# hyperplane-lab/ACL-GAN

Hardware: AMD Instinct MI355X
Metric: training images/sec at 256x256 (gen+dis step) (higher is better)
Workload: dtype fp32

## Files before the change

acl-gan_amd/_lib.py:

```python
import ctypes as C
import os

_HERE = os.path.dirname(os.path.abspath(__file__))
LIB_PATH = os.path.join(_HERE, "libaclgan_hip.so")


class AclganError(RuntimeError):
    pass


if not os.path.exists(LIB_PATH):
    raise ImportError(
        "libaclgan_hip.so not found at %s -- build it first (python -c 'import __graft_entry__ as g; g.build()' "
        "or make -C acl-gan_amd/csrc).  There is no fallback path." % LIB_PATH)

lib = C.CDLL(LIB_PATH)


class Arch(C.Structure):
    _fields_ = [(n, C.c_int) for n in (
        "input_dim_a", "input_dim_b", "gen_dim", "gen_mlp_dim", "gen_style_dim", "gen_output_dim",
        "gen_n_downsample", "gen_n_res", "dis_dim", "dis_n_layer", "dis_num_scales")]


class HParams(C.Structure):
    _fields_ = [(n, C.c_float) for n in (
        "gan_w", "gan_cw", "recon_x_w", "focus_loss", "focus_delta", "focus_upper", "focus_lower",
        "focus_epsilon", "alpha")]


class Adam(C.Structure):
    _fields_ = [(n, C.c_float) for n in ("lr", "beta1", "beta2", "eps", "weight_decay")]


class ConvDesc(C.Structure):
    _fields_ = [(n, C.c_int) for n in ("B", "Hi", "Wi", "Ci", "Co", "k", "stride", "pad", "upsample", "act")]


class ImageDesc(C.Structure):
    _fields_ = [("src_offset", C.c_int64)] + [(n, C.c_int) for n in (
        "src_h", "src_w", "res_h", "res_w", "crop_y", "crop_x", "flip", "tab_x", "tab_y", "ksize_x", "ksize_y")]


GRID_MAX_SRCS = 16


class GridSrc(C.Structure):
    _fields_ = [("data", C.c_void_p), ("bstride", C.c_int64), ("n", C.c_int), ("channels", C.c_int)]


ACT = {"none": 0, "relu": 1, "lrelu": 2, "tanh": 3}
NORM = {"none": 0, "in": 1, "adain": 2, "ln": 3, "sn": 4}
DTYPE = {"fp32": 0, "bf16": 1, "fp16": 2}
GROUP_GEN, GROUP_DIS, GROUP_SN_STATE = 0, 1, 2
EMA_COPY, EMA_BLEND = 0, 1
WEIGHTS_LIVE, WEIGHTS_EMA = 0, 1
NETS = {"gen_AB": 0, "gen_BA": 1, "dis_A": 2, "dis_B": 3, "dis_2": 4}
LOSS_NAMES = [
    "loss_gen_adv_A", "loss_gen_adv_B", "loss_gen_adv_2",
    "loss_gen_focus_B_size", "loss_gen_focus_B_digit", "loss_gen_focus_A_size", "loss_gen_focus_A_digit",
    "loss_gen_focus_A2_size", "loss_gen_focus_A2_digit", "loss_idt_A", "loss_idt_B", "loss_gen_total",
    "loss_dis_A", "loss_dis_B", "loss_dis_2", "loss_dis_total",
]

vp, ci, cf, i64, sz = C.c_void_p, C.c_int, C.c_float, C.c_int64, C.c_size_t
BUCKET_FN = C.CFUNCTYPE(None, vp, ci, ci, i64, i64)
SYNC_FN = C.CFUNCTYPE(None, vp, vp, ci)

SIGNATURES = {
    "aclgan_version": (ci, []),
    "aclgan_launch_count": (C.c_longlong, []),
    "aclgan_gemm_slices_f32": (ci, [vp, vp, vp, ci, ci, ci, ci, vp]),
    "aclgan_winograd_filter_frag": (ci, [vp, vp, ci, ci, ci, vp]),
    "aclgan_conv3x3_winograd_fused": (ci, [vp, vp, vp, vp, ci, ci, ci, ci, ci, ci, ci, ci, vp, vp]),
    "aclgan_gemm_slices_x3_scratch_bytes": (sz, [ci, ci, ci, ci]),
    "aclgan_gemm_slices_x3": (ci, [vp, vp, vp, ci, ci, ci, ci, vp, vp]),
    "aclgan_set_deterministic": (ci, [ci]),
    "aclgan_get_deterministic": (ci, []),
    "aclgan_last_error": (C.c_char_p, []),
    "aclgan_ctx_create": (ci, [C.POINTER(Arch), C.POINTER(vp)]),
    "aclgan_ctx_create_dis_norm": (ci, [C.POINTER(Arch), ci, C.POINTER(vp)]),
    "aclgan_ctx_destroy": (None, [vp]),
    "aclgan_ctx_enable_capture": (ci, [vp]),
    "aclgan_warm_streams": (ci, [ci]),
    "aclgan_debug_capture_masks": (ci, [vp, vp, sz]),
    "aclgan_debug_mask_count": (ci, [vp]),
    "aclgan_debug_mask_info": (ci, [vp, ci, C.POINTER(ci), C.POINTER(C.c_longlong), C.POINTER(ci)]),
    "aclgan_group_numel": (i64, [vp, ci]),
    "aclgan_tensor_count": (ci, [vp, ci]),
    "aclgan_tensor_info": (ci, [vp, ci, ci, C.c_char_p, ci, C.POINTER(i64), C.POINTER(ci), C.POINTER(ci)]),
    "aclgan_bind_params": (ci, [vp, ci, vp, vp, vp, vp]),
    "aclgan_bind_sn_state": (ci, [vp, vp]),
    "aclgan_sn_scratch_bytes": (sz, [ci, vp, vp]),
    "aclgan_sn_power_iteration": (ci, [ci, vp, vp, vp, vp, vp, vp, vp, vp, vp]),
    "aclgan_sn_fold": (ci, [ci, vp, vp, vp, vp, vp, vp, vp, vp, vp, vp]),
    "aclgan_workspace_bytes": (ci, [vp, ci, ci, ci, C.POINTER(sz)]),
    "aclgan_bind_workspace": (ci, [vp, vp, sz]),
    "aclgan_forward_workspace_bytes": (ci, [vp, ci, ci, ci, C.POINTER(sz)]),
    "aclgan_step_algorithmic_bytes": (ci, [vp, ci, ci, ci, ci, C.POINTER(C.c_double)]),
    "aclgan_step_executed_flops": (ci, [vp, ci, ci, ci, ci, C.POINTER(C.c_double)]),
    "aclgan_gen_update": (ci, [vp, vp, vp, vp, ci, ci, ci, C.POINTER(HParams), vp, vp]),
    "aclgan_dis_update": (ci, [vp, vp, vp, vp, ci, ci, ci, C.POINTER(HParams), vp, vp]),
    "aclgan_set_grad_buckets": (ci, [vp, i64, BUCKET_FN, vp]),
    "aclgan_set_forward_sync": (ci, [vp, SYNC_FN, vp, ci]),
    "aclgan_focus_loss_global": (ci, [vp, i64, vp, i64, cf, cf, cf, cf, cf, vp, vp, vp, vp]),
    "aclgan_bucket_schedule": (ci, [vp, ci, ci, ci, ci, ci, C.POINTER(ci), ci, C.POINTER(ci)]),
    "aclgan_zero_grad": (ci, [vp, ci, vp]),
    "aclgan_adam_step": (ci, [vp, ci, C.POINTER(Adam), ci, vp]),
    "aclgan_bind_ema": (ci, [vp, ci, vp]),
    "aclgan_adam_step_ema": (ci, [vp, ci, C.POINTER(Adam), ci, cf, ci, vp]),
    "aclgan_set_forward_weights": (ci, [vp, ci]),
    "aclgan_gen_encode": (ci, [vp, ci, vp, ci, ci, ci, vp, vp, vp]),
    "aclgan_gen_decode": (ci, [vp, ci, vp, vp, ci, ci, ci, vp, vp]),
    "aclgan_dis_forward": (ci, [vp, ci, vp, ci, ci, ci, C.POINTER(vp), vp]),
    "aclgan_conv2d_fwd": (ci, [C.POINTER(ConvDesc), vp, vp, vp, vp, vp]),
    "aclgan_conv2d_fwd_ws": (ci, [C.POINTER(ConvDesc), vp, vp, vp, vp, vp, vp]),
    "aclgan_conv2d_fwd_scratch_bytes": (sz, [C.POINTER(ConvDesc)]),
    "aclgan_conv2d_fwd_naive": (ci, [C.POINTER(ConvDesc), vp, vp, vp, vp, vp]),
    "aclgan_set_compute_dtype": (ci, [vp, ci]),
    "aclgan_bind_params16": (ci, [vp, ci, vp, vp]),
    "aclgan_bind_loss_scale": (ci, [vp, vp]),
    "aclgan_conv16_eligible": (ci, [C.POINTER(ConvDesc), ci]),
    "aclgan_pack_weights16": (ci, [vp, vp, vp, ci, ci, ci, ci, vp]),
    "aclgan_conv2d_fwd16": (ci, [C.POINTER(ConvDesc), ci, vp, vp, vp, vp, vp, vp, vp]),
    "aclgan_conv2d_fwd16_x16": (ci, [C.POINTER(ConvDesc), ci, vp, vp, vp, vp, vp, vp, vp]),
    "aclgan_conv2d_dgrad16": (ci, [C.POINTER(ConvDesc), ci, vp, vp, vp, vp, ci, vp, vp]),
    "aclgan_conv2d_wgrad16": (ci, [C.POINTER(ConvDesc), ci, vp, vp, vp, vp, vp, vp]),
    "aclgan_conv16s_ok": (ci, [C.POINTER(ConvDesc), ci]),
    "aclgan_conv2d_fwd16s": (ci, [C.POINTER(ConvDesc), ci, vp, vp, vp, vp, ci, vp]),
    "aclgan_set_tuning": (ci, [C.c_char_p, ci]),
    "aclgan_tuning": (ci, [C.c_char_p, ci, C.POINTER(ci)]),
    "aclgan_tuning_get": (ci, [C.c_char_p, C.POINTER(C.c_longlong)]),
    "aclgan_check_workspace": (ci, [vp, ci, ci, ci]),
    "aclgan_conv2d_fwd16s_stats_chunk": (ci, [C.POINTER(ConvDesc)]),
    "aclgan_conv2d_fwd16s_stats": (ci, [C.POINTER(ConvDesc), ci, vp, vp, vp, vp, ci, vp, vp]),
    "aclgan_conv2d_dgrad16s_scratch_bytes": (sz, [C.POINTER(ConvDesc)]),
    "aclgan_conv2d_dgrad16s": (ci, [C.POINTER(ConvDesc), ci, vp, vp, vp, ci, ci, vp, vp]),
    "aclgan_conv2d_wgrad16_st": (ci, [C.POINTER(ConvDesc), ci, vp, ci, vp, ci, vp, vp, vp, vp]),
    "aclgan_cast_storage": (ci, [vp, ci, vp, ci, i64, vp]),
    "aclgan_norm_fwd_st": (ci, [ci, ci, ci, ci, ci, vp, vp, vp, ci, vp, vp, vp, vp, vp, C.POINTER(ci), vp]),
    "aclgan_norm_bwd_st": (ci, [ci, ci, ci, ci, ci, vp, vp, vp, vp, ci, vp, vp, vp, vp, vp, vp, ci, vp, C.POINTER(ci), vp]),
    "aclgan_conv2d_fwd16_x16_st": (ci, [C.POINTER(ConvDesc), ci, vp, vp, vp, vp, vp, ci, vp, vp]),
    "aclgan_norm_fwd_x": (ci, [ci, ci, ci, ci, ci, vp, vp, vp, ci, vp, vp, vp, vp, vp, vp, ci, C.POINTER(ci), vp, vp]),
    "aclgan_norm_bwd_x": (ci, [ci, ci, ci, ci, ci, vp, vp, vp, vp, ci, vp, vp, vp, vp, vp, vp, ci, vp, C.POINTER(ci), vp, vp, vp]),
    "aclgan_norm_bwd_ln_params": (ci, [vp, ci, ci, vp, vp, vp]),
    "aclgan_conv2d_fwd16_scratch_bytes": (sz, [C.POINTER(ConvDesc)]),
    "aclgan_conv2d_dgrad16_scratch_bytes": (sz, [C.POINTER(ConvDesc)]),
    "aclgan_conv2d_wgrad16_scratch_bytes": (sz, [C.POINTER(ConvDesc)]),
    "aclgan_conv2d_dgrad": (ci, [C.POINTER(ConvDesc), vp, vp, vp, vp, ci, vp]),
    "aclgan_conv2d_dgrad_scratch_bytes": (sz, [C.POINTER(ConvDesc)]),
    "aclgan_conv2d_wgrad": (ci, [C.POINTER(ConvDesc), vp, vp, vp, vp, vp]),
    "aclgan_conv2d_wgrad_ws": (ci, [C.POINTER(ConvDesc), vp, vp, vp, vp, vp, vp]),
    "aclgan_conv2d_wgrad_scratch_bytes": (sz, [C.POINTER(ConvDesc)]),
    "aclgan_norm_fwd": (ci, [ci, ci, ci, ci, ci, vp, vp, vp, ci, vp, vp, vp, vp, vp, vp]),
    "aclgan_conv2d_block_fwd": (ci, [C.POINTER(ConvDesc), ci, ci, vp, vp, vp, vp, vp, ci, vp, vp, vp, vp, vp, vp, C.POINTER(C.c_int), vp]),
    "aclgan_conv2d_block_fwd_scratch_bytes": (sz, [C.POINTER(ConvDesc)]),
    "aclgan_norm_bwd": (ci, [ci, ci, ci, ci, ci, vp, vp, vp, vp, ci, vp, vp, vp, vp, vp, vp, ci, vp, vp]),
    "aclgan_norm_scratch_bytes": (sz, [ci, ci, ci]),
    "aclgan_avgpool3s2_fwd": (ci, [ci, ci, ci, ci, vp, vp, vp]),
    "aclgan_avgpool3s2_bwd": (ci, [ci, ci, ci, ci, vp, vp, ci, vp]),
    "aclgan_adam_flat": (ci, [vp, vp, vp, vp, i64, C.POINTER(Adam), ci, vp]),
    "aclgan_adam_flat_ema": (ci, [vp, vp, vp, vp, vp, i64, C.POINTER(Adam), ci, cf, ci, vp]),
    "aclgan_linear_fwd": (ci, [ci, ci, ci, vp, vp, vp, ci, vp, vp]),
    "aclgan_mlp3_fwd": (ci, [ci, ci, ci, ci, vp, vp, vp, vp, vp, vp, vp, vp, vp, vp, vp]),
    "aclgan_linear_bwd": (ci, [ci, ci, ci, vp, vp, vp, vp, ci, vp, vp, vp, vp]),
    "aclgan_gap_fwd": (ci, [ci, ci, ci, vp, vp, vp]),
    "aclgan_gap_bwd": (ci, [ci, ci, ci, vp, vp, ci, vp]),
    "aclgan_focus_blend_fwd": (ci, [ci, ci, vp, vp, vp, vp, vp, vp]),
    "aclgan_focus_blend_bwd": (ci, [ci, ci, vp, vp, vp, vp, vp, vp, ci, vp]),
    "aclgan_focus_translation_nchw": (ci, [vp, i64, vp, i64, vp, i64, vp, ci, ci, vp]),
    "aclgan_lsgan_loss": (ci, [vp, ci, cf, cf, vp, vp, cf, vp]),
    "aclgan_lsgan_loss_multi": (ci, [vp, vp, vp, vp, vp, vp, vp, ci, vp]),
    "aclgan_l1_loss": (ci, [vp, ci, vp, i64, vp, vp, cf, ci, vp]),
    "aclgan_focus_loss_scratch_bytes": (sz, [i64]),
    "aclgan_focus_loss": (ci, [vp, i64, cf, cf, cf, cf, cf, vp, vp, vp, vp, vp]),
    "aclgan_nchw_to_nhwc": (ci, [vp, vp, ci, ci, ci, ci, vp]),
    "aclgan_nhwc_to_nchw": (ci, [vp, vp, ci, ci, ci, ci, vp]),
    "aclgan_image_resample_ksize": (ci, [ci, ci]),
    "aclgan_image_resample_coeffs": (ci, [ci, ci, C.POINTER(ci), C.POINTER(ci)]),
    "aclgan_image_batch_transform": (ci, [vp, C.POINTER(ImageDesc), vp, ci, vp, vp, ci, ci, vp]),
    "aclgan_image_grid_scratch_bytes": (sz, []),
    "aclgan_image_grid_u8": (ci, [C.POINTER(GridSrc), ci, ci, ci, ci, vp, vp, vp]),
}

for _name, (_res, _args) in SIGNATURES.items():
    _fn = getattr(lib, _name)
    _fn.restype = _res
    _fn.argtypes = _args


def last_error() -> str:
    return lib.aclgan_last_error().decode("utf-8", "replace")


def check(rc: int, what: str = ""):
    if rc != 0:
        raise AclganError("%s failed (code %d): %s" % (what or "libaclgan_hip call", rc, last_error()))


def ptr(t):
    return None if t is None else C.c_void_p(t.data_ptr())


def stream_ptr(device=None):
    import torch
    return C.c_void_p(torch.cuda.current_stream(device).cuda_stream)
```

acl-gan_amd/csrc/common.h:

```cpp
#pragma once
#include <hip/hip_runtime.h>
#include <stdint.h>
#include <stddef.h>
#include <string>
#include <atomic>
#include "../../include/aclgan_hip.h"
#include "switches.h"

namespace aclgan {

void set_error(const char* fmt, ...);
int hip_fail(hipError_t e, const char* what);

extern std::atomic<long long> g_launches;

#define ACL_CHECK_LAUNCH(what)                                           \
    do {                                                                 \
        ++::aclgan::g_launches;                                          \
        hipError_t e__ = hipGetLastError();                              \
        if (e__ != hipSuccess) return ::aclgan::hip_fail(e__, what);     \
    } while (0)

#define ACL_REQUIRE(cond, ...)                                           \
    do {                                                                 \
        if (!(cond)) { ::aclgan::set_error(__VA_ARGS__); return ACLGAN_EINVAL; } \
    } while (0)

int reduce_slices_ordered(const float* part, int64_t n, int nslices, float* out, hipStream_t st);
size_t colsum_ordered_bytes(int64_t M, int C);
int colsum_ordered(const float* dy, float* db, int64_t M, int C, void* part, hipStream_t st);

static inline int cdiv(int a, int b) { return (a + b - 1) / b; }
static inline int64_t cdiv64(int64_t a, int64_t b) { return (a + b - 1) / b; }

struct ConvGeom {
    int B, Hi, Wi, Ci, Co, k, s, p, up, act;
    int Hu, Wu;
    int Hp, Wp;
    int Ho, Wo;
    int M;
    int K;
};
int make_geom(const aclgan_conv_desc* d, ConvGeom* g);

int conv_fold(const ConvGeom& g, const float* dxp, float* dx, int accumulate, hipStream_t st);
double conv_exec_flops(const ConvGeom& g, int which, bool f16);
bool conv_wgrad_fast_supported(const ConvGeom& g);
int conv_fwd(const ConvGeom& g, const float* x, const float* w, const float* bias, float* y, hipStream_t st, void* scratch = nullptr, float* stats = nullptr,
             float* keepV = nullptr);
size_t conv_fwd_keep_bytes(const ConvGeom& g);
int conv_fwd_stats_chunk(const ConvGeom& g);
size_t conv_fwd_scratch_bytes(const ConvGeom& g);
size_t conv_up5_scratch_bytes(const ConvGeom& g);
int conv_up5_fwd(const ConvGeom& g, const float* x, const float* w, const float* bias, float* y, void* scratch, hipStream_t st, float* keepV = nullptr);
int conv_fwd_naive(const ConvGeom& g, const float* x, const float* w, const float* bias, float* y, hipStream_t st);
size_t conv_dgrad_scratch_bytes(const ConvGeom& g);
int conv_dgrad(const ConvGeom& g, const float* dy, const float* w, float* dx, void* scratch, int accumulate, hipStream_t st);
int conv_wgrad(const ConvGeom& g, const float* x, const float* dy, float* dw, float* db, hipStream_t st, void* scratch = nullptr, const float* haveV = nullptr);
size_t conv_wgrad_scratch_bytes(const ConvGeom& g);
int conv_up5_dgrad(const ConvGeom& g, const float* dy, const float* w, float* dx, int accumulate, void* scratch, hipStream_t st);
int conv_up5_wgrad(const ConvGeom& g, const float* x, const float* dy, float* dw, float* db, void* scratch, hipStream_t st, const float* haveV = nullptr);

int conv_fwd_fast(const ConvGeom& g, const float* x, const float* w, const float* bias, float* y, hipStream_t st, void* scratch = nullptr, float* stats = nullptr,
                  float* keepV = nullptr);
size_t conv_fwd_fast_scratch_bytes(const ConvGeom& g);
int conv_dgrad_fast(const ConvGeom& g, const float* dy, const float* w, float* dxp, float* dx, int accumulate, bool* direct, hipStream_t st);
int conv_wgrad_fast(const ConvGeom& g, const float* x, const float* dy, float* dw, float* db, hipStream_t st, void* scratch = nullptr, const float* haveV = nullptr);
size_t conv_wgrad_fast_scratch_bytes(const ConvGeom& g);

struct WinoUCache { void* user; float* (*lookup)(void* user, const float* w, int variant, size_t bytes, bool* fresh); };
void set_wino_ucache(const WinoUCache* c);
const WinoUCache* wino_ucache();
size_t conv_wino_u_bytes(const ConvGeom& g);
int conv_wino_u_variant(const ConvGeom& g, int dgrad, bool keepV);
int conv_up5_wino_u_variant(const ConvGeom& g, int dgrad, bool keepV);
int conv_wino_prefill(const ConvGeom& g, int uv, const float* w0, int64_t w_stride, float* U0, int64_t u_stride, int count, hipStream_t st);
int wino_fused_filter_batch(const float* w0, int64_t w_stride, float* Uf0, int64_t u_stride, int count, int Co, int Ci, int flip, hipStream_t st);

bool conv_wino_ok(const ConvGeom& g);
size_t conv_wino_scratch_bytes(const ConvGeom& g);
int conv_fwd_wino(const ConvGeom& g, const float* x, const float* w, const float* bias, float* y, void* scratch, hipStream_t st, float* stats = nullptr,
                  float* keepV = nullptr);
size_t conv_wino_keep_bytes(const ConvGeom& g);
size_t conv_up5_wino_keep_bytes(const ConvGeom& g);
int conv_dgrad_wino_interior(const ConvGeom& g, const float* dy, const float* w, float* dx, int accumulate, void* scratch, hipStream_t st);
size_t conv_wgrad_wino_scratch_bytes(const ConvGeom& g);
bool conv_up5_wino_ok(const ConvGeom& g);
size_t conv_up5_wino_fwd_scratch_bytes(const ConvGeom& g);
size_t conv_up5_wino_dgrad_scratch_bytes(const ConvGeom& g);
size_t conv_up5_wino_wgrad_scratch_bytes(const ConvGeom& g);
int conv_up5_wino_fwd_phases(const ConvGeom& g, const float* x, const float* wp, const float* bias, float* y, void* scratch, hipStream_t st, float* keepV = nullptr,
                             const float* wkey = nullptr);
int conv_up5_wino_dgrad_phases(const ConvGeom& g, const float* dy, const float* wp, float* dx, int accumulate, void* scratch, hipStream_t st,
                               const float* wkey = nullptr);
bool wino_u_cached(const float* wkey, int variant);
int conv_up5_wino_wgrad_phases(const ConvGeom& g, const float* x, const float* dy, float* dwp, float* db, void* scratch, hipStream_t st, const float* haveV = nullptr);
size_t conv_up5_dgrad_scratch_bytes(const ConvGeom& g);
// ... 120 lines not shown
```

acl-gan_amd/csrc/engine.hip:

```cpp
#include "common.h"
#include <dlfcn.h>

#include <functional>
#include <map>
#include <string>
#include <vector>
#include <tuple>
#include <mutex>
#include <algorithm>
#include <cstring>
#include <cstdio>
#include <cstdlib>

namespace aclgan {

struct TensorInfo {
    std::string name;
    int64_t offset;
    int64_t numel;
    int shape[4];
    int ndim;
};

struct Group {
// ... 62 lines not shown
struct StreamPool {
    static const int N = 4;
    hipStream_t s[N] = {nullptr, nullptr, nullptr, nullptr};
    static StreamPool& of_device() {
        static StreamPool pools[16];
        int dev = 0;
        (void)hipGetDevice(&dev);
        return pools[(dev >= 0 && dev < 16) ? dev : 0];
    }
    int get(int i, hipStream_t* out) {
        static std::mutex mu;
        std::lock_guard<std::mutex> lock(mu);
        if (!s[i]) {
            const hipError_t e = hipStreamCreateWithFlags(&s[i], hipStreamNonBlocking);
            if (e != hipSuccess) { s[i] = nullptr; return hip_fail(e, "stream pool"); }
        }
        *out = s[i];
        return ACLGAN_OK;
    }
};
}

struct aclgan_ctx {
    aclgan_arch arch;
    int dis_norm = ACLGAN_NORM_NONE;
    struct SnLayer { int co, k; std::string key; int64_t u_off, v_off; };
    std::vector<SnLayer> sn_layers[5];
    Group sn;
    std::vector<std::string> pass_names;
    std::vector<int> tape_pass;
    std::map<std::string, int> pass_count;
    int cur_pass = -1;
    int pass_begin(const char* net, const char* what) {
        if (!Roctx::get().on || dry) return -1;
        const std::string base = std::string(net) + "." + what;
        const int n = ++pass_count[base];
        pass_names.push_back(base + "#" + std::to_string(n));
        const int prev = cur_pass;
        cur_pass = (int)pass_names.size() - 1;
        Roctx::get().push((pass_names.back() + "@" + std::to_string((long long)g_launches)).c_str());
        return prev;
    }
    void pass_end(int prev) {
        if (!Roctx::get().on || dry) return;
        Roctx::get().pop();
        Roctx::get().push(("~end@" + std::to_string((long long)g_launches)).c_str());
        Roctx::get().pop();
        cur_pass = prev;
    }
    Group groups[2];
    char* ws = nullptr;
    size_t ws_bytes = 0;
    hipStream_t st = nullptr;
    bool dry = false;
    size_t top = 0, peak = 0;
    std::vector<Act*> acts;
    std::vector<TapeOp> tape;
    int dtype = ACLGAN_DTYPE_FP32;
    unsigned short* w16[2] = {nullptr, nullptr};
    unsigned short* w16t[2] = {nullptr, nullptr};
    float* lscale = nullptr;
    float* ema = nullptr;
    int fwd_weights = ACLGAN_WEIGHTS_LIVE;
    bool read_ema = false;
    const float* weights(int group) const { return group == ACLGAN_GROUP_GEN && read_ema ? ema : groups[group].param; }
    std::vector<int64_t> cv_off[2];
    std::vector<int> cv_co[2], cv_taps[2], cv_ci[2];
    int trained = -1;
    bool fire_dry = false;
    aclgan_sync_fn sync_fn = nullptr;
    void* sync_user = nullptr;
    int sync_world = 1;
    int64_t bucket_elems = 0;
    aclgan_bucket_fn bucket_fn = nullptr;
    void* bucket_user = nullptr;
    std::vector<int> bucket_order;
    struct NeedKey {
        int which, B, H, W, dtype; long long epoch; int determ, buckets;
        bool operator<(const NeedKey& o) const {
            return std::tie(which, B, H, W, dtype, epoch, determ, buckets) < std::tie(o.which, o.B, o.H, o.W, o.dtype, o.epoch, o.determ, o.buckets);
        }
    };
    std::map<NeedKey, size_t> need_cache;
    double alg_bytes = 0.0;
    void count(double bytes) { alg_bytes += bytes; }
    double exec_flops = 0.0;
    size_t keep_total = 0;
    struct MaskEnt { int B, H, W, C, act; long long off; };
    unsigned char* mask_dst = nullptr; size_t mask_cap = 0, mask_top = 0;
    std::vector<MaskEnt> mask_log;
    struct UEnt { float* u; bool filled; int layout; int lane, ck; };
    std::map<std::pair<const float*, int>, UEnt> ucache;
    WinoUCache ucache_hook;
    static float* ucache_lookup(void* user, const float* w, int variant, size_t bytes, bool* fresh) {
        aclgan_ctx* c = (aclgan_ctx*)user;
        const int layout = variant >> 4;
        auto it = c->ucache.find(std::make_pair(w, variant & 15));
        if (it == c->ucache.end()) return nullptr;
        UEnt& e = it->second;
        if (!e.filled) {
            *fresh = true;
            if (bytes) { e.filled = true; e.layout = layout; e.lane = c->cur_lane; e.ck = c->nck(c->cur_lane); }
            return e.u;
        }
        if (e.layout != layout) return nullptr;
        *fresh = false;
        if (bytes && c->nlanes > 1 && e.lane != c->cur_lane && c->wait_ck(c->cur_lane, e.lane, e.ck) != ACLGAN_OK) return nullptr;
        return e.u;
    }
    int ucache_reserve(const float* w, int variant, size_t bytes) {
        if (sw(SW_NOUCACHE) || !bytes || ucache.count(std::make_pair(w, variant))) return ACLGAN_OK;
        float* u = (float*)alloc(bytes);
        if (!u) return ACLGAN_ENOMEM;
        ucache[std::make_pair(w, variant)] = UEnt{u, false, 0, 0, 0};
        return ACLGAN_OK;
    }
    bool act16() const { return dtype != ACLGAN_DTYPE_FP32 && sw(SW_ACT16); }

    hipStream_t st2 = nullptr;
    hipEvent_t ev_fork = nullptr, ev_join = nullptr;
    bool side_pending = false;
    size_t top2 = 0, peak2 = 0;
    void* alloc2(size_t bytes) {
        const size_t need = top2 + ((bytes + 255) & ~(size_t)255);
        top2 = need;
        if (need > peak2) peak2 = need;
        if (dry) return (void*)(uintptr_t)4096;
        if (peak + need + 256 > ws_bytes) return nullptr;
        return ws + ((ws_bytes - need) & ~(size_t)255);
    }
    int side_fork() {
        if (dry) return ACLGAN_OK;
        if (!st2) {
            int rc = aclgan::StreamPool::of_device().get(0, &st2_pool);
            if (rc) return rc;
            st2 = st2_pool;
        }
        if (st2 == st) return ACLGAN_OK;
        if (!ev_fork) {
            hipError_t e = hipEventCreateWithFlags(&ev_fork, hipEventDisableTiming);
            if (e == hipSuccess) e = hipEventCreateWithFlags(&ev_join, hipEventDisableTiming);
            if (e != hipSuccess) return aclgan::hip_fail(e, "side stream events");
        }
        hipError_t e = hipEventRecord(ev_fork, st);
        if (e == hipSuccess) e = hipStreamWaitEvent(st2, ev_fork, 0);
        if (e != hipSuccess) return aclgan::hip_fail(e, "side stream fork");
        side_pending = true;
        return ACLGAN_OK;
    }
    int side_join() {
        if (dry || !side_pending) return ACLGAN_OK;
        hipError_t e = hipEventRecord(ev_join, st2);
        if (e == hipSuccess) e = hipStreamWaitEvent(st0 ? st0 : st, ev_join, 0);
        if (e != hipSuccess) return aclgan::hip_fail(e, "side stream join");
        side_pending = false;
        return ACLGAN_OK;
    }

    static const int MAXL = 4;
    hipStream_t st0 = nullptr;
    hipStream_t lane_st[MAXL] = {nullptr, nullptr, nullptr, nullptr};
    int nlanes = 1, cur_lane = 0;
    std::vector<hipEvent_t> ev_pool; size_t ev_next = 0;
    std::vector<hipEvent_t> lane_evs[MAXL];
    int seen[MAXL][MAXL] = {};
    size_t hw[MAXL] = {0, 0, 0, 0};
    bool lane_dirty[MAXL] = {false, false, false, false};
    int pass_seq = 0, cur_pass_id = -1;
    hipStream_t lane_stream(int l) const { return l == 0 ? st0 : lane_st[l]; }
    int nck(int l) const { return (int)lane_evs[l].size(); }
    hipStream_t st2_pool = nullptr;
    int lanes_begin(int want) {
        nlanes = std::max(1, std::min(want, (int)MAXL));
        if (!sw(SW_SIDE_STREAM)) nlanes = 1;
        bool capturing = false;
        if (!dry) {
            hipStreamCaptureStatus cs = hipStreamCaptureStatusNone;
            if (hipStreamIsCapturing(st, &cs) == hipSuccess && cs != hipStreamCaptureStatusNone) capturing = true;
            else (void)hipGetLastError();
        }
        if (capturing) nlanes = 1;
        cur_lane = 0; st0 = st;
        for (int l = 0; l < MAXL; ++l) { lane_evs[l].clear(); hw[l] = 0; lane_dirty[l] = false; for (int m = 0; m < MAXL; ++m) seen[l][m] = 0; }
        ev_next = 0;
        if (dry) return ACLGAN_OK;
        if (sw(SW_SIDE_STREAM) && !st2_pool) { int rc = aclgan::StreamPool::of_device().get(0, &st2_pool); if (rc) return rc; }
        st2 = capturing ? st : st2_pool;
        for (int l = 1; l < nlanes; ++l)
            if (!lane_st[l]) { int rc = aclgan::StreamPool::of_device().get(l, &lane_st[l]); if (rc) return rc; }
        return ACLGAN_OK;
    }
    int checkpoint(int l) {
        hipEvent_t ev = nullptr;
        if (!dry) {
            if (ev_next == ev_pool.size()) {
                hipEvent_t e = nullptr;
                hipError_t rc = hipEventCreateWithFlags(&e, hipEventDisableTiming);
                if (rc != hipSuccess) return aclgan::hip_fail(rc, "lane event");
                ev_pool.push_back(e);
            }
            ev = ev_pool[ev_next++];
            hipError_t rc = hipEventRecord(ev, lane_stream(l));
            if (rc != hipSuccess) return aclgan::hip_fail(rc, "lane checkpoint");
        }
        lane_evs[l].push_back(ev);
        lane_dirty[l] = false;
        return ACLGAN_OK;
    }
    int mark() { return nlanes > 1 ? checkpoint(cur_lane) : ACLGAN_OK; }
    int set_lane(int l) {
        if (nlanes <= 1) return ACLGAN_OK;
        l %= nlanes;
// ... 15 lines not shown
        if (!dry) {
            hipError_t e = hipStreamWaitEvent(lane_stream(d), lane_evs[s][k], 0);
            if (e != hipSuccess) return aclgan::hip_fail(e, "lane wait");
        }
        lane_dirty[d] = true;
        seen[d][s] = k + 1;
        return ACLGAN_OK;
    }
    int need(Act* a) {
        if (nlanes <= 1 || !a) return ACLGAN_OK;
        Act* r = a->root();
        for (int i = 0; i < r->ndst; ++i)
            if (r->dst[i].lane != cur_lane) { int rc = wait_ck(cur_lane, r->dst[i].lane, r->dst[i].ck); if (rc) return rc; }
        return ACLGAN_OK;
    }
    void wrote(Act* a) {
        if (!a) return;
        Act* r = a->root();
        for (int i = 0; i < r->ndst; ++i)
            if (r->dst[i].lane == cur_lane) { r->dst[i].ck = nck(cur_lane); return; }
        if (r->ndst < 4) r->dst[r->ndst++] = Act::Stamp{cur_lane, nck(cur_lane)};
    }
    int acq(Act* a) {
        if (nlanes <= 1 || !a) return ACLGAN_OK;
        Act* r = a->root();
        if (r->gst.lane >= 0 && r->gst.lane != cur_lane) { int rc = wait_ck(cur_lane, r->gst.lane, r->gst.ck); if (rc) return rc; }
        r->gst = Act::Stamp{cur_lane, nck(cur_lane)};
        return ACLGAN_OK;
    }
    int lanes_join() {
        if (nlanes > 1) {
            int rc = set_lane(0);
            if (rc) return rc;
            for (int l = 1; l < nlanes; ++l) {
                if (lane_dirty[l]) { rc = checkpoint(l); if (rc) return rc; }
                if (nck(l) > 0) { rc = wait_ck(0, l, nck(l) - 1); if (rc) return rc; }
            }
        }
        return side_join();
    }
    int lanes_barrier() {
        int rc = lanes_join();
        if (rc || nlanes <= 1) return rc;
        rc = checkpoint(0);
        if (rc) return rc;
        for (int l = 1; l < nlanes; ++l) { rc = wait_ck(l, 0, nck(0) - 1); if (rc) return rc; }
        for (int l = 0; l < MAXL; ++l) hw[l] = 0;
        return ACLGAN_OK;
    }
    void lanes_quiesce() {
        if (dry) return;
        for (int l = 1; l < nlanes; ++l) if (lane_st[l]) (void)hipStreamSynchronize(lane_st[l]);
        if (st2) (void)hipStreamSynchronize(st2);
        side_pending = false;
        cur_lane = 0; if (st0) st = st0;
    }
    ~aclgan_ctx() {
        reset_step();
        if (ev_fork) (void)hipEventDestroy(ev_fork);
        if (ev_join) (void)hipEventDestroy(ev_join);
        for (hipEvent_t e : ev_pool) (void)hipEventDestroy(e);
    }
    void reset_step() {
        for (Act* a : acts) delete a;
        acts.clear();
        tape.clear();
        tape_pass.clear(); pass_names.clear(); pass_count.clear(); cur_pass = -1;
        top = 0;
        top2 = 0;
        keep_total = 0;
        ucache.clear();
        read_ema = false;
        for (int l = 0; l < MAXL; ++l) { lane_evs[l].clear(); hw[l] = 0; lane_dirty[l] = false; for (int m = 0; m < MAXL; ++m) seen[l][m] = 0; }
        ev_next = 0; cur_lane = 0; nlanes = 1; pass_seq = 0; cur_pass_id = -1;
        if (st0) { st = st0; st0 = nullptr; }
    }
    void* alloc(size_t bytes) {
        size_t a = (top + 255) & ~(size_t)255;
        if (nlanes > 1) for (int l = 0; l < nlanes; ++l) if (l != cur_lane && hw[l] > a) a = hw[l];
        top = a + bytes;
        if (nlanes > 1) { const size_t e = (top + 255) & ~(size_t)255; if (e > hw[cur_lane]) hw[cur_lane] = e; }
        if (top > peak) peak = top;
        if (dry) return (void*)(uintptr_t)(a + 4096);
        if (top + peak2 + 256 > ws_bytes) return nullptr;
        return ws + a;
    }
    float* allocf(int64_t n) { return (float*)alloc((size_t)n * sizeof(float)); }
    Act* new_act(int B, int H, int W, int C, bool need_grad, int st = 0) {
        Act* a = new Act();
        a->B = B; a->H = H; a->W = W; a->C = C; a->need_grad = need_grad; a->dt = st; a->gdt = st;
        a->d = (float*)alloc((size_t)a->numel() * (st ? 2 : 4));
        if (need_grad) a->g = allocf(a->numel());
        acts.push_back(a);
        wrote(a);
        return a;
    }
    Act* new_view(Act* joint, int b0, int nb) {
        Act* a = new Act();
        a->B = nb; a->H = joint->H; a->W = joint->W; a->C = joint->C; a->need_grad = joint->need_grad;
        const int64_t off = (int64_t)b0 * joint->H * joint->W * joint->C;
        a->d = joint->d + off;
        a->g = joint->g ? joint->g + off : nullptr;
        a->parent = joint;
        acts.push_back(a);
        return a;
    }
    void push(std::function<int()> fn, std::initializer_list<std::pair<const float*, int64_t>> grads = {}) {
        TapeOp op;
        op.fn = std::move(fn);
        if (trained >= 0 && groups[trained].grad)
            for (const auto& g : grads)
                if (g.first && g.second > 0 && op.ng < 4 && g.first >= groups[trained].grad && g.first < groups[trained].grad + groups[trained].numel) {
                    op.goff[op.ng] = g.first - groups[trained].grad; op.gnum[op.ng] = g.second; ++op.ng;
                }
        op.lane = cur_lane; op.pass = cur_pass_id;
        tape.push_back(std::move(op));
        tape_pass.push_back(cur_pass);
    }
    PW pw(int group, int net, const std::string& key, bool with_bias = true) const;
    int64_t numel_of(int group, int net, const std::string& key) const;
    const float* param(int group, int net, const std::string& key) const;
    float* gradp(int group, int net, const std::string& key) const;
};

namespace aclgan {


#define RUN(expr)                                  \
    do {                                           \
        if (!c.dry) { int rc__ = (expr); if (rc__) return rc__; } \
    } while (0)
#define CHK(expr)                                  \
    do { int rc__ = (expr); if (rc__) return rc__; } while (0)
#define NEED(ptr)                                  \
    do { if (!(ptr)) { set_error("workspace too small (need > %zu bytes, bound %zu)", c.top, c.ws_bytes); return ACLGAN_ENOMEM; } } while (0)

static void add_tensor(Group& g, const std::string& name, int ndim, int d0, int d1 = 1, int d2 = 1, int d3 = 1) {
    TensorInfo t;
    t.name = name; t.offset = g.numel; t.ndim = ndim;
    t.shape[0] = d0; t.shape[1] = d1; t.shape[2] = d2; t.shape[3] = d3;
    t.numel = (int64_t)d0 * d1 * d2 * d3;
    g.index[name] = (int)g.tensors.size();
    g.tensors.push_back(t);
    g.numel += (t.numel + 3) / 4 * 4;
}
static void add_conv(Group& g, const std::string& prefix, int co, int ci, int k) {
    add_tensor(g, prefix + ".weight", 4, co, ci, k, k);
    add_tensor(g, prefix + ".bias", 1, co);
}

static void build_gen(Group& g, const std::string& net, const aclgan_arch& a) {
    char buf[160];
    const int nd = a.gen_n_downsample, nr = a.gen_n_res, sd = a.gen_style_dim;
    int d = a.gen_dim;
    add_conv(g, net + "/enc_style.model.0.conv", d, a.input_dim_a, 7);
    for (int i = 0; i < 2; ++i) { snprintf(buf, sizeof buf, "/enc_style.model.%d.conv", 1 + i); add_conv(g, net + buf, 2 * d, d, 4); d *= 2; }
    for (int i = 0; i < 2; ++i) { snprintf(buf, sizeof buf, "/enc_style.model.%d.conv", 3 + i); add_conv(g, net + buf, d, d, 4); }
    add_conv(g, net + "/enc_style.model.6", sd, d, 1);
    d = a.gen_dim;
    add_conv(g, net + "/enc_content.model.0.conv", d, a.input_dim_a, 7);
    for (int i = 0; i < nd; ++i) { snprintf(buf, sizeof buf, "/enc_content.model.%d.conv", 1 + i); add_conv(g, net + buf, 2 * d, d, 4); d *= 2; }
    for (int r = 0; r < nr; ++r)
        for (int j = 0; j < 2; ++j) { snprintf(buf, sizeof buf, "/enc_content.model.%d.model.%d.model.%d.conv", 1 + nd, r, j); add_conv(g, net + buf, d, d, 3); }
    for (int r = 0; r < nr; ++r)
        for (int j = 0; j < 2; ++j) { snprintf(buf, sizeof buf, "/dec.model.0.model.%d.model.%d.conv", r, j); add_conv(g, net + buf, d, d, 3); }
    int idx = 2;
    for (int i = 0; i < nd; ++i) {
        snprintf(buf, sizeof buf, "/dec.model.%d.norm.gamma", idx); add_tensor(g, net + buf, 1, d / 2);
        snprintf(buf, sizeof buf, "/dec.model.%d.norm.beta", idx); add_tensor(g, net + buf, 1, d / 2);
        snprintf(buf, sizeof buf, "/dec.model.%d.conv", idx); add_conv(g, net + buf, d / 2, d, 5);
        d /= 2; idx += 2;
    }
    snprintf(buf, sizeof buf, "/dec.model.%d.conv", idx - 1); add_conv(g, net + buf, a.gen_output_dim, d, 7);
    const int C = a.gen_dim << nd, nad = 2 * C * 2 * nr, md = a.gen_mlp_dim;
    add_tensor(g, net + "/mlp.model.0.fc.weight", 2, md, sd); add_tensor(g, net + "/mlp.model.0.fc.bias", 1, md);
    add_tensor(g, net + "/mlp.model.1.fc.weight", 2, md, md); add_tensor(g, net + "/mlp.model.1.fc.bias", 1, md);
    add_tensor(g, net + "/mlp.model.2.fc.weight", 2, nad, md); add_tensor(g, net + "/mlp.model.2.fc.bias", 1, nad);
}

static void build_dis(Group& g, const std::string& net, int input_dim, const aclgan_arch& a, std::vector<aclgan_ctx::SnLayer>* sn = nullptr,
                      Group* st = nullptr) {
    char buf[160];
    for (int s = 0; s < a.dis_num_scales; ++s) {
        int d = a.dis_dim;
        snprintf(buf, sizeof buf, "/cnns.%d.0.conv", s); add_conv(g, net + buf, d, input_dim, 4);
        for (int i = 0; i < a.dis_n_layer - 1; ++i) {
            snprintf(buf, sizeof buf, "/cnns.%d.%d.conv", s, i + 1);
            if (sn) {
                const std::string pre = net + buf + ".module.";
                add_tensor(g, pre + "bias", 1, 2 * d);
                add_tensor(g, pre + "weight_bar", 4, 2 * d, d, 4, 4);
                aclgan_ctx::SnLayer L;
                L.co = 2 * d; L.k = 16 * d; L.key = std::string(buf + 1) + ".module.";
                L.u_off = st->numel; add_tensor(*st, pre + "weight_u", 1, L.co);
                L.v_off = st->numel; add_tensor(*st, pre + "weight_v", 1, L.k);
                sn->push_back(L);
            } else {
                add_conv(g, net + buf, 2 * d, d, 4);
            }
            d *= 2;
        }
        snprintf(buf, sizeof buf, "/cnns.%d.%d", s, a.dis_n_layer); add_conv(g, net + buf, 1, d, 1);
    }
}

static const char* NET_NAMES[5] = {"gen_AB", "gen_BA", "dis_A", "dis_B", "dis_2"};

}

const float* aclgan_ctx::param(int group, int net, const std::string& key) const {
    const Group& g = groups[group];
    auto it = g.index.find(std::string(NET_NAMES[net]) + "/" + key);
    if (it == g.index.end() || !g.param) return nullptr;
    return weights(group) + g.tensors[it->second].offset;
}
float* aclgan_ctx::gradp(int group, int net, const std::string& key) const {
    const Group& g = groups[group];
    auto it = g.index.find(std::string(NET_NAMES[net]) + "/" + key);
    if (it == g.index.end() || !g.grad) return nullptr;
    return g.grad + g.tensors[it->second].offset;
}
int64_t aclgan_ctx::numel_of(int group, int net, const std::string& key) const {
    const Group& g = groups[group];
    auto it = g.index.find(std::string(NET_NAMES[net]) + "/" + key);
    return it == g.index.end() ? 0 : g.tensors[it->second].numel;
}
PW aclgan_ctx::pw(int group, int net, const std::string& key, bool with_bias) const {
    PW p;
    p.w = param(group, net, key + ".weight"); p.dw = gradp(group, net, key + ".weight"); p.nw = numel_of(group, net, key + ".weight");
    if (with_bias) { p.b = param(group, net, key + ".bias"); p.db = gradp(group, net, key + ".bias"); p.nb = numel_of(group, net, key + ".bias"); }
    if (dtype != ACLGAN_DTYPE_FP32 && p.w && w16[group] && w16t[group]) {
        const int64_t off = p.w - weights(group);
        p.w16 = w16[group] + off; p.w16t = w16t[group] + off;
    }
    return p;
}

namespace aclgan {

struct PassScope {
    aclgan_ctx& c; int prev, prev_id;
    PassScope(aclgan_ctx& c_, int net, const char* what) : c(c_), prev(c_.pass_begin(NET_NAMES[net], what)), prev_id(c_.cur_pass_id) { c.cur_pass_id = c.pass_seq++; }
    ~PassScope() { c.pass_end(prev); c.cur_pass_id = prev_id; }
};

struct NormSpec {
    int kind = ACLGAN_NORM_NONE;
    const float* w = nullptr; const float* b = nullptr;
    float* dw = nullptr; float* db = nullptr;
    int w_stride = 0;
};

static inline void mark_written(Act* a) { a->gw = true; }

static int conv_block(aclgan_ctx& c, const PW& W, bool train_w, Act* in, int Co, int k, int stride, int pad, int up, int act,
                      const NormSpec& ns, Act* residual, Act** out_p, int out16 = 1) {
    aclgan_conv_desc d;
    d.B = in->B; d.Hi = in->H; d.Wi = in->W; d.Ci = in->C; d.Co = Co; d.k = k; d.stride = stride; d.pad = pad; d.upsample = up;
    d.act = ns.kind == ACLGAN_NORM_NONE ? act : ACLGAN_ACT_NONE;
    ConvGeom g;
    CHK(make_geom(&d, &g));
    if (!W.w) { set_error("conv_block: parameters not bound"); return ACLGAN_EINVAL; }
    CHK(c.need(in)); CHK(c.need(residual));
    Act* const gin = in;
    const bool want_grad = train_w || in->need_grad || ns.dw != nullptr;
    const bool has_norm = ns.kind != ACLGAN_NORM_NONE;
    const int dt = c.dtype;
    const bool h16 = dt != ACLGAN_DTYPE_FP32 && W.w16 != nullptr;
    const bool f16 = h16 && conv16_eligible(g, 0), d16 = h16 && conv16_eligible(g, 1), w16 = h16 && conv16_eligible(g, 2);
    const bool a16 = h16 && c.act16();
    const bool s_bwd = a16 && f16 && d16 && w16 && conv16s_ok(g, 1);
    const bool s_fwd = a16 && f16 && conv16s_ok(g, 0) && in->dt != 0;
    if (in->dt != 0 && !(f16 && (w16 || !train_w))) {
        Act* in32 = c.new_act(in->B, in->H, in->W, in->C, false, 0);
        NEED(in32->d);
        RUN(cast_storage(in->d, in->dt, in32->d, 0, in->numel(), c.st));
        in = in32;
    }
    const int out_st = (a16 && Co % 64 == 0 && out16) ? dt : 0;
    const int co_st = has_norm ? ((s_bwd && sw(SW_CO16)) ? dt : 0) : ((f16 || !out_st) ? out_st : 0);
    Act* co = c.new_act(g.B, g.Ho, g.Wo, Co, want_grad, co_st);
    NEED(co->d); if (want_grad) NEED(co->g);
    Act* out = co;
    float *mean = nullptr, *rstd = nullptr, *ss = nullptr;
    const int HW = g.Ho * g.Wo;
    if (has_norm) {
        out = c.new_act(g.B, g.Ho, g.Wo, Co, want_grad, out_st);
        NEED(out->d); if (want_grad) NEED(out->g);
        const int nstat = ns.kind == ACLGAN_NORM_LN ? g.B : g.B * Co;
        mean = c.allocf(nstat); rstd = c.allocf(nstat);
        NEED(mean); NEED(rstd);
        if (want_grad && (act == ACLGAN_ACT_RELU || act == ACLGAN_ACT_LRELU) && sw(SW_NORM_MASK)) { ss = c.allocf((int64_t)2 * g.B * Co); NEED(ss); }
        co->gdt = s_bwd ? dt : 0;
    } else if (out_st && !co_st) {
        out = c.new_act(g.B, g.Ho, g.Wo, Co, want_grad, out_st);
        NEED(out->d); if (want_grad) NEED(out->g);
        out->gdt = 0;
    } else {
        out->gdt = s_bwd ? co_st : 0;
    }
    if (gin->need_grad && !s_bwd) gin->gdt = 0;
    float* keepV = nullptr;
    if (train_w && !f16 && !w16) {
        const size_t kb = conv_fwd_keep_bytes(g);
        if (kb && c.keep_total + kb <= (size_t)(sw_real(SW_KEEPV_BUDGET_GB) * 1073741824.0) + 1) { keepV = (float*)c.alloc(kb); NEED(keepV); c.keep_total += kb; }
    }
    const size_t ubytes = f16 ? 0 : conv_wino_u_bytes(g);
    if (ubytes && c.ucache_reserve(W.w, g.up ? 2 : 0, ubytes)) { set_error("workspace too small (filter-transform cache)"); return ACLGAN_ENOMEM; }
    const double es_in = in->dt ? 2.0 : 4.0, es_co = co->dt ? 2.0 : 4.0, es_out = out->dt ? 2.0 : 4.0, es_w = f16 ? 2.0 : 4.0;
    c.count(es_in * (double)in->numel() + es_w * (double)Co * g.K + 4.0 * Co + es_co * (double)co->numel());
    c.exec_flops += conv_exec_flops(g, 0, f16);
    if (out != co) c.count((es_co + es_out) * (double)co->numel() + ((has_norm && residual) ? (residual->dt ? 2.0 : 4.0) * (double)co->numel() : 0.0));
    const size_t mark = c.top;
    const int schunk = !has_norm ? 0 : (s_fwd ? conv_fwd16s_stats_chunk(g) : (!f16 ? conv_fwd_stats_chunk(g) : 0));
    float* stats = nullptr;
    if (schunk) { stats = c.allocf((size_t)2 * g.B * (HW / schunk) * Co); NEED(stats); }
    {
        const size_t fmark = c.top;
        void* fscr = nullptr;
        const size_t fb = s_fwd ? 0 : (f16 ? conv_fwd16_scratch_bytes(g) : conv_fwd_scratch_bytes(g));
        if (fb) { fscr = c.alloc(fb); NEED(fscr); }
        if (s_fwd) RUN(conv_fwd16s(g, dt, in->d, W.w16, W.b, co->d, co->dt, c.st, stats));
        else if (f16) RUN(conv_fwd16(g, dt, in->dt ? nullptr : in->d, W.w, W.w16, W.b, co->d, fscr, c.st, in->dt ? in->d : nullptr, co->dt));
        else RUN(conv_fwd(g, in->d, W.w, W.b, co->d, c.st, fscr, stats, keepV));
        c.top = fmark;
    }
    NormST nst;
    nst.x = co->dt; nst.y = out->dt; nst.res = residual ? residual->dt : 0;
    if (has_norm) {
        void* scr = c.alloc(norm_scratch_bytes(g.B, HW, Co));
        NEED(scr);
        RUN(norm_fwd(ns.kind, act, g.B, HW, Co, co->d, ns.w, ns.b, ns.w_stride, residual ? residual->d : nullptr, out->d, mean, rstd, scr, c.st, stats, schunk, &nst, ss));
    } else if (out != co) {
        RUN(cast_storage(co->d, co->dt, out->d, out->dt, co->numel(), c.st));
    }
    c.top = mark;
    *out_p = out;
    if (c.mask_dst && !c.dry && want_grad && (act == ACLGAN_ACT_RELU || act == ACLGAN_ACT_LRELU)) {
        const size_t n = (size_t)out->numel();
        if (c.mask_top + n > c.mask_cap) { set_error("aclgan_debug_capture_masks: buffer too small (%zu bytes)", c.mask_cap); return ACLGAN_ENOMEM; }
        RUN(positive_mask(out->d, out->dt, c.mask_dst + c.mask_top, (int64_t)n, c.st));
        c.mask_log.push_back(aclgan_ctx::MaskEnt{out->B, out->H, out->W, out->C, act, (long long)c.mask_top});
        c.mask_top += n;
    }
    c.wrote(out); c.wrote(co);
    if (!want_grad) return ACLGAN_OK;
    aclgan_ctx* cp = &c;
    const bool ln_train = ns.kind == ACLGAN_NORM_LN && ns.dw != nullptr;
    c.push([=]() -> int {
        aclgan_ctx& c = *cp;
        if (!out->gw) return ACLGAN_OK;
        CHK(c.acq(out));
        if (residual && residual->need_grad) CHK(c.acq(residual));
        if (gin->need_grad) CHK(c.acq(gin));
        const double eg_out = out->gdt ? 2.0 : 4.0, eg_co = (has_norm ? co->gdt : (s_bwd ? dt : out->gdt)) ? 2.0 : 4.0, eg_in = gin->gdt ? 2.0 : 4.0;
        c.count((es_co + eg_out + eg_co) * (double)co->numel() + ((residual && residual->need_grad) ? (residual->gdt ? 2.0 : 4.0) * (double)co->numel() : 0.0));
        if (train_w) { c.count(es_in * (double)in->numel() + eg_co * (double)co->numel() + 4.0 * ((double)Co * g.K + Co)); c.exec_flops += conv_exec_flops(g, 2, w16); }
        if (gin->need_grad) { c.count(eg_co * (double)co->numel() + es_w * (double)Co * g.K + eg_in * (double)in->numel()); c.exec_flops += conv_exec_flops(g, 1, d16); }
        const bool side = train_w && sw(SW_SIDE_STREAM);
        if (ubytes && gin->need_grad && !d16 && c.ucache_reserve(W.w, g.up ? 3 : 1, ubytes)) { set_error("workspace too small (filter-transform cache)"); return ACLGAN_ENOMEM; }
        float* g16 = nullptr;
        const size_t mark_pre = c.top;
        if (!has_norm && s_bwd && out->gdt == 0) {
            g16 = (float*)c.alloc((size_t)out->numel() * 2);
            NEED(g16);
        }
        float* sbc = nullptr;
        if (ln_train && side) { sbc = c.allocf((int64_t)2 * g.B * Co); NEED(sbc); }
        const size_t mark0 = side ? c.top : mark_pre;
        const float* dyp = nullptr;
        int dy_st = 0;
        if (has_norm) {
            const size_t mark = c.top;
            void* scr = c.alloc(norm_scratch_bytes(g.B, HW, Co));
            NEED(scr);
            float* dres = nullptr; int dacc = 0;
            if (residual && residual->need_grad) { dres = residual->g; dacc = residual->gw ? 1 : 0; mark_written(residual); }
            NormST bst;
            bst.x = co->dt; bst.y = out->dt; bst.dy = out->gdt; bst.dx = co->gdt; bst.dres = residual ? residual->gdt : 0;
            RUN(norm_bwd(ns.kind, act, g.B, HW, Co, co->d, out->d, out->g, ns.w, ns.w_stride, mean, rstd, co->g, ns.dw, ns.db, dres, dacc, scr, c.st, &bst, sbc, ss));
            c.top = mark;
            dyp = co->g; dy_st = co->gdt;
        } else if (s_bwd && out->gdt == 0) {
            RUN(cast_storage(out->g, 0, g16, dt, out->numel(), c.st));
            RUN(act_bwd_inplace(act, out->d, g16, out->numel(), c.st, out->dt, dt));
            dyp = g16; dy_st = dt;
        } else {
            RUN(act_bwd_inplace(act, co->d, out->g, out->numel(), c.st, co->dt, out->gdt));
            dyp = out->g; dy_st = out->gdt;
        }
        if (train_w) {
            const size_t mark = c.top;
            void* wscr = nullptr;
            const size_t wb = w16 ? conv_wgrad16_scratch_bytes(g) : conv_wgrad_scratch_bytes(g);
            hipStream_t wst = c.st;
            if (side) {
                CHK(c.side_fork());
                if (!c.dry) wst = c.st2;
                c.top2 = 0;
                if (wb) { wscr = c.alloc2(wb); if (!wscr) { set_error("workspace too small for the side-stream scratch"); return ACLGAN_ENOMEM; } }
                if (sbc) RUN(norm_bwd_ln_params(sbc, g.B, Co, ns.dw, ns.db, wst));
            } else if (wb) { wscr = c.alloc(wb); NEED(wscr); }
            if (w16) RUN(conv_wgrad16(g, dt, in->d, dyp, W.dw, W.db, wscr, wst, in->dt, dy_st));
            else {
                if (in->dt || dy_st) { set_error("conv_block: fp32 weight-gradient kernel on 16-bit operands"); return ACLGAN_EINVAL; }
                RUN(conv_wgrad(g, in->d, dyp, W.dw, W.db, wst, wscr, keepV));
            }
            c.top = mark;
        }
        if (gin->need_grad) {
            const size_t mark = c.top;
            if (s_bwd) {
                if (!dy_st) { set_error("conv_block: 16-bit-storage dgrad on an fp32 gradient"); return ACLGAN_EINVAL; }
                void* scr = c.alloc(conv_dgrad16s_scratch_bytes(g));
                NEED(scr);
                RUN(conv_dgrad16s(g, dt, dyp, W.w16t, gin->g, gin->gdt, gin->gw ? 1 : 0, scr, c.st));
            } else {
                if (dy_st || gin->gdt) { set_error("conv_block: fp32-output dgrad kernel on 16-bit gradients"); return ACLGAN_EINVAL; }
                void* scr = c.alloc(d16 ? conv_dgrad16_scratch_bytes(g) + 256 : conv_dgrad_scratch_bytes(g));
                NEED(scr);
                if (d16) RUN(conv_dgrad16(g, dt, dyp, W.w, W.w16t, gin->g, gin->gw ? 1 : 0, scr, c.st));
                else RUN(conv_dgrad(g, dyp, W.w, gin->g, scr, gin->gw ? 1 : 0, c.st));
            }
            mark_written(gin);
            c.top = mark;
        }
        c.top = mark0;
        return ACLGAN_OK;
    }, {{train_w ? W.dw : nullptr, W.nw}, {train_w ? W.db : nullptr, W.nb}, {ln_train ? ns.dw : nullptr, Co}, {ln_train ? ns.db : nullptr, Co}});
    return ACLGAN_OK;
}

static int prefill_wino_u(aclgan_ctx& c, int net, int B, int H, int W, bool train) {
    if (sw(SW_NOUCACHE) || !sw(SW_U_BATCH)) return ACLGAN_OK;
    const aclgan_arch& a = c.arch;
    const int nd = a.gen_n_downsample, count = 2 * a.gen_n_res, C = a.gen_dim << nd;
    if (count < 2) return ACLGAN_OK;
    aclgan_conv_desc d;
    d.B = B; d.Hi = H >> nd; d.Wi = W >> nd; d.Ci = C; d.Co = C; d.k = 3; d.stride = 1; d.pad = 1; d.upsample = 0; d.act = ACLGAN_ACT_NONE;
    ConvGeom g;
    if (make_geom(&d, &g)) return ACLGAN_OK;
    const size_t ubytes = conv_wino_u_bytes(g);
    if (!ubytes) return ACLGAN_OK;
    if (c.dtype != ACLGAN_DTYPE_FP32 && c.w16[0] && conv16_eligible(g, 0)) return ACLGAN_OK;
    char buf[160];
    for (int part = 0; part < 2; ++part) {
        std::vector<const float*> ws;
        for (int r = 0; r < a.gen_n_res; ++r)
            for (int j = 0; j < 2; ++j) {
                if (part == 0) snprintf(buf, sizeof buf, "enc_content.model.%d.model.%d.model.%d.conv.weight", 1 + nd, r, j);
                else snprintf(buf, sizeof buf, "dec.model.0.model.%d.model.%d.conv.weight", r, j);
                ws.push_back(c.param(0, net, buf));
            }
        if (!ws[0]) continue;
        const int64_t wstride = ws[1] - ws[0];
        bool even = wstride > 0;
        for (int i = 1; i < count && even; ++i) even = ws[i] && ws[i] - ws[i - 1] == wstride;
        if (!even) continue;
        for (int dgrad = 0; dgrad <= (train ? 1 : 0); ++dgrad) {
            const bool keepV = train && !dgrad && conv_fwd_keep_bytes(g) > 0;
            const int uv = conv_wino_u_variant(g, dgrad, keepV);
            if (uv < 0 || c.ucache.count(std::make_pair(ws[0], uv & 15))) continue;
            float* u0 = nullptr;
            bool contiguous = true;
            const size_t ustride = (ubytes + 255) & ~(size_t)255;
            for (int i = 0; i < count; ++i) {
                float* u = (float*)c.alloc(ubytes);
                NEED(u);
                if (i == 0) u0 = u;
                else if ((char*)u != (char*)u0 + (size_t)i * ustride) contiguous = false;
                c.ucache[std::make_pair(ws[i], uv & 15)] = aclgan_ctx::UEnt{u, contiguous, uv >> 4, c.cur_lane, c.nck(c.cur_lane)};
            }
            if (!contiguous) {
                for (int i = 0; i < count; ++i) c.ucache[std::make_pair(ws[i], uv & 15)].filled = false;
                continue;
            }
            RUN(conv_wino_prefill(g, uv, ws[0], wstride, u0, (int64_t)(ustride / sizeof(float)), count, c.st));
        }
    }
    return ACLGAN_OK;
}

static int prefill_on_side_lane(aclgan_ctx& c, int B, int H, int W, bool train) {
    const int AB = ACLGAN_NET_GEN_AB, BA = ACLGAN_NET_GEN_BA;
    if (c.nlanes <= 1) { CHK(prefill_wino_u(c, AB, B, H, W, train)); return prefill_wino_u(c, BA, B, H, W, train); }
    const int LP = c.nlanes - 1;
    CHK(c.mark());
    const int k0 = c.nck(0) - 1;
    CHK(c.set_lane(LP));
    CHK(c.wait_ck(LP, 0, k0));
    CHK(prefill_wino_u(c, AB, B, H, W, train)); CHK(prefill_wino_u(c, BA, B, H, W, train));
    CHK(c.mark());
    return c.set_lane(0);
}

static int content_encode(aclgan_ctx& c, int net, bool train, Act* x, Act** out) {
    PassScope pass(c, net, "encode");
    const aclgan_arch& a = c.arch;
    char buf[160];
    NormSpec in_; in_.kind = ACLGAN_NORM_IN;
    Act* h = nullptr;
    int d = a.gen_dim;
    CHK(conv_block(c, c.pw(0, net, "enc_content.model.0.conv"), train, x, d, 7, 1, 3, 0, ACLGAN_ACT_RELU, in_, nullptr, &h));
    for (int i = 0; i < a.gen_n_downsample; ++i) {
        snprintf(buf, sizeof buf, "enc_content.model.%d.conv", 1 + i);
        CHK(conv_block(c, c.pw(0, net, buf), train, h, 2 * d, 4, 2, 1, 0, ACLGAN_ACT_RELU, in_, nullptr, &h));
        d *= 2;
    }
    for (int r = 0; r < a.gen_n_res; ++r) {
        Act *t = nullptr, *o = nullptr;
        snprintf(buf, sizeof buf, "enc_content.model.%d.model.%d.model.0.conv", 1 + a.gen_n_downsample, r);
        CHK(conv_block(c, c.pw(0, net, buf), train, h, d, 3, 1, 1, 0, ACLGAN_ACT_RELU, in_, nullptr, &t));
        snprintf(buf, sizeof buf, "enc_content.model.%d.model.%d.model.1.conv", 1 + a.gen_n_downsample, r);
        CHK(conv_block(c, c.pw(0, net, buf), train, t, d, 3, 1, 1, 0, ACLGAN_ACT_NONE, in_, h, &o));
        h = o;
    }
    *out = h;
    return ACLGAN_OK;
}

static int dense(aclgan_ctx& c, const PW& W, bool train_w, Act* in, int O, int act, Act** out_p, bool launch = true) {
    const int B = in->B, I = in->H * in->W * in->C;
    const bool want = train_w || in->need_grad;
    CHK(c.need(in));
    Act* out = c.new_act(B, 1, 1, O, want);
    NEED(out->d); if (want) NEED(out->g);
    if (!W.w) { set_error("dense: parameters not bound"); return ACLGAN_EINVAL; }
    if (launch) RUN(linear_fwd(B, I, O, in->d, W.w, W.b, act, out->d, c.st));
    c.count(4.0 * ((double)B * I + (double)O * I + O + (double)B * O) * (want ? 3.0 : 1.0));
    c.wrote(out);
    *out_p = out;
    if (!want) return ACLGAN_OK;
    aclgan_ctx* cp = &c;
    c.push([=]() -> int {
        aclgan_ctx& c = *cp;
        if (!out->gw) return ACLGAN_OK;
        CHK(c.acq(out));
        if (in->need_grad) CHK(c.acq(in));
        float* dx = nullptr;
        float* tmp = nullptr;
        const size_t mark = c.top;
        if (in->need_grad) {
            if (in->gw) { tmp = c.allocf((int64_t)B * I); NEED(tmp); dx = tmp; } else dx = in->g;
        }
        const bool side = train_w && sw(SW_SIDE_STREAM);
        RUN(linear_bwd(B, I, O, in->d, out->d, out->g, W.w, act, dx, (train_w && !side) ? W.dw : nullptr, (train_w && !side) ? W.db : nullptr, c.st));
        if (side) {
            CHK(c.side_fork());
            RUN(linear_bwd_params(B, I, O, in->d, out->g, W.dw, W.db, c.st2));
        }
        if (in->need_grad) {
            if (tmp) {
                RUN(gap_bwd(B, 1, I, tmp, in->g, 1, c.st));
            }
            mark_written(in);
        }
        c.top = mark;
        return ACLGAN_OK;
    }, {{train_w ? W.dw : nullptr, W.nw}, {train_w ? W.db : nullptr, W.nb}});
    return ACLGAN_OK;
}

static int style_encode(aclgan_ctx& c, int net, bool train, Act* x, Act** out) {
    PassScope pass(c, net, "style");
    const aclgan_arch& a = c.arch;
    char buf[160];
    NormSpec none;
    Act* h = nullptr;
    int d = a.gen_dim;
    CHK(conv_block(c, c.pw(0, net, "enc_style.model.0.conv"), train, x, d, 7, 1, 3, 0, ACLGAN_ACT_RELU, none, nullptr, &h));
    for (int i = 0; i < 2; ++i) {
        snprintf(buf, sizeof buf, "enc_style.model.%d.conv", 1 + i);
        CHK(conv_block(c, c.pw(0, net, buf), train, h, 2 * d, 4, 2, 1, 0, ACLGAN_ACT_RELU, none, nullptr, &h));
        d *= 2;
    }
    for (int i = 0; i < 2; ++i) {
        snprintf(buf, sizeof buf, "enc_style.model.%d.conv", 3 + i);
        CHK(conv_block(c, c.pw(0, net, buf), train, h, d, 4, 2, 1, 0, ACLGAN_ACT_RELU, none, nullptr, &h));
    }
    const bool want = h->need_grad;
// ... 342 lines not shown
        std::vector<size_t> first(nb, n);
        for (size_t i = 0; i < n; ++i)
            for (int r = 0; r < c.tape[i].ng; ++r) {
                const int64_t b0 = c.tape[i].goff[r] / c.bucket_elems, b1 = (c.tape[i].goff[r] + c.tape[i].gnum[r] - 1) / c.bucket_elems;
                for (int64_t b = b0; b <= b1 && b < nb; ++b) first[b] = std::min(first[b], i);
            }
        done_at.resize(n);
        c.bucket_order.clear();
        for (int b = 0; b < nb; ++b) {
            if (first[b] == n) fire_bucket(c, b);
            else done_at[first[b]].push_back(b);
        }
    }
    CHK(c.lanes_barrier());
    const bool marks = Roctx::get().on && !c.dry && c.tape_pass.size() == n;
    int open = -1, last_pass = -2;
    for (size_t i = n; i-- > 0;) {
        if (marks && c.tape_pass[i] != open) {
            if (open >= 0) { Roctx::get().pop(); Roctx::get().push(("~end@" + std::to_string((long long)g_launches)).c_str()); Roctx::get().pop(); }
            open = c.tape_pass[i];
            if (open >= 0) Roctx::get().push(("bwd:" + c.pass_names[open] + "@" + std::to_string((long long)g_launches)).c_str());
        }
        if (c.tape[i].pass != last_pass) { if (last_pass != -2) CHK(c.mark()); last_pass = c.tape[i].pass; }
        CHK(c.set_lane(c.tape[i].lane));
        int rc_i = c.tape[i].fn();
        if (!rc_i && !c.dry && sw(SW_FAULT_AT) >= 0 && (int)(n - 1 - i) == sw(SW_FAULT_AT)) { set_error("injected fault after backward closure %d (tuning key fault_at)", sw(SW_FAULT_AT)); rc_i = ACLGAN_EHIP; }
        if (rc_i) { if (marks && open >= 0) Roctx::get().pop(); return rc_i; }
        if (buckets && !done_at[i].empty()) {
            const int lane = c.cur_lane;
            CHK(c.lanes_join());
            for (int b : done_at[i]) fire_bucket(c, b);
            CHK(c.set_lane(lane));
        }
    }
    if (marks && open >= 0) { Roctx::get().pop(); Roctx::get().push(("~end@" + std::to_string((long long)g_launches)).c_str()); Roctx::get().pop(); }
    return c.lanes_join();
}
static int run_tape(aclgan_ctx& c) {
    const int rc = run_tape_impl(c);
    if (rc) c.lanes_quiesce();
    return rc;
}

static int check_shape(const aclgan_ctx& c, int B, int H, int W) {
    ACL_REQUIRE(B >= 1 && H >= 64 && W >= 64, "batch shape (%d,%d,%d): need B>=1 and H,W>=64 (third discriminator scale reflect-pads a >=2x2 map)", B, H, W);
    const int q = 1 << c.arch.gen_n_downsample;
    ACL_REQUIRE(H % q == 0 && W % q == 0, "H, W must be multiples of %d (2^n_downsample: decoder output must match the input size)", q);
    return ACLGAN_OK;
}

static int gen_update_impl(aclgan_ctx& c, const float* x_a, const float* x_b, const float* z, int B, int H, int W,
                           const aclgan_hparams& hp, float* L) {
    CHK(check_shape(c, B, H, W));
    const bool focus = hp.focus_loss > 0.f;
    ACL_REQUIRE(c.arch.gen_output_dim == (focus ? 4 : 3), "focus_loss %s 0 needs gen.output_dim %d (trainer.py:107-121), the context was built with %d",
                focus ? ">" : "<=", focus ? 4 : 3, c.arch.gen_output_dim);
    const int sd = c.arch.gen_style_dim;
    const int AB = ACLGAN_NET_GEN_AB, BA = ACLGAN_NET_GEN_BA;
    const int nfs = 2 * focus_sums_blocks((int64_t)B * H * W);
    float* sums = c.allocf((int64_t)3 * nfs);
    NEED(sums);
    if (!c.dry) {
        hipError_t e = hipMemsetAsync(L, 0, sizeof(float) * (ACLGAN_L_GEN_TOTAL + 1), c.st);
        if (e != hipSuccess) return hip_fail(e, "memset losses");
    }
    CHK(c.lanes_begin(sw(SW_LANES)));
    CHK(pack_params(c));
    Act *xa, *xb, *z1, *z2, *z3;
    CHK(input_act(c, x_a, B, 3, H, W, &xa));
    CHK(input_act(c, x_b, B, 3, H, W, &xb));
    CHK(wrap_vec(c, z, B, sd, 1.f, &z1));
    CHK(wrap_vec(c, z + (size_t)B * sd, B, sd, hp.alpha, &z2));
    CHK(wrap_vec(c, z + (size_t)2 * B * sd, B, sd, 1.f, &z3));
    CHK(prefill_on_side_lane(c, B, H, W, true));
    Act *c1, *c2, *s2, *c4, *s4, *c3;
    Act *dB4, *dA4, *xB, *xA, *pA1, *rA4, *rB4, *dA24, *xA2, *pA2;
    Act* jA = c.new_act(2 * B, H, W, 3, true);
    Act* jP = c.new_act(2 * B, H, W, 6, true);
    NEED(jA->d); NEED(jA->g); NEED(jP->d); NEED(jP->g);
    const int L0 = 0, L1 = 1, L2 = c.nlanes > 2 ? 2 : 1, LS = c.nlanes > 2 ? 2 : 0;
#define PASS(expr) do { CHK(expr); CHK(c.mark()); } while (0)
    CHK(c.mark());
    CHK(c.set_lane(L0));
    PASS(content_encode(c, AB, true, xa, &c1));
    CHK(c.set_lane(L1));
    PASS(content_encode(c, BA, true, xa, &c2));
    PASS(style_encode(c, BA, true, xa, &s2));
    CHK(c.set_lane(L0));
    PASS(decode(c, AB, true, c1, z1, &dB4)); CHK(zero_grad_of(c, dB4));
    PASS(blend(c, dB4, xa, nullptr, &xB, nullptr));
    CHK(c.set_lane(L1));
    PASS(decode(c, BA, true, c2, z2, &dA4)); CHK(zero_grad_of(c, dA4));
    Act *vA1 = c.new_view(jA, 0, B), *vP1 = c.new_view(jP, 0, B), *vA2 = c.new_view(jA, B, B), *vP2 = c.new_view(jP, B, B);
    PASS(blend(c, dA4, xa, xa, &xA, &pA1, vA1, vP1));
    CHK(c.set_lane(L0));
    PASS(content_encode(c, BA, true, xB, &c3));
    PASS(decode(c, BA, true, c3, z3, &dA24)); CHK(zero_grad_of(c, dA24));
    PASS(blend(c, dA24, xB, xa, &xA2, &pA2, vA2, vP2));
    CHK(c.set_lane(L1));
    PASS(decode(c, BA, true, c2, s2, &rA4)); CHK(zero_grad_of(c, rA4));
    CHK(c.set_lane(L2));
    PASS(content_encode(c, AB, true, xb, &c4));
    PASS(style_encode(c, AB, true, xb, &s4));
    PASS(decode(c, AB, true, c4, s4, &rB4)); CHK(zero_grad_of(c, rB4));
    PASS(dis_lsgan(c, ACLGAN_NET_DIS_B, false, xB, B, {{1.f, 1.f, hp.gan_w, L + ACLGAN_L_GEN_ADV_B}}, L1, LS));
    if (c.dis_norm != ACLGAN_NORM_SN) {
        PASS(dis_lsgan(c, ACLGAN_NET_DIS_A, false, jA, B, {{1.f, 0.5f, hp.gan_w, L + ACLGAN_L_GEN_ADV_A}, {1.f, 0.5f, hp.gan_w, L + ACLGAN_L_GEN_ADV_A}}, L0, L2));
        PASS(dis_lsgan(c, ACLGAN_NET_DIS_2, false, jP, B, {{1.f, 1.f, hp.gan_cw, L + ACLGAN_L_GEN_ADV_2},
                                                            {0.f, 1.f, hp.gan_cw, L + ACLGAN_L_GEN_ADV_2}}, L1, LS));
    } else {
        PASS(dis_lsgan(c, ACLGAN_NET_DIS_A, false, vA1, B, {{1.f, 0.5f, hp.gan_w, L + ACLGAN_L_GEN_ADV_A}}, L0, L2));
        PASS(dis_lsgan(c, ACLGAN_NET_DIS_A, false, vA2, B, {{1.f, 0.5f, hp.gan_w, L + ACLGAN_L_GEN_ADV_A}}, L0, L2));
        PASS(dis_lsgan(c, ACLGAN_NET_DIS_2, false, vP1, B, {{1.f, 1.f, hp.gan_cw, L + ACLGAN_L_GEN_ADV_2}}, L1, LS));
        PASS(dis_lsgan(c, ACLGAN_NET_DIS_2, false, vP2, B, {{0.f, 1.f, hp.gan_cw, L + ACLGAN_L_GEN_ADV_2}}, L1, LS));
    }
    CHK(c.lanes_join());
    const int64_t npix = (int64_t)B * H * W;
    const float fscale = hp.focus_loss / (float)H / (float)W / (float)B / 3.f;
    struct { Act* a; int size_slot; int digit_slot; } fl[3] = {
        {dB4, ACLGAN_L_GEN_FOCUS_B_SIZE, ACLGAN_L_GEN_FOCUS_B_DIGIT},
        {dA4, ACLGAN_L_GEN_FOCUS_A_SIZE, ACLGAN_L_GEN_FOCUS_A_DIGIT},
        {dA24, ACLGAN_L_GEN_FOCUS_A2_SIZE, ACLGAN_L_GEN_FOCUS_A2_DIGIT}};
    float* ftot = nullptr;
    if (c.sync_fn) { ftot = c.allocf(8); NEED(ftot); }
    for (int i = 0; i < 3 && focus; ++i) RUN(focus_sums(fl[i].a->d, npix, hp.focus_epsilon, hp.focus_upper, sums + (size_t)i * nfs, c.st));
    if (c.mask_dst && !c.dry) {
        auto cap = [&](int code, int C_, size_t n) -> int {
            if (c.mask_top + n > c.mask_cap) { set_error("aclgan_debug_capture_masks: buffer too small (%zu bytes)", c.mask_cap); return ACLGAN_ENOMEM; }
            c.mask_log.push_back(aclgan_ctx::MaskEnt{B, H, W, C_, code, (long long)c.mask_top});
            c.mask_top += n;
            return ACLGAN_OK;
        };
        for (int i = 0; i < 3 && focus; ++i) {
            const size_t n = (size_t)fl[i].a->numel();
            unsigned char* dst = c.mask_dst + c.mask_top;
            CHK(cap(100, fl[i].a->C, n));
            RUN(positive_mask(fl[i].a->d, fl[i].a->dt, dst, (int64_t)n, c.st));
        }
        Act* rr[2] = {rA4, rB4}; Act* xx[2] = {xa, xb};
        for (int i = 0; i < 2; ++i) {
            unsigned char* dst = c.mask_dst + c.mask_top;
            CHK(cap(101, 3, (size_t)npix * 3));
            RUN(positive_mask_diff(rr[i]->d, rr[i]->C, xx[i]->d, 3, dst, npix, c.st));
        }
    }
    c.count(4.0 * (double)npix * ((focus ? 3 * 2 : 0) + 2 * (4 + 3 + 4)));
    if (ftot && focus) {
        RUN(focus_totals(sums, npix, 3, ftot, c.st));
        if (!c.dry) c.sync_fn(c.sync_user, ftot, 6);
    }
    for (int i = 0; i < 3 && focus; ++i)
        RUN(focus_loss_finish(fl[i].a->d, npix, sums + (size_t)i * nfs, hp.focus_delta, hp.focus_upper, hp.focus_lower, hp.focus_epsilon, fscale,
                              L + fl[i].size_slot, L + fl[i].digit_slot, fl[i].a->g, c.st, c.lscale, ftot ? ftot + 2 * i : nullptr,
                              npix * (int64_t)c.sync_world));
    {
        const size_t mark = c.top;
        float* l1p = c.allocf(2 * L1_PART_FLOATS);
        NEED(l1p);
        RUN(l1_loss(rA4->d, rA4->C, xa->d, npix, L + ACLGAN_L_IDT_A, rA4->g, hp.recon_x_w, 1, c.st, c.lscale, l1p));
        RUN(l1_loss(rB4->d, rB4->C, xb->d, npix, L + ACLGAN_L_IDT_B, rB4->g, hp.recon_x_w, 1, c.st, c.lscale, l1p + L1_PART_FLOATS));
        c.top = mark;
    }
    if (!c.dry) {
        hipLaunchKernelGGL(gen_total_kernel, dim3(1), dim3(1), 0, c.st, L, hp, ftot ? fscale / (float)c.sync_world : fscale);
        ACL_CHECK_LAUNCH("gen_total_kernel");
    }
    return run_tape(c);
}

static int dis_update_impl(aclgan_ctx& c, const float* x_a, const float* x_b, const float* z, int B, int H, int W,
                           const aclgan_hparams& hp, float* L) {
    CHK(check_shape(c, B, H, W));
    const bool focus = hp.focus_loss > 0.f;
    ACL_REQUIRE(c.arch.gen_output_dim == (focus ? 4 : 3), "focus_loss %s 0 needs gen.output_dim %d (trainer.py:266-276), the context was built with %d",
                focus ? ">" : "<=", focus ? 4 : 3, c.arch.gen_output_dim);
    const int sd = c.arch.gen_style_dim;
    const int AB = ACLGAN_NET_GEN_AB, BA = ACLGAN_NET_GEN_BA;
    if (!c.dry) {
        hipError_t e = hipMemsetAsync(L + ACLGAN_L_DIS_A, 0, sizeof(float) * 4, c.st);
        if (e != hipSuccess) return hip_fail(e, "memset losses");
    }
    CHK(c.lanes_begin(sw(SW_LANES)));
    CHK(pack_params(c));
    Act *xa, *xb, *z1, *z2, *z3;
    CHK(input_act(c, x_a, B, 3, H, W, &xa));
    CHK(input_act(c, x_b, B, 3, H, W, &xb));
    CHK(wrap_vec(c, z, B, sd, 1.f, &z1));
    CHK(wrap_vec(c, z + (size_t)B * sd, B, sd, hp.alpha, &z2));
    CHK(wrap_vec(c, z + (size_t)2 * B * sd, B, sd, 1.f, &z3));
    CHK(prefill_on_side_lane(c, B, H, W, false));
    Act *c1, *c2, *c3, *dB4, *dA4, *dA24, *xB, *xA, *xA2, *pA1, *pA2;
    Act* jA = c.new_act(3 * B, H, W, 3, false);
    Act* jB = c.new_act(2 * B, H, W, 3, false);
    Act* jP = c.new_act(2 * B, H, W, 6, false);
    NEED(jA->d); NEED(jB->d); NEED(jP->d);
    if (!c.dry) {
        hipError_t e = hipMemcpyAsync(jA->d + (size_t)2 * xa->numel(), xa->d, sizeof(float) * xa->numel(), hipMemcpyDeviceToDevice, c.st);
        if (e == hipSuccess) e = hipMemcpyAsync(jB->d + (size_t)xb->numel(), xb->d, sizeof(float) * xb->numel(), hipMemcpyDeviceToDevice, c.st);
        if (e != hipSuccess) return hip_fail(e, "copy real images into the joint discriminator batch");
    }
    const int L0 = 0, L1 = 1, L2 = c.nlanes > 2 ? 2 : 1, LS = c.nlanes > 2 ? 2 : 0;
    CHK(c.mark());
    CHK(c.set_lane(L0));
    PASS(content_encode(c, AB, false, xa, &c1));
    CHK(c.set_lane(L1));
    PASS(content_encode(c, BA, false, xa, &c2));
    CHK(c.set_lane(L0));
    PASS(decode(c, AB, false, c1, z1, &dB4));
    PASS(blend(c, dB4, xa, nullptr, &xB, nullptr, c.new_view(jB, 0, B), nullptr));
    CHK(c.set_lane(L1));
    PASS(decode(c, BA, false, c2, z2, &dA4));
    PASS(blend(c, dA4, xa, xa, &xA, &pA1, c.new_view(jA, 0, B), c.new_view(jP, 0, B)));
    const bool sn = c.dis_norm == ACLGAN_NORM_SN;
    if (!sn) PASS(dis_lsgan(c, ACLGAN_NET_DIS_B, true, jB, B, {{0.f, 1.f, hp.gan_w, L + ACLGAN_L_DIS_B}, {1.f, 1.f, hp.gan_w, L + ACLGAN_L_DIS_B}}, L1, L2));
    else {
        PASS(dis_lsgan(c, ACLGAN_NET_DIS_B, true, c.new_view(jB, 0, B), B, {{0.f, 1.f, hp.gan_w, L + ACLGAN_L_DIS_B}}, L1, L2));
        PASS(dis_lsgan(c, ACLGAN_NET_DIS_B, true, c.new_view(jB, B, B), B, {{1.f, 1.f, hp.gan_w, L + ACLGAN_L_DIS_B}}, L1, L2));
    }
    CHK(c.set_lane(L0));
    PASS(content_encode(c, BA, false, xB, &c3));
    PASS(decode(c, BA, false, c3, z3, &dA24));
    PASS(blend(c, dA24, xB, xa, &xA2, &pA2, c.new_view(jA, B, B), c.new_view(jP, B, B)));
    if (!sn) {
        PASS(dis_lsgan(c, ACLGAN_NET_DIS_A, true, jA, B, {{0.f, 0.5f, hp.gan_w, L + ACLGAN_L_DIS_A}, {0.f, 0.5f, hp.gan_w, L + ACLGAN_L_DIS_A},
                                                           {1.f, 1.0f, hp.gan_w, L + ACLGAN_L_DIS_A}}, L0, L2));
        PASS(dis_lsgan(c, ACLGAN_NET_DIS_2, true, jP, B, {{0.f, 1.f, hp.gan_cw, L + ACLGAN_L_DIS_2}, {1.f, 1.f, hp.gan_cw, L + ACLGAN_L_DIS_2}}, L1, LS));
    } else {
        Act* vx = c.new_view(jA, 2 * B, B);
        PASS(dis_lsgan(c, ACLGAN_NET_DIS_A, true, c.new_view(jA, 0, B), B, {{0.f, 0.5f, hp.gan_w, L + ACLGAN_L_DIS_A}}, L0, L2));
        PASS(dis_lsgan(c, ACLGAN_NET_DIS_A, true, vx, B, {{1.f, 0.5f, hp.gan_w, L + ACLGAN_L_DIS_A}}, L0, L2));
        PASS(dis_lsgan(c, ACLGAN_NET_DIS_A, true, c.new_view(jA, B, B), B, {{0.f, 0.5f, hp.gan_w, L + ACLGAN_L_DIS_A}}, L0, L2));
        PASS(dis_lsgan(c, ACLGAN_NET_DIS_A, true, vx, B, {{1.f, 0.5f, hp.gan_w, L + ACLGAN_L_DIS_A}}, L0, L2));
        PASS(dis_lsgan(c, ACLGAN_NET_DIS_2, true, c.new_view(jP, 0, B), B, {{0.f, 1.f, hp.gan_cw, L + ACLGAN_L_DIS_2}}, L1, LS));
        PASS(dis_lsgan(c, ACLGAN_NET_DIS_2, true, c.new_view(jP, B, B), B, {{1.f, 1.f, hp.gan_cw, L + ACLGAN_L_DIS_2}}, L1, LS));
    }
    CHK(c.lanes_join());
    if (!c.dry) {
        hipLaunchKernelGGL(dis_total_kernel, dim3(1), dim3(1), 0, c.st, L, hp);
        ACL_CHECK_LAUNCH("dis_total_kernel");
    }
    return run_tape(c);
}
#undef PASS

}

extern "C" {

int aclgan_ctx_create(const aclgan_arch* arch, aclgan_ctx** out) {
    return aclgan_ctx_create_dis_norm(arch, ACLGAN_NORM_NONE, out);
}

int aclgan_ctx_create_dis_norm(const aclgan_arch* arch, int dis_norm, aclgan_ctx** out) {
    ACL_REQUIRE(arch && out, "null argument");
    ACL_REQUIRE(dis_norm == ACLGAN_NORM_NONE || dis_norm == ACLGAN_NORM_SN, "dis_norm %d: only none (%d) and sn (%d) are implemented", dis_norm,
                ACLGAN_NORM_NONE, ACLGAN_NORM_SN);
    ACL_REQUIRE(arch->input_dim_a == 3 && arch->input_dim_b == 6, "input_dim_a must be 3 and input_dim_b 6 (trainer.py:19-23,132-133)");
    ACL_REQUIRE(arch->gen_output_dim == 4 || arch->gen_output_dim == 3, "gen.output_dim must be 4 (image + focus mask, trainer.py:108) or 3 (non-focus configuration, trainer.py:117-121)");
    ACL_REQUIRE(arch->gen_dim >= 4 && (arch->gen_dim & (arch->gen_dim - 1)) == 0, "gen.dim must be a power of two >= 4");
    ACL_REQUIRE(arch->dis_dim >= 4 && arch->dis_dim % 4 == 0, "dis.dim must be a multiple of 4");
    ACL_REQUIRE(arch->gen_n_downsample >= 1 && arch->gen_n_res >= 1 && arch->dis_n_layer >= 1 && arch->dis_num_scales >= 1, "bad layer counts");
    ACL_REQUIRE(arch->gen_mlp_dim >= 1 && arch->gen_style_dim >= 1, "bad mlp/style dims");
    ACL_REQUIRE(dis_norm != ACLGAN_NORM_SN || arch->dis_num_scales * (arch->dis_n_layer - 1) <= SN_MAX_LAYERS,
                "spectral norm: at most %d normalised layers per discriminator", SN_MAX_LAYERS);
    aclgan_ctx* c = new aclgan_ctx();
    c->arch = *arch;
    c->dis_norm = dis_norm;
    const bool sn = dis_norm == ACLGAN_NORM_SN;
    build_gen(c->groups[0], "gen_AB", *arch);
    build_gen(c->groups[0], "gen_BA", *arch);
    build_dis(c->groups[1], "dis_A", arch->input_dim_a, *arch, sn ? &c->sn_layers[ACLGAN_NET_DIS_A] : nullptr, &c->sn);
    build_dis(c->groups[1], "dis_B", arch->input_dim_a, *arch, sn ? &c->sn_layers[ACLGAN_NET_DIS_B] : nullptr, &c->sn);
    build_dis(c->groups[1], "dis_2", arch->input_dim_b, *arch, sn ? &c->sn_layers[ACLGAN_NET_DIS_2] : nullptr, &c->sn);
    for (int g = 0; g < 2; ++g)
        for (const TensorInfo& t : c->groups[g].tensors)
            if (t.ndim == 4) {
                c->cv_off[g].push_back(t.offset); c->cv_co[g].push_back(t.shape[0]);
                c->cv_taps[g].push_back(t.shape[2] * t.shape[3]); c->cv_ci[g].push_back(t.shape[1]);
            }
    *out = c;
    return ACLGAN_OK;
}

void aclgan_ctx_destroy(aclgan_ctx* ctx) { delete ctx; }

int aclgan_ctx_enable_capture(aclgan_ctx* ctx) {
    ACL_REQUIRE(ctx, "null ctx");
    return ACLGAN_OK;
}

int aclgan_warm_streams(int lanes) {
    int n = 0;
    if (hipGetDeviceCount(&n) != hipSuccess || n <= 0) { (void)hipGetLastError(); return ACLGAN_OK; }
    if (!sw(SW_SIDE_STREAM)) return ACLGAN_OK;
    lanes = std::max(1, std::min(lanes <= 0 ? sw(SW_LANES) : lanes, 3));
    hipStream_t s = nullptr;
    int rc = aclgan::StreamPool::of_device().get(0, &s);
    for (int l = 1; l < lanes && rc == ACLGAN_OK; ++l) rc = aclgan::StreamPool::of_device().get(l, &s);
    return rc;
}

int aclgan_debug_capture_masks(aclgan_ctx* ctx, unsigned char* dst, size_t cap_bytes) {
    ACL_REQUIRE(ctx, "null ctx");
    ctx->mask_dst = dst; ctx->mask_cap = dst ? cap_bytes : 0; ctx->mask_top = 0; ctx->mask_log.clear();
    return ACLGAN_OK;
}
int aclgan_debug_mask_count(const aclgan_ctx* ctx) { return ctx ? (int)ctx->mask_log.size() : 0; }
int aclgan_debug_mask_info(const aclgan_ctx* ctx, int index, int* dims4, long long* offset, int* act) {
    ACL_REQUIRE(ctx && index >= 0 && index < (int)ctx->mask_log.size(), "mask index out of range");
    const aclgan_ctx::MaskEnt& e = ctx->mask_log[index];
    if (dims4) { dims4[0] = e.B; dims4[1] = e.H; dims4[2] = e.W; dims4[3] = e.C; }
    if (offset) *offset = e.off;
    if (act) *act = e.act;
    return ACLGAN_OK;
}

int aclgan_set_compute_dtype(aclgan_ctx* ctx, int dtype) {
    ACL_REQUIRE(ctx && dtype >= ACLGAN_DTYPE_FP32 && dtype <= ACLGAN_DTYPE_FP16, "bad ctx / dtype %d", dtype);
    ctx->dtype = dtype;
    return ACLGAN_OK;
}
int aclgan_bind_params16(aclgan_ctx* ctx, int group, void* w16, void* w16t) {
    ACL_REQUIRE(ctx && group >= 0 && group <= 1, "bad ctx/group");
    ctx->w16[group] = (unsigned short*)w16; ctx->w16t[group] = (unsigned short*)w16t;
    return ACLGAN_OK;
}
int aclgan_bind_loss_scale(aclgan_ctx* ctx, float* state) {
    ACL_REQUIRE(ctx, "null ctx");
    ctx->lscale = state;
    return ACLGAN_OK;
}

int64_t aclgan_group_numel(const aclgan_ctx* ctx, int group) {
    if (!ctx || group < 0 || group > ACLGAN_GROUP_SN_STATE) return -1;
    return group == ACLGAN_GROUP_SN_STATE ? ctx->sn.numel : ctx->groups[group].numel;
}
int aclgan_tensor_count(const aclgan_ctx* ctx, int group) {
    if (!ctx || group < 0 || group > ACLGAN_GROUP_SN_STATE) return -1;
    return (int)(group == ACLGAN_GROUP_SN_STATE ? ctx->sn : ctx->groups[group]).tensors.size();
}
int aclgan_tensor_info(const aclgan_ctx* ctx, int group, int index, char* name, int name_cap, int64_t* offset, int* shape4, int* ndim) {
    ACL_REQUIRE(ctx && group >= 0 && group <= ACLGAN_GROUP_SN_STATE, "bad ctx/group");
    const Group& g = group == ACLGAN_GROUP_SN_STATE ? ctx->sn : ctx->groups[group];
    ACL_REQUIRE(index >= 0 && index < (int)g.tensors.size(), "tensor index %d out of range", index);
    const TensorInfo& t = g.tensors[index];
    if (name && name_cap > 0) { strncpy(name, t.name.c_str(), name_cap - 1); name[name_cap - 1] = 0; }
    if (offset) *offset = t.offset;
    if (shape4) for (int i = 0; i < 4; ++i) shape4[i] = t.shape[i];
    if (ndim) *ndim = t.ndim;
    return ACLGAN_OK;
}
int aclgan_bind_params(aclgan_ctx* ctx, int group, float* param, float* grad, float* exp_avg, float* exp_avg_sq) {
    ACL_REQUIRE(ctx && group >= 0 && group <= 1, "bad ctx/group");
    ACL_REQUIRE(param, "param buffer is null");
    Group& g = ctx->groups[group];
    g.param = param; g.grad = grad; g.m = exp_avg; g.v = exp_avg_sq;
    return ACLGAN_OK;
}
int aclgan_bind_sn_state(aclgan_ctx* ctx, float* state) {
    ACL_REQUIRE(ctx, "null ctx");
    ACL_REQUIRE(state || ctx->sn.numel == 0, "spectral-norm state buffer is null");
    ctx->sn.param = state;
    return ACLGAN_OK;
}

static int update_need_bytes(aclgan_ctx& c, int which, int B, int H, int W, size_t* out) {
    aclgan_hparams hp;
    memset(&hp, 0, sizeof hp);
    hp.focus_loss = c.arch.gen_output_dim == 4 ? 1.f : 0.f; hp.alpha = 1.f;
    c.reset_step();
    c.dry = true; c.peak = 0; c.peak2 = 0; c.trained = -1;
    const aclgan_bucket_fn keep = c.bucket_fn;
    c.bucket_fn = nullptr;
    const int rc = which == 0 ? gen_update_impl(c, nullptr, nullptr, nullptr, B, H, W, hp, nullptr)
                              : dis_update_impl(c, nullptr, nullptr, nullptr, B, H, W, hp, nullptr);
    c.bucket_fn = keep;
    c.dry = false; c.trained = -1;
    *out = c.peak + c.peak2 + 512;
    c.reset_step();
    c.peak = 0; c.peak2 = 0;
    return rc;
}
int aclgan_workspace_bytes(aclgan_ctx* ctx, int B, int H, int W, size_t* out) {
    ACL_REQUIRE(ctx && out, "null argument");
    aclgan_ctx& c = *ctx;
    ACL_REQUIRE(c.groups[0].param && c.groups[1].param, "bind parameters first");
    size_t best = 0;
    for (int which = 0; which < 2; ++which) {
        size_t pk = 0;
        const int rc = update_need_bytes(c, which, B, H, W, &pk);
        if (rc) return rc;
        if (pk > best) best = pk;
    }
    *out = best + 4096;
    return ACLGAN_OK;
}
int aclgan_check_workspace(aclgan_ctx* ctx, int B, int H, int W) {
    ACL_REQUIRE(ctx, "null ctx");
    ACL_REQUIRE(ctx->groups[0].param && ctx->groups[1].param, "bind parameters first");
    size_t need = 0;
    const int rc = aclgan_workspace_bytes(ctx, B, H, W, &need);
    if (rc) return rc;
    if (!ctx->ws || ctx->ws_bytes < need) {
        set_error("workspace too small: bound %zu bytes, aclgan_workspace_bytes(%d, %d, %d) = %zu", ctx->ws ? ctx->ws_bytes : (size_t)0, B, H, W, need);
        return ACLGAN_ENOMEM;
    }
    return ACLGAN_OK;
}
int aclgan_step_algorithmic_bytes(aclgan_ctx* ctx, int which, int B, int H, int W, double* out) {
    ACL_REQUIRE(ctx && out && (which == 0 || which == 1), "bad argument");
    aclgan_ctx& c = *ctx;
    ACL_REQUIRE(c.groups[0].param && c.groups[1].param, "bind parameters first");
    aclgan_hparams hp;
    memset(&hp, 0, sizeof hp);
    hp.focus_loss = c.arch.gen_output_dim == 4 ? 1.f : 0.f; hp.alpha = 1.f;
    c.reset_step();
    c.dry = true; c.peak = 0; c.trained = which; c.alg_bytes = 0.0; c.exec_flops = 0.0;
    const aclgan_bucket_fn keep = c.bucket_fn;
    c.bucket_fn = nullptr;
    const int rc = which == 0 ? gen_update_impl(c, nullptr, nullptr, nullptr, B, H, W, hp, nullptr)
                              : dis_update_impl(c, nullptr, nullptr, nullptr, B, H, W, hp, nullptr);
    c.bucket_fn = keep;
    c.dry = false; c.trained = -1;
    c.reset_step();
    c.peak = 0; c.peak2 = 0;
    if (rc) return rc;
    *out = c.alg_bytes + (4.0 + 28.0) * (double)c.groups[which].numel;
    if (which == ACLGAN_GROUP_GEN && c.ema) *out += 8.0 * (double)c.groups[which].numel;
    return ACLGAN_OK;
}
int aclgan_step_executed_flops(aclgan_ctx* ctx, int which, int B, int H, int W, double* out) {
    double bytes = 0.0;
    const int rc = aclgan_step_algorithmic_bytes(ctx, which, B, H, W, &bytes);
    if (rc) return rc;
    *out = ctx->exec_flops;
    return ACLGAN_OK;
}
int aclgan_forward_workspace_bytes(aclgan_ctx* ctx, int B, int H, int W, size_t* out) {
    ACL_REQUIRE(ctx && out, "null argument");
    aclgan_ctx& c = *ctx;
    ACL_REQUIRE(c.groups[0].param && c.groups[1].param, "bind parameters first");
    ACL_REQUIRE(B >= 1 && H >= 4 && W >= 4, "bad shape (%d,%d,%d)", B, H, W);
    const int q = 1 << c.arch.gen_n_downsample, C = c.arch.gen_dim << c.arch.gen_n_downsample;
    size_t best = 0;
    for (int which = 0; which < 3; ++which) {
        c.reset_step();
        c.dry = true; c.peak = 0; c.peak2 = 0; c.trained = -1;
        Act *x = nullptr, *o = nullptr, *s = nullptr;
        std::vector<Act*> outs;
        int rc = ACLGAN_OK;
        if (which == 0) {
            rc = input_act(c, nullptr, B, 3, H, W, &x);
            if (!rc) rc = content_encode(c, ACLGAN_NET_GEN_AB, false, x, &o);
            if (!rc && o && o->dt) c.allocf(o->numel());
            if (!rc) rc = style_encode(c, ACLGAN_NET_GEN_AB, false, x, &s);
        } else if (which == 1) {
            rc = input_act(c, nullptr, B, C, std::max(1, H / q), std::max(1, W / q), &x);
            if (!rc) rc = wrap_vec(c, nullptr, B, c.arch.gen_style_dim, 1.f, &s);
            if (!rc) rc = decode(c, ACLGAN_NET_GEN_AB, false, x, s, &o);
        } else if (H >= 64 && W >= 64) {
            rc = input_act(c, nullptr, B, c.arch.input_dim_b, H, W, &x);
            if (!rc) rc = dis_forward(c, ACLGAN_NET_DIS_2, false, x, &outs);
        }
        c.dry = false;
        const size_t pk = c.peak;
        c.reset_step();
        if (rc) return rc;
        if (pk > best) best = pk;
    }
    *out = best + 4096;
    return ACLGAN_OK;
}
int aclgan_bind_workspace(aclgan_ctx* ctx, void* workspace, size_t bytes) {
    ACL_REQUIRE(ctx, "null ctx");
    ctx->ws = (char*)workspace; ctx->ws_bytes = bytes;
    return ACLGAN_OK;
}

static int step_common(aclgan_ctx* ctx, const float* x_a, const float* x_b, const float* z, const aclgan_hparams* hp, float* losses, void* stream, int group_trained,
                       int B, int H, int W) {
    ACL_REQUIRE(ctx && x_a && x_b && z && hp && losses, "null argument");
    ACL_REQUIRE(ctx->ws, "bind a workspace first (aclgan_workspace_bytes / aclgan_bind_workspace)");
    ACL_REQUIRE(ctx->groups[0].param && ctx->groups[1].param, "bind parameters first");
    ACL_REQUIRE(ctx->groups[group_trained].grad, "gradient buffer of the trained group is not bound");
    if (check_shape(*ctx, B, H, W) == ACLGAN_OK) {
        const aclgan_ctx::NeedKey key{group_trained, B, H, W, ctx->dtype, tuning_epoch(), sw(SW_DETERMINISTIC), ctx->bucket_elems > 0 ? 1 : 0};
        auto it = ctx->need_cache.find(key);
        if (it == ctx->need_cache.end()) {
            size_t need = 0;
            const int rc = update_need_bytes(*ctx, group_trained, B, H, W, &need);
            if (rc) return rc;
            it = ctx->need_cache.emplace(key, need).first;
        }
        if (it->second > ctx->ws_bytes) {
            set_error("workspace too small: bound %zu bytes, this update needs %zu (aclgan_workspace_bytes)", ctx->ws_bytes, it->second);
            return ACLGAN_ENOMEM;
        }
    }
    ctx->reset_step();
    ctx->st = (hipStream_t)stream; ctx->dry = false; ctx->peak = 0; ctx->peak2 = 0; ctx->trained = group_trained;
    return ACLGAN_OK;
}

int aclgan_gen_update(aclgan_ctx* ctx, const float* x_a, const float* x_b, const float* z, int B, int H, int W,
                      const aclgan_hparams* hp, float* losses, void* stream) {
    int rc = step_common(ctx, x_a, x_b, z, hp, losses, stream, 0, B, H, W);
    if (rc) return rc;
    ctx->ucache_hook = WinoUCache{ctx, &aclgan_ctx::ucache_lookup};
    set_wino_ucache(&ctx->ucache_hook);
    rc = gen_update_impl(*ctx, x_a, x_b, z, B, H, W, *hp, losses);
    set_wino_ucache(nullptr);
    if (rc) ctx->lanes_quiesce();
    ctx->reset_step();
    return rc;
}
int aclgan_dis_update(aclgan_ctx* ctx, const float* x_a, const float* x_b, const float* z, int B, int H, int W,
                      const aclgan_hparams* hp, float* losses, void* stream) {
    int rc = step_common(ctx, x_a, x_b, z, hp, losses, stream, 1, B, H, W);
    if (rc) return rc;
    ctx->ucache_hook = WinoUCache{ctx, &aclgan_ctx::ucache_lookup};
    set_wino_ucache(&ctx->ucache_hook);
    rc = dis_update_impl(*ctx, x_a, x_b, z, B, H, W, *hp, losses);
    set_wino_ucache(nullptr);
    if (rc) ctx->lanes_quiesce();
    ctx->reset_step();
    return rc;
}

int aclgan_set_forward_sync(aclgan_ctx* ctx, aclgan_sync_fn fn, void* user, int world_size) {
    ACL_REQUIRE(ctx && world_size >= 1, "bad ctx / world size");
    ctx->sync_fn = fn; ctx->sync_user = user; ctx->sync_world = fn ? world_size : 1;
    return ACLGAN_OK;
}

int aclgan_set_grad_buckets(aclgan_ctx* ctx, int64_t bucket_elems, aclgan_bucket_fn fn, void* user) {
    ACL_REQUIRE(ctx && bucket_elems >= 0, "bad ctx/bucket size");
    ctx->bucket_elems = bucket_elems; ctx->bucket_fn = fn; ctx->bucket_user = user;
    return ACLGAN_OK;
}

int aclgan_bucket_schedule(aclgan_ctx* ctx, int group, int B, int H, int W, int fire, int* order, int cap, int* count) {
    ACL_REQUIRE(ctx && count && group >= 0 && group <= 1, "bad argument");
    aclgan_ctx& c = *ctx;
    ACL_REQUIRE(c.groups[0].param && c.groups[1].param && c.groups[group].grad, "bind parameters (and the group's gradient buffer) first");
    ACL_REQUIRE(c.bucket_elems > 0, "aclgan_set_grad_buckets first");
    aclgan_hparams hp;
    memset(&hp, 0, sizeof hp);
    hp.focus_loss = c.arch.gen_output_dim == 4 ? 1.f : 0.f; hp.alpha = 1.f;
    c.reset_step();
    c.dry = true; c.peak = 0; c.trained = group; c.fire_dry = fire != 0;
    const int rc = group == 0 ? gen_update_impl(c, nullptr, nullptr, nullptr, B, H, W, hp, nullptr)
                              : dis_update_impl(c, nullptr, nullptr, nullptr, B, H, W, hp, nullptr);
    c.dry = false; c.fire_dry = false; c.trained = -1;
    c.reset_step();
    c.peak = 0; c.peak2 = 0;
    if (rc) return rc;
    *count = (int)c.bucket_order.size();
    for (int i = 0; i < *count && i < cap && order; ++i) order[i] = c.bucket_order[i];
    return ACLGAN_OK;
}

int aclgan_zero_grad(aclgan_ctx* ctx, int group, void* stream) {
    ACL_REQUIRE(ctx && group >= 0 && group <= 1, "bad ctx/group");
    Group& g = ctx->groups[group];
    ACL_REQUIRE(g.grad, "gradient buffer not bound");
    return fill_zero(g.grad, g.numel, (hipStream_t)stream);
}
int aclgan_adam_step(aclgan_ctx* ctx, int group, const aclgan_adam* opt, int step, void* stream) {
    ACL_REQUIRE(ctx && opt && group >= 0 && group <= 1, "bad ctx/group/opt");
    Group& g = ctx->groups[group];
    ACL_REQUIRE(g.param && g.grad && g.m && g.v, "param/grad/exp_avg/exp_avg_sq must all be bound");
    if (ctx->lscale) return adam_flat_scaled(g.param, g.grad, g.m, g.v, g.numel, opt, step, ctx->lscale, group, (hipStream_t)stream);
    return adam_flat(g.param, g.grad, g.m, g.v, g.numel, opt, step, (hipStream_t)stream);
}

int aclgan_bind_ema(aclgan_ctx* ctx, int group, float* ema) {
    ACL_REQUIRE(ctx, "null ctx");
    ACL_REQUIRE(group == ACLGAN_GROUP_GEN, "bind_ema: only the generator group (ACLGAN_GROUP_GEN) has an averaged copy; got group %d", group);
    ctx->ema = ema;
    if (!ema) ctx->fwd_weights = ACLGAN_WEIGHTS_LIVE;
    return ACLGAN_OK;
}
int aclgan_adam_step_ema(aclgan_ctx* ctx, int group, const aclgan_adam* opt, int step, float decay, int mode, void* stream) {
    ACL_REQUIRE(ctx && opt, "bad ctx/opt");
    ACL_REQUIRE(group == ACLGAN_GROUP_GEN && ctx->ema, "adam_step_ema: no averaged copy is bound for group %d (aclgan_bind_ema)", group);
    Group& g = ctx->groups[group];
    ACL_REQUIRE(g.param && g.grad && g.m && g.v, "param/grad/exp_avg/exp_avg_sq must all be bound");
    if (ctx->lscale) return adam_flat_scaled_ema(g.param, g.grad, g.m, g.v, ctx->ema, g.numel, opt, step, decay, mode, ctx->lscale, group, (hipStream_t)stream);
    return adam_flat_ema(g.param, g.grad, g.m, g.v, ctx->ema, g.numel, opt, step, decay, mode, (hipStream_t)stream);
}
int aclgan_set_forward_weights(aclgan_ctx* ctx, int which) {
    ACL_REQUIRE(ctx, "null ctx");
    ACL_REQUIRE(which == ACLGAN_WEIGHTS_LIVE || which == ACLGAN_WEIGHTS_EMA, "set_forward_weights: %d is neither ACLGAN_WEIGHTS_LIVE nor ACLGAN_WEIGHTS_EMA", which);
    ACL_REQUIRE(which == ACLGAN_WEIGHTS_LIVE || ctx->ema, "set_forward_weights: no averaged copy is bound (aclgan_bind_ema)");
    ctx->fwd_weights = which;
    return ACLGAN_OK;
}

static int fwd_begin(aclgan_ctx* ctx, void* stream) {
    ACL_REQUIRE(ctx && ctx->ws, "bind a workspace first");
    ACL_REQUIRE(ctx->groups[0].param && ctx->groups[1].param, "bind parameters first");
    ctx->reset_step();
    ctx->st = (hipStream_t)stream; ctx->dry = false; ctx->peak = 0; ctx->peak2 = 0; ctx->trained = -1;
    ctx->read_ema = ctx->fwd_weights == ACLGAN_WEIGHTS_EMA;
    return ACLGAN_OK;
}

int aclgan_gen_encode(aclgan_ctx* ctx, int net, const float* x, int B, int H, int W, float* content, float* style, void* stream) {
    int rc = fwd_begin(ctx, stream);
    if (rc) return rc;
    ACL_REQUIRE(net == ACLGAN_NET_GEN_AB || net == ACLGAN_NET_GEN_BA, "encode: net must be a generator");
    aclgan_ctx& c = *ctx;
    rc = pack_params(c);
    if (rc) return rc;
    Act *xa = nullptr, *cc = nullptr, *ss = nullptr;
    rc = input_act(c, x, B, 3, H, W, &xa);
    if (!rc && content) {
        rc = content_encode(c, net, false, xa, &cc);
        const float* src = cc ? cc->d : nullptr;
        if (!rc && cc->dt) {
            float* tmp = c.allocf(cc->numel());
            if (!tmp) { set_error("workspace too small"); rc = ACLGAN_ENOMEM; }
            else { rc = cast_storage(cc->d, cc->dt, tmp, 0, cc->numel(), c.st); src = tmp; }
        }
        if (!rc) rc = nhwc_to_nchw(src, content, cc->B, cc->C, cc->H, cc->W, c.st);
    }
    if (!rc && style) {
        rc = style_encode(c, net, false, xa, &ss);
        if (!rc) { hipError_t e = hipMemcpyAsync(style, ss->d, sizeof(float) * ss->numel(), hipMemcpyDeviceToDevice, c.st); if (e != hipSuccess) rc = hip_fail(e, "copy style"); }
    }
    c.reset_step();
    return rc;
}

int aclgan_gen_decode(aclgan_ctx* ctx, int net, const float* content, const float* style, int B, int h, int w, float* out, void* stream) {
    int rc = fwd_begin(ctx, stream);
    if (rc) return rc;
    ACL_REQUIRE(net == ACLGAN_NET_GEN_AB || net == ACLGAN_NET_GEN_BA, "decode: net must be a generator");
    aclgan_ctx& c = *ctx;
    rc = pack_params(c);
    if (rc) return rc;
    const int C = c.arch.gen_dim << c.arch.gen_n_downsample;
    Act *cc = nullptr, *ss = nullptr, *o = nullptr;
    rc = input_act(c, content, B, C, h, w, &cc);
    if (!rc) rc = wrap_vec(c, style, B, c.arch.gen_style_dim, 1.f, &ss);
    if (!rc) rc = decode(c, net, false, cc, ss, &o);
    if (!rc) rc = nhwc_to_nchw(o->d, out, o->B, o->C, o->H, o->W, c.st);
    c.reset_step();
    return rc;
}

int aclgan_dis_forward(aclgan_ctx* ctx, int net, const float* x, int B, int H, int W, float* const* outs, void* stream) {
    int rc = fwd_begin(ctx, stream);
    if (rc) return rc;
    ACL_REQUIRE(net >= ACLGAN_NET_DIS_A && net <= ACLGAN_NET_DIS_2, "dis_forward: net must be a discriminator");
    aclgan_ctx& c = *ctx;
    rc = pack_params(c);
    if (rc) return rc;
    const int Cin = net == ACLGAN_NET_DIS_2 ? c.arch.input_dim_b : c.arch.input_dim_a;
    Act* xa = nullptr;
    std::vector<Act*> o;
    rc = input_act(c, x, B, Cin, H, W, &xa);
    if (!rc) rc = dis_forward(c, net, false, xa, &o);
    for (size_t s = 0; !rc && s < o.size(); ++s) {
        hipError_t e = hipMemcpyAsync(outs[s], o[s]->d, sizeof(float) * o[s]->numel(), hipMemcpyDeviceToDevice, c.st);
        if (e != hipSuccess) rc = hip_fail(e, "copy dis out");
    }
    c.reset_step();
    return rc;
}

}
```

acl-gan_amd/csrc/switches.h:

```cpp
#pragma once
#include <atomic>

namespace aclgan {

enum SwitchId {
    SW_LANES, SW_U_BATCH, SW_NORM_MASK, SW_MLP_FUSED, SW_FAULT_AT,
    SW_GLDS_TILE, SW_WINO_X3, SW_WINO_FUSED, SW_WINO_WGRAD_FUSED, SW_WINO_S2K4, SW_DGRAD16S_DIRECT, SW_FWD16_PATCH,
    SW_DETERMINISTIC,
    SW_NOFAST, SW_NOUP5, SW_SPLIT_NWG,
    SW_NOWGKC, SW_NOUP5DGRAD,
    SW_NOSTATFUSE, SW_NOKEEPV, SW_NODIRECT,
    SW_NOWGRAD16S, SW_WGRAD16S_MINPIX, SW_NOGLDS16,
    SW_NOSMALL, SW_NOTHIN,
    SW_NOWINO, SW_NOWINOUP5, SW_WINO_VEC, SW_WINO_VEC3,
    SW_ROCTX, SW_NOUCACHE, SW_ACT16, SW_CO16, SW_SIDE_STREAM, SW_KEEPV_BUDGET_GB,
    SW_COUNT
};

const long long SW_BIAS = 1ll << 32;
extern std::atomic<long long> g_switches[SW_COUNT];
int sw_latch(SwitchId id);
inline int sw(SwitchId id) {
    const long long e = g_switches[id].load(std::memory_order_relaxed);
    return e ? (int)(e - SW_BIAS) : sw_latch(id);
}
double sw_real(SwitchId id);
int sw_set(SwitchId id, int v);

long long tuning_epoch();

}
```

acl-gan_amd/csrc/switches.hip:

```cpp
#include <string.h>
#include "common.h"

#include <climits>
#include <cmath>
#include <cstdlib>

namespace aclgan {

namespace {

enum Rule {
    R_INT,
    R_BOOL,
    R_NOT,
    R_CLAMP,
    R_RANGE,
    R_LOW4,
    R_ONEOF,
};
enum { SETTABLE = 1,
       EMPTY_UNSET = 2 };

struct Switch {
    const char* key;
    const char* env;
    int dflt;
    Rule rule;
    int lo, hi;
    int flags;
    double (*parse)(const char*);
};

double parse_real(const char* s) { return atof(s); }
const int VEC_124 = (1 << 1) | (1 << 2) | (1 << 4);

const Switch kSwitches[SW_COUNT] = {
    {"lanes",             "ACLGAN_LANES",             3,  R_CLAMP, 1, 3,       SETTABLE | EMPTY_UNSET, nullptr},
    {"u_batch",           "ACLGAN_U_BATCH",           1,  R_BOOL,  0, 0,       SETTABLE | EMPTY_UNSET, nullptr},
    {"norm_mask",         "ACLGAN_NORM_MASK",         1,  R_BOOL,  0, 0,       SETTABLE | EMPTY_UNSET, nullptr},
    {"mlp_fused",         "ACLGAN_MLP_FUSED",         1,  R_BOOL,  0, 0,       SETTABLE | EMPTY_UNSET, nullptr},
    {"fault_at",          nullptr,                    -1, R_INT,   0, 0,       SETTABLE, nullptr},
    {"glds_tile",         "ACLGAN_GLDS_TILE",         0,  R_CLAMP, 0, INT_MAX, SETTABLE, nullptr},
    {"wino_x3",           "ACLGAN_WINO_X3",           0,  R_BOOL,  0, 0,       SETTABLE, nullptr},
    {"wino_fused",        "ACLGAN_WINO_FUSED",        1,  R_LOW4,  0, 2,       SETTABLE, nullptr},
    {"wino_wgrad_fused",  "ACLGAN_WINO_WGRAD_FUSED",  1,  R_RANGE, 0, 2,       SETTABLE, nullptr},
    {"wino_s2k4",         "ACLGAN_NOWINOS2",          1,  R_NOT,   0, 0,       SETTABLE, nullptr},
    {"dgrad16s_direct",   "ACLGAN_DGRAD16S_DIRECT",   0,  R_BOOL,  0, 0,       SETTABLE, nullptr},
    {"fwd16_patch",       "ACLGAN_FWD16_PATCH",       1,  R_LOW4,  0, 2,       SETTABLE, nullptr},
    {"deterministic",     "ACLGAN_DETERMINISTIC",     0,  R_BOOL,  0, 0,       0, nullptr},
    {"nofast",            "ACLGAN_NOFAST",            0,  R_BOOL,  0, 0,       0, nullptr},
    {"noup5",             "ACLGAN_NOUP5",             0,  R_BOOL,  0, 0,       0, nullptr},
    {"split_nwg",         "ACLGAN_SPLIT_NWG",         256, R_INT,  0, 0,       0, nullptr},
    {"nowgkc",            "ACLGAN_NOWGKC",            0,  R_BOOL,  0, 0,       0, nullptr},
    {"noup5dgrad",        "ACLGAN_NOUP5DGRAD",        0,  R_BOOL,  0, 0,       0, nullptr},
    {"nostatfuse",        "ACLGAN_NOSTATFUSE",        0,  R_BOOL,  0, 0,       0, nullptr},
    {"nokeepv",           "ACLGAN_NOKEEPV",           0,  R_BOOL,  0, 0,       0, nullptr},
    {"nodirect",          "ACLGAN_NODIRECT",          0,  R_BOOL,  0, 0,       0, nullptr},
    {"nowgrad16s",        "ACLGAN_NOWGRAD16S",        0,  R_BOOL,  0, 0,       0, nullptr},
    {"wgrad16s_minpix",   "ACLGAN_WGRAD16S_MINPIX",   64, R_INT,   0, 0,       0, nullptr},
    {"noglds16",          "ACLGAN_NOGLDS16",          0,  R_BOOL,  0, 0,       0, nullptr},
    {"nosmall",           "ACLGAN_NOSMALL",           0,  R_BOOL,  0, 0,       0, nullptr},
    {"nothin",            "ACLGAN_NOTHIN",            0,  R_BOOL,  0, 0,       0, nullptr},
    {"nowino",            "ACLGAN_NOWINO",            0,  R_BOOL,  0, 0,       0, nullptr},
    {"nowinoup5",         "ACLGAN_NOWINOUP5",         0,  R_BOOL,  0, 0,       0, nullptr},
    {"wino_vec",          "ACLGAN_WINO_VEC",          2,  R_ONEOF, VEC_124, 0, 0, nullptr},
    {"wino_vec3",         "ACLGAN_WINO_VEC3",         2,  R_ONEOF, VEC_124, 0, 0, nullptr},
    {"roctx",             "ACLGAN_ROCTX",             0,  R_BOOL,  0, 0,       0, nullptr},
    {"noucache",          "ACLGAN_NOUCACHE",          0,  R_BOOL,  0, 0,       0, nullptr},
    {"act16",             "ACLGAN_ACT16",             1,  R_BOOL,  0, 0,       0, nullptr},
    {"co16",              "ACLGAN_CO16",              1,  R_BOOL,  0, 0,       0, nullptr},
    {"side_stream",       "ACLGAN_SIDE_STREAM",       1,  R_BOOL,  0, 0,       0, nullptr},
    {"keepv_budget_gb",   "ACLGAN_KEEPV_BUDGET_GB",   64, R_INT,   0, 0,       0, parse_real},
};

int normalise(const Switch& s, int v, bool from_env) {
    switch (s.rule) {
    case R_INT: return v;
    case R_BOOL: return v ? 1 : 0;
    case R_NOT: return (v ? 1 : 0) ^ (from_env ? 1 : 0);
    case R_CLAMP: return v < s.lo ? s.lo : v > s.hi ? s.hi : v;
    case R_RANGE: return (v < s.lo || v > s.hi) ? s.dflt : v;
    case R_LOW4: return (v < 0 || (v & 15) < s.lo || (v & 15) > s.hi) ? s.dflt : v;
    case R_ONEOF: return (v >= 0 && v < 31 && ((s.lo >> v) & 1)) ? v : s.dflt;
    }
    return v;
}

std::atomic<double> g_real[SW_COUNT];
std::atomic<long long> g_tuning_epoch{0};

int find(const char* key) {
    for (int i = 0; i < SW_COUNT; ++i)
        if (!strcmp(key, kSwitches[i].key)) return i;
    return -1;
}

}

std::atomic<long long> g_switches[SW_COUNT];

int sw_latch(SwitchId id) {
    const Switch& s = kSwitches[id];
    const char* e = s.env ? getenv(s.env) : nullptr;
    if (e && !*e && (s.flags & EMPTY_UNSET)) e = nullptr;
    int v = s.dflt;
    if (e && s.parse) {
        const double r = s.parse(e);
        g_real[id].store(r, std::memory_order_relaxed);
        v = std::isfinite(r) && std::fabs(r) < 2e9 ? (int)r : 0;
    } else if (e) {
        v = normalise(s, atoi(e), true);
    } else if (s.parse) {
        g_real[id].store(s.dflt, std::memory_order_relaxed);
    }
    long long expected = 0;
    return g_switches[id].compare_exchange_strong(expected, v + SW_BIAS, std::memory_order_release, std::memory_order_acquire) ? v : (int)(expected - SW_BIAS);
}

double sw_real(SwitchId id) {
    if (!g_switches[id].load(std::memory_order_acquire)) sw_latch(id);
    return g_real[id].load(std::memory_order_relaxed);
}

int sw_set(SwitchId id, int v) {
    sw(id);
    return (int)(g_switches[id].exchange(normalise(kSwitches[id], v, false) + SW_BIAS) - SW_BIAS);
}

long long tuning_epoch() { return g_tuning_epoch.load(); }

}

using namespace aclgan;

extern "C" {

int aclgan_set_deterministic(int on) { sw_set(SW_DETERMINISTIC, on); return ACLGAN_OK; }
int aclgan_get_deterministic(void) { return sw(SW_DETERMINISTIC); }

int aclgan_tuning(const char* key, int value, int* previous) {
    ACL_REQUIRE(key, "aclgan_tuning: null key");
    const int i = find(key);
    if (i < 0) { set_error("aclgan_tuning: unknown key '%s'", key); return ACLGAN_EINVAL; }
    if (!(kSwitches[i].flags & SETTABLE)) { set_error("aclgan_tuning: key '%s' is read-only (set %s before the first use instead)", key, kSwitches[i].env); return ACLGAN_EINVAL; }
    const int old = sw_set((SwitchId)i, value);
    ++g_tuning_epoch;
    if (previous) *previous = old;
    return ACLGAN_OK;
}
int aclgan_tuning_get(const char* key, long long* value) {
    ACL_REQUIRE(key && value, "aclgan_tuning_get: null argument");
    if (!strcmp(key, "epoch")) { *value = tuning_epoch(); return ACLGAN_OK; }
    const int i = find(key);
    if (i < 0) { set_error("aclgan_tuning_get: unknown key '%s'", key); return ACLGAN_EINVAL; }
    *value = sw((SwitchId)i);
    return ACLGAN_OK;
}
int aclgan_set_tuning(const char* key, int value) {
    int old = 0;
    return aclgan_tuning(key, value, &old) == ACLGAN_OK ? old : -1;
}

}
```

acl-gan_amd/trainer.py:

```python
import ctypes as C
import math
import os
from collections import OrderedDict
from contextlib import contextmanager

import torch

from . import _lib as L

__all__ = ["aclgan_Trainer", "AdaINGen", "MsImageDis", "arch_from_config", "dis_norm_from_config", "ema_from_config", "hparams_from_config"]

DIS_NORMS = ("none", "sn")


def dis_norm_from_config(hp):
    norm = hp["dis"].get("norm", "none")
    if norm not in DIS_NORMS:
        raise L.AclganError("dis.norm=%r unsupported (implemented: %s)" % (norm, ", ".join(DIS_NORMS)))
    return L.NORM[norm]


def arch_from_config(hp):
    g, d = hp["gen"], hp["dis"]
    for key, want in (("activ", "relu"), ("pad_type", "reflect")):
        if g.get(key, want) != want:
            raise L.AclganError("gen.%s=%r unsupported (only %r is reached by the shipped config)" % (key, g.get(key), want))
    for key, want in (("activ", "lrelu"), ("pad_type", "reflect"), ("gan_type", "lsgan")):
        if d.get(key, want) != want:
            raise L.AclganError("dis.%s=%r unsupported (only %r is reached by the shipped config)" % (key, d.get(key), want))
    dis_norm_from_config(hp)
    return L.Arch(int(hp["input_dim_a"]), int(hp["input_dim_b"]), int(g["dim"]), int(g["mlp_dim"]), int(g["style_dim"]),
                  int(g["output_dim"]), int(g["n_downsample"]), int(g["n_res"]), int(d["dim"]), int(d["n_layer"]),
                  int(d["num_scales"]))


def ema_from_config(hp):
    decay, start, display = hp.get("ema_decay", 0), hp.get("ema_start", 0), hp.get("ema_display", False)
    if isinstance(decay, bool) or not isinstance(decay, (int, float)) or not (0 <= decay and C.c_float(decay).value < 1):
        raise L.AclganError("ema_decay=%r: expected a number in [0, 1) (0 switches the averaged generator off)" % (decay,))
    if isinstance(start, bool) or not isinstance(start, int) or start < 0:
        raise L.AclganError("ema_start=%r: expected an integer >= 0" % (start,))
    if not isinstance(display, bool):
        raise L.AclganError("ema_display=%r: expected true or false" % (display,))
    if display and not decay > 0:
        raise L.AclganError("ema_display: true needs ema_decay > 0 (there is no averaged generator to sample from)")
    return float(decay), start, display


def hparams_from_config(hp):
    return L.HParams(float(hp["gan_w"]), float(hp["gan_cw"]), float(hp["recon_x_w"]), float(hp["focus_loss"]),
                     float(hp["focus_delta"]), float(hp["focus_upper"]), float(hp["focus_lower"]),
                     float(hp["focus_epsilon"]), float(hp.get("alpha", 1)))


class _Net:

    def __init__(self, trainer, name):
        self._t = trainer
        self.name = name
        self.net_id = L.NETS[name]
        self.group = L.GROUP_GEN if name.startswith("gen") else L.GROUP_DIS
        self._entries = [e for e in trainer._tensors[self.group] if e["net"] == name]

    def _view(self, e, buf):
        flat = buf[e["offset"]: e["offset"] + e["numel"]]
        shp = e["shape"]
        if len(shp) == 4:
            co, ci, kh, kw = shp
            return flat.view(co, kh, kw, ci).permute(0, 3, 1, 2)
        return flat.view(*shp)

    def _named_views(self, buf):
        for e in self._entries:
            yield e["key"], self._view(e, buf)

    def named_parameters(self):
        return self._named_views(self._t._param[self.group])

    def named_grads(self):
        for e in self._entries:
            yield e["key"], self._view(e, self._t._grad[self.group])

    def parameters(self):
        return [p for _, p in self.named_parameters()]

    def state_dict(self):
        return self._state_dict_of(self._t._param[self.group])

    def _state_dict_of(self, buf):
        sd = OrderedDict()
        params = OrderedDict((k, v.contiguous().clone()) for k, v in self._named_views(buf))
        bufs = self._buffers()
        for k in self._t._ref_key_order(self.name, list(params.keys()), list(bufs.keys())):
            sd[k] = params[k] if k in params else bufs[k]
        return sd

    def _buffers(self):
        return OrderedDict()

    def load_state_dict(self, sd, strict=True):
        mine = OrderedDict(self.named_parameters())
        missing = [k for k in mine if k not in sd]
        unexpected = [k for k in sd if k not in mine and k not in self._buffers()]
        if strict and (missing or unexpected):
            raise L.AclganError("load_state_dict(%s): missing %s unexpected %s" % (self.name, missing, unexpected))
        with torch.no_grad():
            for k, v in mine.items():
                if k in sd:
                    src = sd[k].to(device=v.device, dtype=torch.float32)
                    if tuple(src.shape) != tuple(v.shape):
                        raise L.AclganError("load_state_dict(%s): shape mismatch for %s: %s vs %s" % (self.name, k, tuple(src.shape), tuple(v.shape)))
                    v.copy_(src)
        for k in self._buffers():
            if k in sd:
                self._load_buffer(k, sd[k])

    def _load_buffer(self, key, value):
        self._t._dummy_buffers[self.name][key] = value.detach().clone().cpu()

    def cuda(self, *a, **k):
        return self

    def eval(self):
        return self

    def train(self, mode=True):
        return self


class AdaINGen(_Net):

    def _buffers(self):
        return self._t._dummy_buffers[self.name]

    def encode(self, images):
        t = self._t
        images = images.to(t.device, torch.float32).contiguous()
        B, Cin, H, W = images.shape
        a = t.arch
        q = 1 << a.gen_n_downsample
        content = torch.empty(B, a.gen_dim * q, H // q, W // q, device=t.device)
        style = torch.empty(B, a.gen_style_dim, 1, 1, device=t.device)
        with torch.cuda.device(t.device):
            t._ensure_workspace(B, H, W, forward_only=True)
            L.check(L.lib.aclgan_gen_encode(t._ctx, self.net_id, L.ptr(images), B, H, W, L.ptr(content), L.ptr(style), t._st()), "gen_encode")
        return content, style

    def decode(self, content, style):
        t = self._t
        content = content.to(t.device, torch.float32).contiguous()
        style = style.to(t.device, torch.float32).contiguous()
        B, Cc, h, w = content.shape
        a = t.arch
        q = 1 << a.gen_n_downsample
        out = torch.empty(B, a.gen_output_dim, h * q, w * q, device=t.device)
        with torch.cuda.device(t.device):
            t._ensure_workspace(B, h * q, w * q, forward_only=True)
            L.check(L.lib.aclgan_gen_decode(t._ctx, self.net_id, L.ptr(content), L.ptr(style), B, h, w, L.ptr(out), t._st()), "gen_decode")
        return out

    def forward(self, images):
        content, style = self.encode(images)
        return self.decode(content, style)

    __call__ = forward


class MsImageDis(_Net):

    def _sn_entries(self):
        return [e for e in self._t._tensors.get(L.GROUP_SN_STATE, []) if e["net"] == self.name]

    def _sn_view(self, e):
        flat = self._t._sn_state[e["offset"]: e["offset"] + e["numel"]]
        if e["key"].endswith("weight_v"):
            ci, kh, kw = e["vshape"]
            return flat.view(kh, kw, ci).permute(2, 0, 1).reshape(-1)
        return flat

    def _buffers(self):
        return OrderedDict((e["key"], self._sn_view(e).clone()) for e in self._sn_entries())

    def load_state_dict(self, sd, strict=True):
# ... 58 lines not shown
        L.check(L.lib.aclgan_ctx_create_dis_norm(C.byref(self.arch), dis_norm_from_config(hp), C.byref(self._ctx)), "ctx_create")
        L.check(L.lib.aclgan_set_compute_dtype(self._ctx, L.DTYPE[self.compute_dtype]), "set_compute_dtype")
        if os.environ.get("ACLGAN_WARM_STREAMS", "1") not in ("", "0"):
            with torch.cuda.device(self.device):
                L.check(L.lib.aclgan_warm_streams(0), "warm_streams")
        if self.hip_graph:
            with torch.cuda.device(self.device):
                L.check(L.lib.aclgan_ctx_enable_capture(self._ctx), "ctx_enable_capture")
        self.style_dim = hp["gen"]["style_dim"]
        self.alpha = hp["alpha"]
        self.focus_lam = hp["focus_loss"]
        self._hp = hp
        self._tensors, self._param, self._grad, self._m, self._v = {}, {}, {}, {}, {}
        self._w16, self._w16t = {}, {}
        for grp in (L.GROUP_GEN, L.GROUP_DIS):
            n = L.lib.aclgan_group_numel(self._ctx, grp)
            ents = []
            name = C.create_string_buffer(256)
            off = C.c_int64(); shp = (C.c_int * 4)(); nd = C.c_int()
            for i in range(L.lib.aclgan_tensor_count(self._ctx, grp)):
                L.check(L.lib.aclgan_tensor_info(self._ctx, grp, i, name, 256, C.byref(off), shp, C.byref(nd)))
                full = name.value.decode()
                net, key = full.split("/", 1)
                shape = tuple(shp[j] for j in range(nd.value))
                ents.append(dict(net=net, key=key, offset=off.value, shape=shape, numel=int(math.prod(shape))))
            self._tensors[grp] = ents
            self._param[grp] = torch.zeros(n, device=self.device)
            self._grad[grp] = torch.zeros(n, device=self.device)
            self._m[grp] = torch.zeros(n, device=self.device)
            self._v[grp] = torch.zeros(n, device=self.device)
            L.check(L.lib.aclgan_bind_params(self._ctx, grp, L.ptr(self._param[grp]), L.ptr(self._grad[grp]),
                                             L.ptr(self._m[grp]), L.ptr(self._v[grp])), "bind_params")
            if self.compute_dtype != "fp32":
                self._w16[grp] = torch.zeros(n, dtype=torch.int16, device=self.device)
                self._w16t[grp] = torch.zeros(n, dtype=torch.int16, device=self.device)
                L.check(L.lib.aclgan_bind_params16(self._ctx, grp, L.ptr(self._w16[grp]), L.ptr(self._w16t[grp])), "bind_params16")
        ents = []
        for i in range(L.lib.aclgan_tensor_count(self._ctx, L.GROUP_SN_STATE)):
            L.check(L.lib.aclgan_tensor_info(self._ctx, L.GROUP_SN_STATE, i, name, 256, C.byref(off), shp, C.byref(nd)))
            net, key = name.value.decode().split("/", 1)
            ents.append(dict(net=net, key=key, offset=off.value, shape=(shp[0],), numel=shp[0]))
        for e in ents:
            if e["key"].endswith("weight_v"):
                bar = next(t for t in self._tensors[L.GROUP_DIS] if t["net"] == e["net"] and t["key"] == e["key"][:-len("weight_v")] + "weight_bar")
                e["vshape"] = bar["shape"][1:]
        self._tensors[L.GROUP_SN_STATE] = ents
        self._sn_state = torch.zeros(max(1, L.lib.aclgan_group_numel(self._ctx, L.GROUP_SN_STATE)), device=self.device)
        L.check(L.lib.aclgan_bind_sn_state(self._ctx, L.ptr(self._sn_state)), "bind_sn_state")
        d = self.arch.gen_dim << self.arch.gen_n_downsample
        self._dummy_buffers = {}
        for net in ("gen_AB", "gen_BA"):
            b = OrderedDict()
            for r in range(self.arch.gen_n_res):
                for j in range(2):
                    b["dec.model.0.model.%d.model.%d.norm.running_mean" % (r, j)] = torch.zeros(d)
                    b["dec.model.0.model.%d.model.%d.norm.running_var" % (r, j)] = torch.ones(d)
            self._dummy_buffers[net] = b
        self.gen_AB, self.gen_BA = AdaINGen(self, "gen_AB"), AdaINGen(self, "gen_BA")
        self.dis_A, self.dis_B, self.dis_2 = MsImageDis(self, "dis_A"), MsImageDis(self, "dis_B"), MsImageDis(self, "dis_2")
        ds = int(hp["display_size"])
        self.z_1 = torch.randn(ds, self.style_dim, 1, 1).to(self.device)
        self.z_2 = torch.randn(ds, self.style_dim, 1, 1).to(self.device)
        self.z_3 = torch.randn(ds, self.style_dim, 1, 1).to(self.device)
        self._opt = {grp: dict(lr=float(hp["lr"]), beta1=float(hp["beta1"]), beta2=float(hp["beta2"]), eps=1e-8,
                               weight_decay=float(hp["weight_decay"]), steps=0) for grp in (L.GROUP_GEN, L.GROUP_DIS)}
        self._sched_calls = 0
        self._init_weights(hp.get("init", "kaiming"))
        self._ws = None
        self._ws_shape = None
        self._losses = torch.zeros(len(L.LOSS_NAMES), device=self.device)
        for n in L.LOSS_NAMES:
            setattr(self, n, torch.zeros((), device=self.device))
        self._zgen = None
        self._lscale = None
        if self.compute_dtype == "fp16":
            s0 = float(hp.get("loss_scale_init", 65536.0))
            self._lscale = torch.tensor([s0, 1.0 / s0, 0, 0, 0, 0, float(hp.get("loss_scale_growth_interval", 2000)), 0],
                                        dtype=torch.float32, device=self.device)
            L.check(L.lib.aclgan_bind_loss_scale(self._ctx, L.ptr(self._lscale)), "bind_loss_scale")
        self._gscale = None if self._lscale is None else torch.zeros(2, dtype=torch.float32, device=self.device)
        self._last_grp = None
        self._ema = None
        self._fwd_ema = False
        self._setup_data_parallel()
        if self._ema_decay > 0:
            self._ema = self._param[L.GROUP_GEN].clone()
            L.check(L.lib.aclgan_bind_ema(self._ctx, L.GROUP_GEN, L.ptr(self._ema)), "bind_ema")

    def __del__(self):
        try:
            if getattr(self, "_ctx", None):
                L.lib.aclgan_ctx_destroy(self._ctx)
                self._ctx = None
        except Exception:
            pass

    NETS = ("gen_AB", "gen_BA", "dis_A", "dis_B", "dis_2")

    def state_dict(self):
        sd = OrderedDict()
        for n in self.NETS:
            for k, v in getattr(self, n).state_dict().items():
                sd[n + "." + k] = v
        return sd

    def load_state_dict(self, sd, strict=True):
        known = set()
        for n in self.NETS:
            sub = OrderedDict((k[len(n) + 1:], v) for k, v in sd.items() if k.startswith(n + "."))
            known.update(n + "." + k for k in sub)
            getattr(self, n).load_state_dict(sub, strict=strict)
        extra = [k for k in sd if k not in known]
        if strict and extra:
            raise L.AclganError("load_state_dict: unexpected keys %s" % extra[:5])

    def named_parameters(self):
        for n in self.NETS:
            for k, v in getattr(self, n).named_parameters():
                yield n + "." + k, v

    def parameters(self):
        return [p for _, p in self.named_parameters()]

    def zero_grad(self):
        for grp in (L.GROUP_GEN, L.GROUP_DIS):
            self._grad[grp].zero_()

    def to(self, *a, **k):
        return self

    def cuda(self, *a, **k):
        return self

    def eval(self):
        return self

    def train(self, mode=True):
        return self

    def _ref_key_order(self, net, pkeys, bkeys):
        out = []
        for k in pkeys:
            if k.endswith("conv.weight") and k.startswith("dec.model.0."):
                pre = k[: -len("conv.weight")]
                out += [pre + "norm.running_mean", pre + "norm.running_var"]
            if k.endswith(".module.weight_bar"):
                pre = k[: -len("weight_bar")]
                out += [pre + "weight_u", pre + "weight_v"]
            out.append(k)
        assert set(out) == set(pkeys) | set(bkeys), (set(out) ^ (set(pkeys) | set(bkeys)))
        return out

    def _init_weights(self, kind):
        for grp, nets in ((L.GROUP_GEN, (self.gen_AB, self.gen_BA)), (L.GROUP_DIS, (self.dis_A, self.dis_B, self.dis_2))):
            for net in nets:
                for key, v in net.named_parameters():
                    if ".module." in key:
                        if key.endswith("weight_bar"):
                            v.copy_(torch.nn.init.kaiming_uniform_(torch.empty(tuple(v.shape)), a=math.sqrt(5.0)).to(self.device))
                        else:
                            bar = next(e for e in net._entries if e["key"] == key[: -len("bias")] + "weight_bar")
                            fan_in = int(math.prod(bar["shape"][1:]))
                            b = 1.0 / math.sqrt(fan_in)
                            v.copy_(torch.empty(tuple(v.shape)).uniform_(-b, b).to(self.device))
                    elif key.endswith(".weight"):
                        fan_in = int(math.prod(v.shape[1:]))
                        if grp == L.GROUP_DIS or kind == "gaussian":
                            w = torch.randn(tuple(v.shape)) * 0.02
                        elif kind == "kaiming":
                            w = torch.randn(tuple(v.shape)) * math.sqrt(2.0 / fan_in)
                        elif kind == "xavier":
                            fan_out = v.shape[0] * int(math.prod(v.shape[2:]))
                            w = torch.randn(tuple(v.shape)) * math.sqrt(2.0) * math.sqrt(2.0 / (fan_in + fan_out))
                        elif kind == "orthogonal":
                            w = torch.nn.init.orthogonal_(torch.empty(tuple(v.shape)), gain=math.sqrt(2.0))
                        elif kind == "default":
                            w = torch.nn.init.kaiming_uniform_(torch.empty(tuple(v.shape)), a=math.sqrt(5.0))
                        else:
                            raise L.AclganError("Unsupported initialization: %s" % kind)
                        v.copy_(w.to(self.device))
                    elif key.endswith(".gamma"):
                        v.copy_(torch.rand(tuple(v.shape)).to(self.device))
                    else:
                        v.zero_()
        for e in self._tensors[L.GROUP_SN_STATE]:
            x = torch.randn(e["numel"], dtype=torch.float64)
            self._sn_state[e["offset"]: e["offset"] + e["numel"]].copy_((x / (x.norm() + 1e-12)).float().to(self.device))

    def _st(self):
        return L.stream_ptr(self.device)

    def _ensure_workspace(self, B, H, W, forward_only=False):
        key = (B, H, W)
        have = self._ws_shape
        ep = C.c_longlong()
        L.check(L.lib.aclgan_tuning_get(b"epoch", C.byref(ep)), "tuning_get")
        if have is not None and have[0] >= B and have[1:3] == (H, W) and have[4] == ep.value and (forward_only or have[3]):
            return
        need = C.c_size_t()
        if forward_only:
            L.check(L.lib.aclgan_forward_workspace_bytes(self._ctx, B, H, W, C.byref(need)), "forward_workspace_bytes")
        else:
            L.check(L.lib.aclgan_workspace_bytes(self._ctx, B, H, W, C.byref(need)), "workspace_bytes")
        if self._ws is None or self._ws.numel() < need.value:
            self._ws = None
            try:
                self._ws = torch.empty(need.value, dtype=torch.uint8, device=self.device)
            except torch.OutOfMemoryError:
                import gc
                gc.collect(); torch.cuda.empty_cache()
                self._ws = torch.empty(need.value, dtype=torch.uint8, device=self.device)
        L.check(L.lib.aclgan_bind_workspace(self._ctx, L.ptr(self._ws), self._ws.numel()), "bind_workspace")
        self._ws_shape = key + (not forward_only, ep.value)

    def loss_scale_state(self):
        if self._lscale is None:
            return None
        v = self._lscale.cpu().tolist()
        return {"scale": v[0], "clean_updates": int(v[2]), "skipped_gen": int(v[4]), "skipped_dis": int(v[5])}

    def grad_scale(self, grp=None):
        if self._lscale is None:
            return 1.0
        if grp is None:
            grp = self._last_grp
        elif isinstance(grp, str):
            grp = {"gen": L.GROUP_GEN, "dis": L.GROUP_DIS}[grp]
        live = float(self._lscale[0].item())
        if grp is None:
            return live
        own = float(self._gscale[grp].item())
        return own if own > 0 else live

    def _draw_z(self, B):
        return [torch.randn(B, self.style_dim, 1, 1, generator=self._zgen) for _ in range(3)]

    def _current_lr(self, hp):
        if hp.get("lr_policy", "constant") == "step":
            return float(hp["lr"]) * float(hp["gamma"]) ** (self._sched_calls // int(hp["step_size"]))
        return float(hp["lr"])

    def _publish_losses(self, lo, hi):
        vals = self._losses[lo:hi].clone()
        for i in range(lo, hi):
            setattr(self, L.LOSS_NAMES[i], vals[i - lo])

    def _update(self, which, x_a, x_b, hp, z):
        grp = L.GROUP_GEN if which == "gen" else L.GROUP_DIS
        x_a = x_a.to(self.device, torch.float32).contiguous()
        x_b = x_b.to(self.device, torch.float32).contiguous()
        B, Cc, H, W = x_a.shape
        if x_b.shape != x_a.shape or Cc != 3:
            raise L.AclganError("x_a / x_b must both be (B,3,H,W); got %s and %s" % (tuple(x_a.shape), tuple(x_b.shape)))
        if z is None:
            z = self._draw_z(B)
        zz = torch.stack([t.reshape(B, self.style_dim).to(torch.float32) for t in z]).to(self.device).contiguous()
        hpc = hparams_from_config(hp)
        with torch.cuda.device(self.device):
            det_now = bool(L.lib.aclgan_get_deterministic())
            if det_now != self.deterministic:
                self.deterministic = det_now
                self._ws_shape = None
                self._graphs = {}
            self._ensure_workspace(B, H, W)
            st = self._st()
            if self._gscale is not None:
                self._gscale[grp:grp + 1].copy_(self._lscale[0:1])
                self._last_grp = grp
            fn = L.lib.aclgan_gen_update if which == "gen" else L.lib.aclgan_dis_update
            if self.hip_graph and self._reducer is None and self._run_graph(which, grp, fn, x_a, x_b, zz, B, H, W, hpc):
                pass
            else:
                L.check(L.lib.aclgan_zero_grad(self._ctx, grp, st), "zero_grad")
                if self._reducer is not None:
                    self._reducer.begin(grp)
                L.check(fn(self._ctx, L.ptr(x_a), L.ptr(x_b), L.ptr(zz), B, H, W, C.byref(hpc), L.ptr(self._losses), st), which + "_update")
            if getattr(self, "_sync_error", None) is not None:
                raise self._sync_error
            self._allreduce_grads(grp)
            o = self._opt[grp]
            o["steps"] += 1
            adam = L.Adam(self._current_lr(self._hp), o["beta1"], o["beta2"], o["eps"], o["weight_decay"])
            if grp == L.GROUP_GEN and self._ema is not None:
                mode = L.EMA_COPY if o["steps"] <= self._ema_start else L.EMA_BLEND
                L.check(L.lib.aclgan_adam_step_ema(self._ctx, grp, C.byref(adam), o["steps"], self._ema_decay, mode, st), "adam_step_ema")
            else:
                L.check(L.lib.aclgan_adam_step(self._ctx, grp, C.byref(adam), o["steps"], st), "adam_step")
        if which == "gen":
            self._publish_losses(0, 12)
        else:
            self._publish_losses(12, 16)

    def _run_graph(self, which, grp, fn, x_a, x_b, zz, B, H, W, hpc):
        key = (B, H, W, bytes(hpc), self._ws.data_ptr(), self._ws.numel(), self.compute_dtype, self.deterministic)
        ent = self._graphs.get(which)
        if ent is None or ent["key"] != key:
            self._graphs[which] = {"key": key, "graph": None}
            return False
        if ent["graph"] is None:
            try:
                sx_a, sx_b, szz = torch.empty_like(x_a), torch.empty_like(x_b), torch.empty_like(zz)
                g = torch.cuda.CUDAGraph()
                with torch.cuda.graph(g):
                    st = self._st()
                    L.check(L.lib.aclgan_zero_grad(self._ctx, grp, st), "zero_grad (capture)")
                    L.check(fn(self._ctx, L.ptr(sx_a), L.ptr(sx_b), L.ptr(szz), B, H, W, C.byref(hpc), L.ptr(self._losses), st), which + "_update (capture)")
                ent.update(graph=g, x_a=sx_a, x_b=sx_b, zz=szz)
            except Exception as e:
                import warnings
                warnings.warn("aclgan_Trainer: HIP-graph capture failed (%r); running eagerly" % (e,))
                self.hip_graph = False
                self._graphs = {}
                return False
        ent["x_a"].copy_(x_a); ent["x_b"].copy_(x_b); ent["zz"].copy_(zz)
        ent["graph"].replay()
        return True

    def _dist_world(self):
        import torch.distributed as dist
        if not (dist.is_available() and dist.is_initialized()):
            return 0
        if dist.get_world_size() == 1 and os.environ.get("ACLGAN_BENCH_FORCE_DIST") != "1":
            return 0
        return dist.get_world_size()

    def _setup_data_parallel(self):
        self._reducer = None
        self._exposed_events, self._exposed_ms = [], 0.0
        world = self._dist_world()
        if not world:
            return
        import torch.distributed as dist
        from .ddp import BucketReducer, broadcast_flat
        for grp in (L.GROUP_GEN, L.GROUP_DIS):
            for buf in (self._param[grp], self._m[grp], self._v[grp]):
                broadcast_flat(buf)
        if self._ema is not None:
            broadcast_flat(self._ema)
        if self._tensors[L.GROUP_SN_STATE]:
            broadcast_flat(self._sn_state)
        steps = torch.tensor([self._opt[0]["steps"], self._opt[1]["steps"], self._sched_calls], dtype=torch.int64, device=self.device)
        dist.broadcast(steps, 0)
        self._opt[0]["steps"], self._opt[1]["steps"], self._sched_calls = (int(v) for v in steps.tolist())
        self._zgen = torch.Generator().manual_seed(torch.initial_seed() + dist.get_rank())
        if os.environ.get("ACLGAN_DDP_OVERLAP", "1") != "0":
            self._reducer = BucketReducer(self._ctx, lambda g: self._grad[g], world)
        if self.hip_graph:
            import warnings
            warnings.warn("aclgan_Trainer: hip_graph=True is ignored in data-parallel runs (world size %d): updates run eagerly" % world)
            self.hip_graph = False
        if self._hp.get("ddp_global_focus", False) or os.environ.get("ACLGAN_DDP_GLOBAL_FOCUS") == "1":
            def on_sync(user, ptr, n):
                try:
                    off = int(ptr) - self._ws.data_ptr()
                    t = self._ws[off: off + 4 * n].view(torch.float32)
                    dist.all_reduce(t, op=dist.ReduceOp.SUM)
                except BaseException as e:
                    self._sync_error = e
            self._sync_error = None
            self._sync_cb = L.SYNC_FN(on_sync)
            L.check(L.lib.aclgan_set_forward_sync(self._ctx, self._sync_cb, None, world), "set_forward_sync")

    def _allreduce_grads(self, grp):
        world = self._dist_world()
        if not world:
            return
        ev = (torch.cuda.Event(enable_timing=True), torch.cuda.Event(enable_timing=True))
        ev[0].record()
        if self._reducer is not None:
            self._reducer.finish(grp)
        else:
            from .ddp import allreduce_flat
            allreduce_flat(self._grad[grp], world)
        ev[1].record()
        self._exposed_events.append(ev)
        if len(self._exposed_events) > 4096:
            self.allreduce_exposed_ms()

    def allreduce_exposed_ms(self, reset=True):
        torch.cuda.synchronize(self.device)
        self._exposed_ms += sum(a.elapsed_time(b) for a, b in self._exposed_events)
        self._exposed_events = []
        v = self._exposed_ms
        if reset:
            self._exposed_ms = 0.0
        return v

    def gen_update(self, x_a, x_b, hyperparameters, z=None):
        self._update("gen", x_a, x_b, hyperparameters, z)

    def dis_update(self, x_a, x_b, hyperparameters, z=None):
        self._update("dis", x_a, x_b, hyperparameters, z)

    def update_learning_rate(self):
        self._sched_calls += 1

    def focus_translation(self, x_fg, x_bg, x_focus):
        B, Cc, H, W = x_fg.shape
        if Cc != 3 or x_focus.shape[1] != 1 or tuple(x_bg.shape) != (B, 3, H, W):
            raise L.AclganError("focus_translation: expected (B,3,H,W), (B,3,H,W), (B,1,H,W)")

        def dense(t):
            t = t.to(self.device, torch.float32)
            ok = t.stride(3) == 1 and t.stride(2) == W and t.stride(1) == H * W
            return t if ok else t.contiguous()
        fg, bg, fo = dense(x_fg), dense(x_bg), dense(x_focus)
        out = torch.empty(B, 3, H, W, device=self.device)
        with torch.cuda.device(self.device):
            L.check(L.lib.aclgan_focus_translation_nchw(L.ptr(fg), fg.stride(0), L.ptr(bg), bg.stride(0), L.ptr(fo), fo.stride(0),
                                                        L.ptr(out), B, H * W, self._st()), "focus_translation")
        return out

    @property
    def ema_updates(self):
        return self._opt[L.GROUP_GEN]["steps"]

    def _require_ema(self, what):
        if self._ema is None:
            raise L.AclganError("%s: the averaged generator is off (set ema_decay in (0, 1))" % what)

    @contextmanager
    def ema_weights(self):
        self._require_ema("ema_weights()")
        prev = self._fwd_ema
        self._select_forward_weights(True)
        try:
            yield self
        finally:
            self._select_forward_weights(prev)

    def _select_forward_weights(self, ema):
        L.check(L.lib.aclgan_set_forward_weights(self._ctx, L.WEIGHTS_EMA if ema else L.WEIGHTS_LIVE), "set_forward_weights")
        self._fwd_ema = ema

    def ema_state_dict(self):
        self._require_ema("ema_state_dict()")
        return {"AB": self.gen_AB._state_dict_of(self._ema), "BA": self.gen_BA._state_dict_of(self._ema)}

    def ema_reset(self):
        self._require_ema("ema_reset()")
        self._ema.copy_(self._param[L.GROUP_GEN])

    def sample(self, x_a, x_b, ema=False):
        if ema:
            with self.ema_weights():
                return self.sample(x_a, x_b)
        x_a = x_a.to(self.device, torch.float32)
        x_b = x_b.to(self.device, torch.float32)
        if not (self.focus_lam > 0):
            return self._sample_plain(x_a, x_b)
        X_A, X_B, A_fake, B_fake, A2_fake, m_A, m_B, m_A2, m_rec, A_rec = [], [], [], [], [], [], [], [], [], []
        for i in range(x_a.size(0)):
            xa = x_a[i].unsqueeze(0)
            X_A.append(xa); X_B.append(x_b[i].unsqueeze(0))
            c_1, s_1 = self.gen_BA.encode(xa)
            img, mask = self.gen_BA.decode(c_1, self.z_1[i].unsqueeze(0)).split(3, 1)
            A_fake.append(self.focus_translation(img, xa, mask)); m_A.append(mask)
            img, mask = self.gen_BA.decode(c_1, s_1).split(3, 1)
            A_rec.append(img); m_rec.append(mask)
            c_2, _ = self.gen_AB.encode(xa)
            xb_img, mask = self.gen_AB.decode(c_2, self.z_2[i].unsqueeze(0)).split(3, 1)
            xb_img = self.focus_translation(xb_img, xa, mask)
            B_fake.append(xb_img); m_B.append(mask)
            c_3, _ = self.gen_BA.encode(xb_img)
            img, mask = self.gen_BA.decode(c_3, self.z_3[i].unsqueeze(0)).split(3, 1)
            A2_fake.append(self.focus_translation(img, xb_img, mask)); m_A2.append(mask)
        cat = torch.cat
        return (cat(X_A), cat(A_fake), cat(m_A), cat(B_fake), cat(m_B), cat(A2_fake), cat(m_A2), cat(A_rec), cat(m_rec))

    def _sample_plain(self, x_a, x_b):
        X_A, X_B, A_fake, B_fake, A2_fake, A_rec, B_rec = [], [], [], [], [], [], []
        for i in range(x_a.size(0)):
            xa = x_a[i].unsqueeze(0)
            X_A.append(xa); X_B.append(x_b[i].unsqueeze(0))
            c_1, s_1 = self.gen_BA.encode(xa)
            A_fake.append(self.gen_BA.decode(c_1, self.z_1[i].unsqueeze(0)))
            A_rec.append(self.gen_BA.decode(c_1, s_1))
            c_2, _ = self.gen_AB.encode(xa)
            x_B1 = self.gen_AB.decode(c_2, self.z_2[i].unsqueeze(0))
            B_fake.append(x_B1)
            c_3, _ = self.gen_BA.encode(x_B1)
            A2_fake.append(self.gen_BA.decode(c_3, self.z_3[i].unsqueeze(0)))
            c_4, s_4 = self.gen_AB.encode(x_b)
            B_rec.append(self.gen_AB.decode(c_4, s_4))
        cat = torch.cat
        return (cat(X_A), cat(A_fake), cat(B_fake), cat(A2_fake), cat(A_rec), cat(X_B), cat(B_rec))

    def _opt_state_dict(self, grp):
        o = self._opt[grp]
        state = {}
        nets = (self.gen_AB, self.gen_BA) if grp == L.GROUP_GEN else (self.dis_A, self.dis_B, self.dis_2)
        idx = 0
        for net in nets:
            for e in net._entries:
                if o["steps"] > 0:
                    state[idx] = {"step": torch.tensor(float(o["steps"])),
                                  "exp_avg": net._view(e, self._m[grp]).contiguous().clone(),
                                  "exp_avg_sq": net._view(e, self._v[grp]).contiguous().clone()}
                idx += 1
        pg = {"lr": self._current_lr(self._hp), "betas": (o["beta1"], o["beta2"]), "eps": o["eps"], "weight_decay": o["weight_decay"],
              "amsgrad": False, "initial_lr": float(self._hp["lr"]), "params": list(range(idx))}
        return {"state": state, "param_groups": [pg]}

    def _load_opt_state_dict(self, grp, sd):
        o = self._opt[grp]
        nets = (self.gen_AB, self.gen_BA) if grp == L.GROUP_GEN else (self.dis_A, self.dis_B, self.dis_2)
        idx = 0
        steps = 0
        with torch.no_grad():
            for net in nets:
                for e in net._entries:
                    st = sd["state"].get(idx)
                    if st is not None:
                        net._view(e, self._m[grp]).copy_(st["exp_avg"].to(self.device))
# ... 61 lines not shown
```

include/aclgan_hip.h:

```cpp
#ifndef ACLGAN_HIP_H
#define ACLGAN_HIP_H

#include <stddef.h>
#include <stdint.h>

#ifdef __cplusplus
extern "C" {
#endif

#define ACLGAN_OK 0
#define ACLGAN_EINVAL (-1)
#define ACLGAN_EUNSUPPORTED (-2)
#define ACLGAN_EHIP (-3)
#define ACLGAN_ENOMEM (-4)

#define ACLGAN_ACT_NONE 0
#define ACLGAN_ACT_RELU 1
#define ACLGAN_ACT_LRELU 2
#define ACLGAN_ACT_TANH 3

#define ACLGAN_NORM_NONE 0
#define ACLGAN_NORM_IN 1
#define ACLGAN_NORM_ADAIN 2
#define ACLGAN_NORM_LN 3
// ... 15 lines not shown
#define ACLGAN_NET_GEN_AB 0
#define ACLGAN_NET_GEN_BA 1
#define ACLGAN_NET_DIS_A 2
#define ACLGAN_NET_DIS_B 3
#define ACLGAN_NET_DIS_2 4

enum {
    ACLGAN_L_GEN_ADV_A = 0, ACLGAN_L_GEN_ADV_B, ACLGAN_L_GEN_ADV_2,
    ACLGAN_L_GEN_FOCUS_B_SIZE, ACLGAN_L_GEN_FOCUS_B_DIGIT,
    ACLGAN_L_GEN_FOCUS_A_SIZE, ACLGAN_L_GEN_FOCUS_A_DIGIT,
    ACLGAN_L_GEN_FOCUS_A2_SIZE, ACLGAN_L_GEN_FOCUS_A2_DIGIT,
    ACLGAN_L_IDT_A, ACLGAN_L_IDT_B, ACLGAN_L_GEN_TOTAL,
    ACLGAN_L_DIS_A, ACLGAN_L_DIS_B, ACLGAN_L_DIS_2, ACLGAN_L_DIS_TOTAL,
    ACLGAN_L_COUNT
};

typedef struct aclgan_arch {
    int input_dim_a, input_dim_b;
    int gen_dim, gen_mlp_dim, gen_style_dim, gen_output_dim, gen_n_downsample, gen_n_res;
    int dis_dim, dis_n_layer, dis_num_scales;
} aclgan_arch;

typedef struct aclgan_hparams {
    float gan_w, gan_cw, recon_x_w;
    float focus_loss, focus_delta, focus_upper, focus_lower, focus_epsilon;
    float alpha;
} aclgan_hparams;

typedef struct aclgan_adam {
    float lr, beta1, beta2, eps, weight_decay;
} aclgan_adam;

typedef struct aclgan_conv_desc {
    int B, Hi, Wi, Ci;
    int Co, k, stride, pad;
    int upsample;
    int act;
} aclgan_conv_desc;

typedef struct aclgan_ctx aclgan_ctx;

int aclgan_version(void);
long long aclgan_launch_count(void);
int aclgan_gemm_slices_f32(const float* A, const float* B, float* C, int T, int K, int N, int nslices, void* stream);
int aclgan_winograd_filter_frag(const float* w, float* Uf, int Co, int Ci, int flip, void* stream);
int aclgan_conv3x3_winograd_fused(const float* x, const float* Uf, const float* bias, float* y, int B, int H, int W, int Cin, int Cout, int act, int reflect,
                                  int accumulate, float* stats, void* stream);
size_t aclgan_gemm_slices_x3_scratch_bytes(int T, int K, int N, int nslices);
int aclgan_gemm_slices_x3(const float* A, const float* B, float* C, int T, int K, int N, int nslices, void* scratch, void* stream);
const char* aclgan_last_error(void);
int aclgan_set_deterministic(int on);
int aclgan_get_deterministic(void);

int aclgan_ctx_create(const aclgan_arch* arch, aclgan_ctx** out);
int aclgan_ctx_create_dis_norm(const aclgan_arch* arch, int dis_norm, aclgan_ctx** out);
void aclgan_ctx_destroy(aclgan_ctx* ctx);
int aclgan_ctx_enable_capture(aclgan_ctx* ctx);
int aclgan_warm_streams(int lanes);

int aclgan_debug_capture_masks(aclgan_ctx* ctx, unsigned char* dst, size_t cap_bytes);
int aclgan_debug_mask_count(const aclgan_ctx* ctx);
int aclgan_debug_mask_info(const aclgan_ctx* ctx, int index, int* dims4, long long* offset, int* act);

int64_t aclgan_group_numel(const aclgan_ctx* ctx, int group);
int aclgan_tensor_count(const aclgan_ctx* ctx, int group);
int aclgan_tensor_info(const aclgan_ctx* ctx, int group, int index, char* name, int name_cap,
                       int64_t* offset, int* shape4, int* ndim);
int aclgan_bind_params(aclgan_ctx* ctx, int group, float* param, float* grad, float* exp_avg,
                       float* exp_avg_sq);
int aclgan_bind_sn_state(aclgan_ctx* ctx, float* state);
size_t aclgan_sn_scratch_bytes(int n, const int* co, const int* k);
int aclgan_sn_power_iteration(int n, const int* co, const int* k, const float* w, float* u, float* v, float* w_sn, float* sigma,
                              void* scratch, void* stream);
int aclgan_sn_fold(int n, const int* co, const int* k, const float* w, const float* g, const float* u, const float* v,
                   const float* sigma, float* grad, void* scratch, void* stream);

int aclgan_set_compute_dtype(aclgan_ctx* ctx, int dtype);
int aclgan_bind_params16(aclgan_ctx* ctx, int group, void* w16, void* w16t);
int aclgan_bind_loss_scale(aclgan_ctx* ctx, float* state);

int aclgan_workspace_bytes(aclgan_ctx* ctx, int B, int H, int W, size_t* out);
int aclgan_bind_workspace(aclgan_ctx* ctx, void* workspace, size_t bytes);
int aclgan_check_workspace(aclgan_ctx* ctx, int B, int H, int W);
int aclgan_forward_workspace_bytes(aclgan_ctx* ctx, int B, int H, int W, size_t* out);
int aclgan_step_algorithmic_bytes(aclgan_ctx* ctx, int which, int B, int H, int W, double* out);
int aclgan_step_executed_flops(aclgan_ctx* ctx, int which, int B, int H, int W, double* out);

int aclgan_gen_update(aclgan_ctx* ctx, const float* x_a, const float* x_b, const float* z,
                      int B, int H, int W, const aclgan_hparams* hp, float* losses, void* stream);
int aclgan_dis_update(aclgan_ctx* ctx, const float* x_a, const float* x_b, const float* z,
                      int B, int H, int W, const aclgan_hparams* hp, float* losses, void* stream);
typedef void (*aclgan_bucket_fn)(void* user, int group, int bucket, int64_t offset, int64_t numel);
int aclgan_set_grad_buckets(aclgan_ctx* ctx, int64_t bucket_elems, aclgan_bucket_fn fn, void* user);
int aclgan_bucket_schedule(aclgan_ctx* ctx, int group, int B, int H, int W, int fire, int* order, int cap, int* count);

typedef void (*aclgan_sync_fn)(void* user, float* sums_dev, int n);
int aclgan_set_forward_sync(aclgan_ctx* ctx, aclgan_sync_fn fn, void* user, int world_size);

int aclgan_zero_grad(aclgan_ctx* ctx, int group, void* stream);
int aclgan_adam_step(aclgan_ctx* ctx, int group, const aclgan_adam* opt, int step, void* stream);
int aclgan_bind_ema(aclgan_ctx* ctx, int group, float* ema);
int aclgan_adam_step_ema(aclgan_ctx* ctx, int group, const aclgan_adam* opt, int step, float decay, int mode, void* stream);
int aclgan_set_forward_weights(aclgan_ctx* ctx, int which);

int aclgan_gen_encode(aclgan_ctx* ctx, int net, const float* x, int B, int H, int W,
                      float* content, float* style, void* stream);
int aclgan_gen_decode(aclgan_ctx* ctx, int net, const float* content, const float* style,
                      int B, int h, int w, float* out, void* stream);
int aclgan_dis_forward(aclgan_ctx* ctx, int net, const float* x, int B, int H, int W,
                       float* const* outs, void* stream);

int aclgan_conv2d_fwd(const aclgan_conv_desc* d, const float* x, const float* w, const float* bias,
                      float* y, void* stream);
int aclgan_conv2d_fwd_ws(const aclgan_conv_desc* d, const float* x, const float* w, const float* bias,
                         float* y, void* scratch, void* stream);
size_t aclgan_conv2d_fwd_scratch_bytes(const aclgan_conv_desc* d);
int aclgan_conv2d_dgrad(const aclgan_conv_desc* d, const float* dy, const float* w, float* dx,
                        void* scratch, int accumulate, void* stream);
size_t aclgan_conv2d_dgrad_scratch_bytes(const aclgan_conv_desc* d);
int aclgan_conv2d_wgrad(const aclgan_conv_desc* d, const float* x, const float* dy, float* dw,
                        float* db, void* stream);
int aclgan_conv2d_wgrad_ws(const aclgan_conv_desc* d, const float* x, const float* dy, float* dw,
                           float* db, void* scratch, void* stream);
size_t aclgan_conv2d_wgrad_scratch_bytes(const aclgan_conv_desc* d);
int aclgan_conv16_eligible(const aclgan_conv_desc* d, int which);
int aclgan_pack_weights16(const float* w, void* w16, void* w16t, int Co, int taps, int Ci, int dtype, void* stream);
int aclgan_conv2d_fwd16(const aclgan_conv_desc* d, int dtype, const float* x, const float* w, const void* w16,
                        const float* bias, float* y, void* scratch, void* stream);
int aclgan_conv2d_fwd16_x16(const aclgan_conv_desc* d, int dtype, const void* x16, const float* w, const void* w16,
                            const float* bias, float* y, void* scratch, void* stream);
int aclgan_conv2d_dgrad16(const aclgan_conv_desc* d, int dtype, const float* dy, const float* w, const void* w16t,
                          float* dx, int accumulate, void* scratch, void* stream);
int aclgan_conv2d_wgrad16(const aclgan_conv_desc* d, int dtype, const float* x, const float* dy, float* dw,
                          float* db, void* scratch, void* stream);

int aclgan_conv16s_ok(const aclgan_conv_desc* d, int which);
int aclgan_conv2d_fwd16s(const aclgan_conv_desc* d, int dtype, const void* x16, const void* w16, const float* bias, void* y, int y_storage, void* stream);
int aclgan_set_tuning(const char* key, int value);
int aclgan_tuning(const char* key, int value, int* previous);
int aclgan_tuning_get(const char* key, long long* value);
int aclgan_conv2d_fwd16s_stats_chunk(const aclgan_conv_desc* d);
int aclgan_conv2d_fwd16s_stats(const aclgan_conv_desc* d, int dtype, const void* x16, const void* w16, const float* bias, void* y, int y_storage,
                               float* stats, void* stream);
size_t aclgan_conv2d_dgrad16s_scratch_bytes(const aclgan_conv_desc* d);
int aclgan_conv2d_dgrad16s(const aclgan_conv_desc* d, int dtype, const void* dy16, const void* w16t, void* dx, int dx_storage, int accumulate,
                           void* scratch, void* stream);
int aclgan_conv2d_wgrad16_st(const aclgan_conv_desc* d, int dtype, const void* x, int x_storage, const void* dy, int dy_storage, float* dw, float* db,
                             void* scratch, void* stream);
int aclgan_cast_storage(const void* src, int src_storage, void* dst, int dst_storage, int64_t n, void* stream);
int aclgan_norm_fwd_st(int kind, int act, int B, int HW, int C, const void* x, const float* w, const float* b, int w_stride, const void* residual,
                       void* y, float* mean, float* rstd, void* scratch, const int* storage, void* stream);
int aclgan_norm_bwd_st(int kind, int act, int B, int HW, int C, const void* x, const void* y, const void* dy, const float* w, int w_stride,
                       const float* mean, const float* rstd, void* dx, float* dw, float* db, void* dres, int dres_accumulate, void* scratch,
                       const int* storage, void* stream);
int aclgan_conv2d_fwd16_x16_st(const aclgan_conv_desc* d, int dtype, const void* x16, const float* w, const void* w16, const float* bias, void* y,
                               int y_storage, void* scratch, void* stream);
int aclgan_norm_fwd_x(int kind, int act, int B, int HW, int C, const void* x, const float* w, const float* b, int w_stride, const void* residual,
                      void* y, float* mean, float* rstd, void* scratch, const float* stats, int stats_chunk, const int* storage, float* ss_out,
                      void* stream);
int aclgan_norm_bwd_x(int kind, int act, int B, int HW, int C, const void* x, const void* y, const void* dy, const float* w, int w_stride,
                      const float* mean, const float* rstd, void* dx, float* dw, float* db, void* dres, int dres_accumulate, void* scratch,
                      const int* storage, const float* ss, float* sbc_out, void* stream);
int aclgan_norm_bwd_ln_params(const float* sbc, int B, int C, float* dgamma, float* dbeta, void* stream);
size_t aclgan_conv2d_fwd16_scratch_bytes(const aclgan_conv_desc* d);
size_t aclgan_conv2d_dgrad16_scratch_bytes(const aclgan_conv_desc* d);
size_t aclgan_conv2d_wgrad16_scratch_bytes(const aclgan_conv_desc* d);
// ... 83 lines not shown
```

Baseline: 100.5.

## Carry content encodings from discriminator step into generator step

During the discriminator update, the two content-encoder passes now keep their outputs in a reserved tail of the workspace. That covers the fp32 input casts, conv outputs, norm outputs, mean/rstd and sign masks. The following generator update then adopts these buffers instead of recomputing both encoder forwards, provided the trainer's input pointer, version, generator-parameter and epoch checks match. Any parameter rebind, Adam generator step, EMA or weight switch drops the carry. The cost is a larger workspace requirement and a smaller usable region for other scratch, which can shrink keep buffers. It also adds bookkeeping that must stay consistent with the generator's forward layout.

```diff
diff --git a/acl-gan_amd/_lib.py b/acl-gan_amd/_lib.py
--- a/acl-gan_amd/_lib.py
+++ b/acl-gan_amd/_lib.py
@@ -55,6 +55,7 @@
 GROUP_GEN, GROUP_DIS, GROUP_SN_STATE = 0, 1, 2
 EMA_COPY, EMA_BLEND = 0, 1
 WEIGHTS_LIVE, WEIGHTS_EMA = 0, 1
+CARRY_OFF, CARRY_KEEP, CARRY_ADOPT = 0, 1, 2
 NETS = {"gen_AB": 0, "gen_BA": 1, "dis_A": 2, "dis_B": 3, "dis_2": 4}
 LOSS_NAMES = [
     "loss_gen_adv_A", "loss_gen_adv_B", "loss_gen_adv_2",
@@ -132,6 +133,7 @@
     "aclgan_tuning": (ci, [C.c_char_p, ci, C.POINTER(ci)]),
     "aclgan_tuning_get": (ci, [C.c_char_p, C.POINTER(C.c_longlong)]),
     "aclgan_check_workspace": (ci, [vp, ci, ci, ci]),
+    "aclgan_ctx_carry_encodings": (ci, [vp, ci]),
     "aclgan_conv2d_fwd16s_stats_chunk": (ci, [C.POINTER(ConvDesc)]),
     "aclgan_conv2d_fwd16s_stats": (ci, [C.POINTER(ConvDesc), ci, vp, vp, vp, vp, ci, vp, vp]),
     "aclgan_conv2d_dgrad16s_scratch_bytes": (sz, [C.POINTER(ConvDesc)]),
diff --git a/acl-gan_amd/csrc/common.h b/acl-gan_amd/csrc/common.h
--- a/acl-gan_amd/csrc/common.h
+++ b/acl-gan_amd/csrc/common.h
@@ -13,6 +13,7 @@
 int hip_fail(hipError_t e, const char* what);
 
 extern std::atomic<long long> g_launches;
+extern std::atomic<long long> g_enc_reuse_hits;
 
 #define ACL_CHECK_LAUNCH(what)                                           \
     do {                                                                 \
diff --git a/acl-gan_amd/csrc/engine.hip b/acl-gan_amd/csrc/engine.hip
--- a/acl-gan_amd/csrc/engine.hip
+++ b/acl-gan_amd/csrc/engine.hip
@@ -168,6 +168,35 @@
         }
     };
     std::map<NeedKey, size_t> need_cache;
+    struct CarryBlock { float *in32, *co, *out, *mean, *rstd, *ss; int B, H, W, C, co_st, out_st; };
+    struct CarryRec {
+        bool valid = false;
+        int B = 0, H = 0, W = 0, dtype = 0, determ = 0;
+        const float* x_a = nullptr;
+        long long gen_epoch = 0, tune_epoch = 0;
+        char* ws = nullptr; size_t ws_bytes = 0, bytes = 0;
+        std::vector<CarryBlock> blocks[2];
+    };
+    CarryRec carry;
+    long long gen_epoch = 0;
+    int carry_arm = ACLGAN_CARRY_OFF;
+    int carry_call = ACLGAN_CARRY_OFF;
+    int carry_mode = ACLGAN_CARRY_OFF;
+    int carry_pass = 0; size_t carry_blk = 0;
+    bool carry_fail = false;
+    size_t carry_res = 0;
+    int last_mode[2] = {ACLGAN_CARRY_OFF, ACLGAN_CARRY_OFF};
+    void carry_drop() { carry.valid = false; ++gen_epoch; }
+    size_t lim() const { return carry_res ? ((ws_bytes - carry_res) & ~(size_t)255) : ws_bytes; }
+    void* alloc_carry(size_t bytes) {
+        const size_t need = carry_res + ((bytes + 255) & ~(size_t)255);
+        if (dry) { carry_res = need; return (void*)(uintptr_t)4096; }
+        if (peak + peak2 + need + 512 > ws_bytes) return nullptr;
+        carry_res = need;
+        return ws + ((ws_bytes - need) & ~(size_t)255);
+    }
+    void carry_pass_begin(int pass) { carry_mode = carry_call; carry_pass = pass; carry_blk = 0; }
+    void carry_pass_end() { carry_mode = ACLGAN_CARRY_OFF; }
     double alg_bytes = 0.0;
     void count(double bytes) { alg_bytes += bytes; }
     double exec_flops = 0.0;
@@ -212,8 +241,8 @@
         top2 = need;
         if (need > peak2) peak2 = need;
         if (dry) return (void*)(uintptr_t)4096;
-        if (peak + need + 256 > ws_bytes) return nullptr;
-        return ws + ((ws_bytes - need) & ~(size_t)255);
+        if (peak + need + 256 > lim()) return nullptr;
+        return ws + ((lim() - need) & ~(size_t)255);
     }
     int side_fork() {
         if (dry) return ACLGAN_OK;
@@ -395,7 +424,7 @@
         if (nlanes > 1) { const size_t e = (top + 255) & ~(size_t)255; if (e > hw[cur_lane]) hw[cur_lane] = e; }
         if (top > peak) peak = top;
         if (dry) return (void*)(uintptr_t)(a + 4096);
-        if (top + peak2 + 256 > ws_bytes) return nullptr;
+        if (top + peak2 + 256 > lim()) return nullptr;
         return ws + a;
     }
     float* allocf(int64_t n) { return (float*)alloc((size_t)n * sizeof(float)); }
@@ -403,6 +432,15 @@
         Act* a = new Act();
         a->B = B; a->H = H; a->W = W; a->C = C; a->need_grad = need_grad; a->dt = st; a->gdt = st;
         a->d = (float*)alloc((size_t)a->numel() * (st ? 2 : 4));
+        if (need_grad) a->g = allocf(a->numel());
+        acts.push_back(a);
+        wrote(a);
+        return a;
+    }
+    Act* new_act_at(int B, int H, int W, int C, bool need_grad, int st, float* d) {
+        Act* a = new Act();
+        a->B = B; a->H = H; a->W = W; a->C = C; a->need_grad = need_grad; a->dt = st; a->gdt = st;
+        a->d = d;
         if (need_grad) a->g = allocf(a->numel());
         acts.push_back(a);
         wrote(a);
@@ -519,6 +557,8 @@
 
 static const char* NET_NAMES[5] = {"gen_AB", "gen_BA", "dis_A", "dis_B", "dis_2"};
 
+std::atomic<long long> g_enc_reuse_hits{0};
+
 }
 
 const float* aclgan_ctx::param(int group, int net, const std::string& key) const {
@@ -584,29 +624,61 @@
     const bool a16 = h16 && c.act16();
     const bool s_bwd = a16 && f16 && d16 && w16 && conv16s_ok(g, 1);
     const bool s_fwd = a16 && f16 && conv16s_ok(g, 0) && in->dt != 0;
-    if (in->dt != 0 && !(f16 && (w16 || !train_w))) {
-        Act* in32 = c.new_act(in->B, in->H, in->W, in->C, false, 0);
+    const bool keep = c.carry_mode == ACLGAN_CARRY_KEEP, adopt = c.carry_mode == ACLGAN_CARRY_ADOPT, carried = keep || adopt;
+    const bool tw = train_w || keep;
+    aclgan_ctx::CarryBlock cb_dry = {};
+    aclgan_ctx::CarryBlock* cb = &cb_dry;
+    if (carried && !c.dry) {
+        std::vector<aclgan_ctx::CarryBlock>& blocks = c.carry.blocks[c.carry_pass];
+        if (keep) { blocks.push_back(cb_dry); cb = &blocks.back(); }
+        else {
+            if (c.carry_blk >= blocks.size()) { set_error("conv_block: the kept encodings hold no block %zu", c.carry_blk); return ACLGAN_EINVAL; }
+            cb = &blocks[c.carry_blk++];
+        }
+    }
+    auto carry_buf = [&](float* aclgan_ctx::CarryBlock::*slot, size_t bytes) -> float* {
+        if (adopt && !c.dry) return cb->*slot;
+        float* p = (float*)c.alloc_carry(bytes);
+        cb->*slot = p;
+        return p;
+    };
+    if (in->dt != 0 && !(f16 && (w16 || !tw))) {
+        Act* in32 = carried ? c.new_act_at(in->B, in->H, in->W, in->C, false, 0, carry_buf(&aclgan_ctx::CarryBlock::in32, (size_t)in->numel() * 4))
+                            : c.new_act(in->B, in->H, in->W, in->C, false, 0);
         NEED(in32->d);
-        RUN(cast_storage(in->d, in->dt, in32->d, 0, in->numel(), c.st));
+        if (!adopt) RUN(cast_storage(in->d, in->dt, in32->d, 0, in->numel(), c.st));
         in = in32;
     }
     const int out_st = (a16 && Co % 64 == 0 && out16) ? dt : 0;
     const int co_st = has_norm ? ((s_bwd && sw(SW_CO16)) ? dt : 0) : ((f16 || !out_st) ? out_st : 0);
-    Act* co = c.new_act(g.B, g.Ho, g.Wo, Co, want_grad, co_st);
+    const size_t co_bytes = (size_t)g.B * g.Ho * g.Wo * Co * (co_st ? 2 : 4), out_bytes = (size_t)g.B * g.Ho * g.Wo * Co * (out_st ? 2 : 4);
+    if (adopt && !c.dry && (cb->B != g.B || cb->H != g.Ho || cb->W != g.Wo || cb->C != Co || cb->co_st != co_st || cb->out_st != out_st)) {
+        set_error("conv_block: the kept encodings do not match this layer (%d x %d x %d x %d)", g.B, g.Ho, g.Wo, Co);
+        return ACLGAN_EINVAL;
+    }
+    if (keep) { cb->B = g.B; cb->H = g.Ho; cb->W = g.Wo; cb->C = Co; cb->co_st = co_st; cb->out_st = out_st; }
+    Act* co = carried ? c.new_act_at(g.B, g.Ho, g.Wo, Co, want_grad, co_st, carry_buf(&aclgan_ctx::CarryBlock::co, co_bytes))
+                      : c.new_act(g.B, g.Ho, g.Wo, Co, want_grad, co_st);
     NEED(co->d); if (want_grad) NEED(co->g);
     Act* out = co;
     float *mean = nullptr, *rstd = nullptr, *ss = nullptr;
     const int HW = g.Ho * g.Wo;
     if (has_norm) {
-        out = c.new_act(g.B, g.Ho, g.Wo, Co, want_grad, out_st);
+        out = carried ? c.new_act_at(g.B, g.Ho, g.Wo, Co, want_grad, out_st, carry_buf(&aclgan_ctx::CarryBlock::out, out_bytes))
+                      : c.new_act(g.B, g.Ho, g.Wo, Co, want_grad, out_st);
         NEED(out->d); if (want_grad) NEED(out->g);
         const int nstat = ns.kind == ACLGAN_NORM_LN ? g.B : g.B * Co;
-        mean = c.allocf(nstat); rstd = c.allocf(nstat);
+        if (carried) { mean = carry_buf(&aclgan_ctx::CarryBlock::mean, (size_t)nstat * 4); rstd = carry_buf(&aclgan_ctx::CarryBlock::rstd, (size_t)nstat * 4); }
+        else { mean = c.allocf(nstat); rstd = c.allocf(nstat); }
         NEED(mean); NEED(rstd);
-        if (want_grad && (act == ACLGAN_ACT_RELU || act == ACLGAN_ACT_LRELU) && sw(SW_NORM_MASK)) { ss = c.allocf((int64_t)2 * g.B * Co); NEED(ss); }
+        if ((want_grad || keep) && (act == ACLGAN_ACT_RELU || act == ACLGAN_ACT_LRELU) && sw(SW_NORM_MASK)) {
+            ss = carried ? carry_buf(&aclgan_ctx::CarryBlock::ss, (size_t)2 * g.B * Co * 4) : c.allocf((int64_t)2 * g.B * Co);
+            NEED(ss);
+        }
         co->gdt = s_bwd ? dt : 0;
     } else if (out_st && !co_st) {
-        out = c.new_act(g.B, g.Ho, g.Wo, Co, want_grad, out_st);
+        out = carried ? c.new_act_at(g.B, g.Ho, g.Wo, Co, want_grad, out_st, carry_buf(&aclgan_ctx::CarryBlock::out, out_bytes))
+                      : c.new_act(g.B, g.Ho, g.Wo, Co, want_grad, out_st);
         NEED(out->d); if (want_grad) NEED(out->g);
         out->gdt = 0;
     } else {
@@ -614,17 +686,18 @@
     }
     if (gin->need_grad && !s_bwd) gin->gdt = 0;
     float* keepV = nullptr;
-    if (train_w && !f16 && !w16) {
+    if (train_w && !adopt && !f16 && !w16) {
         const size_t kb = conv_fwd_keep_bytes(g);
         if (kb && c.keep_total + kb <= (size_t)(sw_real(SW_KEEPV_BUDGET_GB) * 1073741824.0) + 1) { keepV = (float*)c.alloc(kb); NEED(keepV); c.keep_total += kb; }
     }
     const size_t ubytes = f16 ? 0 : conv_wino_u_bytes(g);
-    if (ubytes && c.ucache_reserve(W.w, g.up ? 2 : 0, ubytes)) { set_error("workspace too small (filter-transform cache)"); return ACLGAN_ENOMEM; }
+    if (ubytes && !adopt && c.ucache_reserve(W.w, g.up ? 2 : 0, ubytes)) { set_error("workspace too small (filter-transform cache)"); return ACLGAN_ENOMEM; }
     const double es_in = in->dt ? 2.0 : 4.0, es_co = co->dt ? 2.0 : 4.0, es_out = out->dt ? 2.0 : 4.0, es_w = f16 ? 2.0 : 4.0;
-    c.count(es_in * (double)in->numel() + es_w * (double)Co * g.K + 4.0 * Co + es_co * (double)co->numel());
-    c.exec_flops += conv_exec_flops(g, 0, f16);
-    if (out != co) c.count((es_co + es_out) * (double)co->numel() + ((has_norm && residual) ? (residual->dt ? 2.0 : 4.0) * (double)co->numel() : 0.0));
+    if (!adopt) c.count(es_in * (double)in->numel() + es_w * (double)Co * g.K + 4.0 * Co + es_co * (double)co->numel());
+    if (!adopt) c.exec_flops += conv_exec_flops(g, 0, f16);
+    if (out != co && !adopt) c.count((es_co + es_out) * (double)co->numel() + ((has_norm && residual) ? (residual->dt ? 2.0 : 4.0) * (double)co->numel() : 0.0));
     const size_t mark = c.top;
+    if (!adopt) {
     const int schunk = !has_norm ? 0 : (s_fwd ? conv_fwd16s_stats_chunk(g) : (!f16 ? conv_fwd_stats_chunk(g) : 0));
     float* stats = nullptr;
     if (schunk) { stats = c.allocf((size_t)2 * g.B * (HW / schunk) * Co); NEED(stats); }
@@ -646,6 +719,7 @@
         RUN(norm_fwd(ns.kind, act, g.B, HW, Co, co->d, ns.w, ns.b, ns.w_stride, residual ? residual->d : nullptr, out->d, mean, rstd, scr, c.st, stats, schunk, &nst, ss));
     } else if (out != co) {
         RUN(cast_storage(co->d, co->dt, out->d, out->dt, co->numel(), c.st));
+    }
     }
     c.top = mark;
     *out_p = out;
@@ -808,7 +882,7 @@
 }
 
 static int content_encode(aclgan_ctx& c, int net, bool train, Act* x, Act** out) {
-    PassScope pass(c, net, "encode");
+    PassScope pass(c, net, c.carry_mode == ACLGAN_CARRY_ADOPT ? "encode(adopted)" : "encode");
     const aclgan_arch& a = c.arch;
     char buf[160];
     NormSpec in_; in_.kind = ACLGAN_NORM_IN;
@@ -1317,9 +1391,12 @@
 #define PASS(expr) do { CHK(expr); CHK(c.mark()); } while (0)
     CHK(c.mark());
     CHK(c.set_lane(L0));
-    PASS(content_encode(c, AB, true, xa, &c1));
+    c.carry_pass_begin(0);
+    { const int rc = content_encode(c, AB, true, xa, &c1); c.carry_pass_end(); CHK(rc); } CHK(c.mark());
     CHK(c.set_lane(L1));
-    PASS(content_encode(c, BA, true, xa, &c2));
+    c.carry_pass_begin(1);
+    { const int rc = content_encode(c, BA, true, xa, &c2); c.carry_pass_end(); CHK(rc); } CHK(c.mark());
+    if (c.carry_call == ACLGAN_CARRY_ADOPT && !c.dry) { c.carry.valid = false; g_enc_reuse_hits += 2; }
     PASS(style_encode(c, BA, true, xa, &s2));
     CHK(c.set_lane(L0));
     PASS(decode(c, AB, true, c1, z1, &dB4)); CHK(zero_grad_of(c, dB4));
@@ -1437,9 +1514,11 @@
     const int L0 = 0, L1 = 1, L2 = c.nlanes > 2 ? 2 : 1, LS = c.nlanes > 2 ? 2 : 0;
     CHK(c.mark());
     CHK(c.set_lane(L0));
-    PASS(content_encode(c, AB, false, xa, &c1));
+    c.carry_pass_begin(0);
+    { const int rc = content_encode(c, AB, false, xa, &c1); c.carry_pass_end(); CHK(rc); } CHK(c.mark());
     CHK(c.set_lane(L1));
-    PASS(content_encode(c, BA, false, xa, &c2));
+    c.carry_pass_begin(1);
+    { const int rc = content_encode(c, BA, false, xa, &c2); c.carry_pass_end(); CHK(rc); } CHK(c.mark());
     CHK(c.set_lane(L0));
     PASS(decode(c, AB, false, c1, z1, &dB4));
     PASS(blend(c, dB4, xa, nullptr, &xB, nullptr, c.new_view(jB, 0, B), nullptr));
@@ -1553,11 +1632,13 @@
 int aclgan_set_compute_dtype(aclgan_ctx* ctx, int dtype) {
     ACL_REQUIRE(ctx && dtype >= ACLGAN_DTYPE_FP32 && dtype <= ACLGAN_DTYPE_FP16, "bad ctx / dtype %d", dtype);
     ctx->dtype = dtype;
+    ctx->carry_drop();
     return ACLGAN_OK;
 }
 int aclgan_bind_params16(aclgan_ctx* ctx, int group, void* w16, void* w16t) {
     ACL_REQUIRE(ctx && group >= 0 && group <= 1, "bad ctx/group");
     ctx->w16[group] = (unsigned short*)w16; ctx->w16t[group] = (unsigned short*)w16t;
+    ctx->carry_drop();
     return ACLGAN_OK;
 }
 int aclgan_bind_loss_scale(aclgan_ctx* ctx, float* state) {
@@ -1590,6 +1671,7 @@
     ACL_REQUIRE(param, "param buffer is null");
     Group& g = ctx->groups[group];
     g.param = param; g.grad = grad; g.m = exp_avg; g.v = exp_avg_sq;
+    ctx->carry_drop();
     return ACLGAN_OK;
 }
 int aclgan_bind_sn_state(aclgan_ctx* ctx, float* state) {
@@ -1599,19 +1681,21 @@
     return ACLGAN_OK;
 }
 
-static int update_need_bytes(aclgan_ctx& c, int which, int B, int H, int W, size_t* out) {
+static int update_need_bytes(aclgan_ctx& c, int which, int B, int H, int W, size_t* out, int carry = ACLGAN_CARRY_OFF) {
     aclgan_hparams hp;
     memset(&hp, 0, sizeof hp);
     hp.focus_loss = c.arch.gen_output_dim == 4 ? 1.f : 0.f; hp.alpha = 1.f;
     c.reset_step();
     c.dry = true; c.peak = 0; c.peak2 = 0; c.trained = -1;
+    c.carry_call = carry; c.carry_res = 0;
     const aclgan_bucket_fn keep = c.bucket_fn;
     c.bucket_fn = nullptr;
     const int rc = which == 0 ? gen_update_impl(c, nullptr, nullptr, nullptr, B, H, W, hp, nullptr)
                               : dis_update_impl(c, nullptr, nullptr, nullptr, B, H, W, hp, nullptr);
     c.bucket_fn = keep;
     c.dry = false; c.trained = -1;
-    *out = c.peak + c.peak2 + 512;
+    *out = c.peak + c.peak2 + 512 + (c.carry_res ? c.carry_res + 256 : 0);
+    c.carry_call = ACLGAN_CARRY_OFF; c.carry_res = 0;
     c.reset_step();
     c.peak = 0; c.peak2 = 0;
     return rc;
@@ -1621,12 +1705,13 @@
     aclgan_ctx& c = *ctx;
     ACL_REQUIRE(c.groups[0].param && c.groups[1].param, "bind parameters first");
     size_t best = 0;
-    for (int which = 0; which < 2; ++which) {
-        size_t pk = 0;
-        const int rc = update_need_bytes(c, which, B, H, W, &pk);
-        if (rc) return rc;
-        if (pk > best) best = pk;
-    }
+    for (int which = 0; which < 2; ++which)
+        for (int carry = 0; carry <= (sw(SW_ENC_REUSE) ? 1 : 0); ++carry) {
+            size_t pk = 0;
+            const int rc = update_need_bytes(c, which, B, H, W, &pk, !carry ? ACLGAN_CARRY_OFF : which == 0 ? ACLGAN_CARRY_ADOPT : ACLGAN_CARRY_KEEP);
+            if (rc) return rc;
+            if (pk > best) best = pk;
+        }
     *out = best + 4096;
     return ACLGAN_OK;
 }
@@ -1651,12 +1736,14 @@
     hp.focus_loss = c.arch.gen_output_dim == 4 ? 1.f : 0.f; hp.alpha = 1.f;
     c.reset_step();
     c.dry = true; c.peak = 0; c.trained = which; c.alg_bytes = 0.0; c.exec_flops = 0.0;
+    c.carry_call = c.last_mode[which]; c.carry_res = 0;
     const aclgan_bucket_fn keep = c.bucket_fn;
     c.bucket_fn = nullptr;
     const int rc = which == 0 ? gen_update_impl(c, nullptr, nullptr, nullptr, B, H, W, hp, nullptr)
                               : dis_update_impl(c, nullptr, nullptr, nullptr, B, H, W, hp, nullptr);
     c.bucket_fn = keep;
     c.dry = false; c.trained = -1;
+    c.carry_call = ACLGAN_CARRY_OFF; c.carry_res = 0;
     c.reset_step();
     c.peak = 0; c.peak2 = 0;
     if (rc) return rc;
@@ -1709,6 +1796,14 @@
 int aclgan_bind_workspace(aclgan_ctx* ctx, void* workspace, size_t bytes) {
     ACL_REQUIRE(ctx, "null ctx");
     ctx->ws = (char*)workspace; ctx->ws_bytes = bytes;
+    ctx->carry_drop();
+    return ACLGAN_OK;
+}
+
+int aclgan_ctx_carry_encodings(aclgan_ctx* ctx, int mode) {
+    ACL_REQUIRE(ctx, "null ctx");
+    ACL_REQUIRE(mode == ACLGAN_CARRY_OFF || mode == ACLGAN_CARRY_KEEP || mode == ACLGAN_CARRY_ADOPT, "carry_encodings: mode %d is none of ACLGAN_CARRY_OFF / KEEP / ADOPT", mode);
+    ctx->carry_arm = mode;
     return ACLGAN_OK;
 }
 
@@ -1718,22 +1813,43 @@
     ACL_REQUIRE(ctx->ws, "bind a workspace first (aclgan_workspace_bytes / aclgan_bind_workspace)");
     ACL_REQUIRE(ctx->groups[0].param && ctx->groups[1].param, "bind parameters first");
     ACL_REQUIRE(ctx->groups[group_trained].grad, "gradient buffer of the trained group is not bound");
+    int carry = ctx->carry_arm;
+    ctx->carry_arm = ACLGAN_CARRY_OFF;
+    if (carry != (group_trained == 0 ? ACLGAN_CARRY_ADOPT : ACLGAN_CARRY_KEEP) || !sw(SW_ENC_REUSE) || ctx->mask_dst || sw(SW_FAULT_AT) >= 0) carry = ACLGAN_CARRY_OFF;
+    if (carry) {
+        hipStreamCaptureStatus cs = hipStreamCaptureStatusNone;
+        if (hipStreamIsCapturing((hipStream_t)stream, &cs) != hipSuccess) { (void)hipGetLastError(); carry = ACLGAN_CARRY_OFF; }
+        else if (cs != hipStreamCaptureStatusNone) carry = ACLGAN_CARRY_OFF;
+    }
+    if (carry == ACLGAN_CARRY_ADOPT) {
+        const aclgan_ctx::CarryRec& r = ctx->carry;
+        if (!(r.valid && r.B == B && r.H == H && r.W == W && r.dtype == ctx->dtype && r.x_a == x_a && r.gen_epoch == ctx->gen_epoch &&
+              r.tune_epoch == tuning_epoch() && r.determ == sw(SW_DETERMINISTIC) && r.ws == ctx->ws && r.ws_bytes == ctx->ws_bytes))
+            carry = ACLGAN_CARRY_OFF;
+    }
+    if (carry != ACLGAN_CARRY_ADOPT) ctx->carry.valid = false;
     if (check_shape(*ctx, B, H, W) == ACLGAN_OK) {
-        const aclgan_ctx::NeedKey key{group_trained, B, H, W, ctx->dtype, tuning_epoch(), sw(SW_DETERMINISTIC), ctx->bucket_elems > 0 ? 1 : 0};
-        auto it = ctx->need_cache.find(key);
-        if (it == ctx->need_cache.end()) {
-            size_t need = 0;
-            const int rc = update_need_bytes(*ctx, group_trained, B, H, W, &need);
-            if (rc) return rc;
-            it = ctx->need_cache.emplace(key, need).first;
-        }
-        if (it->second > ctx->ws_bytes) {
+        for (;;) {
+            const aclgan_ctx::NeedKey key{group_trained, B, H, W, ctx->dtype, tuning_epoch(), sw(SW_DETERMINISTIC), (ctx->bucket_elems > 0 ? 1 : 0) | (carry << 1)};
+            auto it = ctx->need_cache.find(key);
+            if (it == ctx->need_cache.end()) {
+                size_t need = 0;
+                const int rc = update_need_bytes(*ctx, group_trained, B, H, W, &need, carry);
+                if (rc) return rc;
+                it = ctx->need_cache.emplace(key, need).first;
+            }
+            if (it->second <= ctx->ws_bytes) break;
+            if (carry) { carry = ACLGAN_CARRY_OFF; ctx->carry.valid = false; continue; }
             set_error("workspace too small: bound %zu bytes, this update needs %zu (aclgan_workspace_bytes)", ctx->ws_bytes, it->second);
             return ACLGAN_ENOMEM;
         }
-    }
+    } else carry = ACLGAN_CARRY_OFF;
     ctx->reset_step();
     ctx->st = (hipStream_t)stream; ctx->dry = false; ctx->peak = 0; ctx->peak2 = 0; ctx->trained = group_trained;
+    ctx->carry_call = carry; ctx->carry_mode = ACLGAN_CARRY_OFF; ctx->carry_fail = false;
+    ctx->carry_res = carry == ACLGAN_CARRY_ADOPT ? ctx->carry.bytes : 0;
+    if (carry == ACLGAN_CARRY_KEEP) { ctx->carry.blocks[0].clear(); ctx->carry.blocks[1].clear(); }
+    ctx->last_mode[group_trained] = carry;
     return ACLGAN_OK;
 }
 
@@ -1746,6 +1862,8 @@
     rc = gen_update_impl(*ctx, x_a, x_b, z, B, H, W, *hp, losses);
     set_wino_ucache(nullptr);
     if (rc) ctx->lanes_quiesce();
+    ctx->carry.valid = false;
+    ctx->carry_call = ACLGAN_CARRY_OFF; ctx->carry_res = 0;
     ctx->reset_step();
     return rc;
 }
@@ -1758,6 +1876,13 @@
     rc = dis_update_impl(*ctx, x_a, x_b, z, B, H, W, *hp, losses);
     set_wino_ucache(nullptr);
     if (rc) ctx->lanes_quiesce();
+    if (ctx->carry_call == ACLGAN_CARRY_KEEP) {
+        aclgan_ctx::CarryRec& r = ctx->carry;
+        r.valid = rc == ACLGAN_OK && !ctx->carry_fail && ctx->carry_res > 0;
+        r.B = B; r.H = H; r.W = W; r.dtype = ctx->dtype; r.determ = sw(SW_DETERMINISTIC); r.x_a = x_a;
+        r.gen_epoch = ctx->gen_epoch; r.tune_epoch = tuning_epoch(); r.ws = ctx->ws; r.ws_bytes = ctx->ws_bytes; r.bytes = ctx->carry_res;
+    }
+    ctx->carry_call = ACLGAN_CARRY_OFF; ctx->carry_res = 0;
     ctx->reset_step();
     return rc;
 }
@@ -1805,6 +1930,7 @@
     ACL_REQUIRE(ctx && opt && group >= 0 && group <= 1, "bad ctx/group/opt");
     Group& g = ctx->groups[group];
     ACL_REQUIRE(g.param && g.grad && g.m && g.v, "param/grad/exp_avg/exp_avg_sq must all be bound");
+    if (group == ACLGAN_GROUP_GEN) ctx->carry_drop();
     if (ctx->lscale) return adam_flat_scaled(g.param, g.grad, g.m, g.v, g.numel, opt, step, ctx->lscale, group, (hipStream_t)stream);
     return adam_flat(g.param, g.grad, g.m, g.v, g.numel, opt, step, (hipStream_t)stream);
 }
@@ -1813,6 +1939,7 @@
     ACL_REQUIRE(ctx, "null ctx");
     ACL_REQUIRE(group == ACLGAN_GROUP_GEN, "bind_ema: only the generator group (ACLGAN_GROUP_GEN) has an averaged copy; got group %d", group);
     ctx->ema = ema;
+    ctx->carry_drop();
     if (!ema) ctx->fwd_weights = ACLGAN_WEIGHTS_LIVE;
     return ACLGAN_OK;
 }
@@ -1821,6 +1948,7 @@
     ACL_REQUIRE(group == ACLGAN_GROUP_GEN && ctx->ema, "adam_step_ema: no averaged copy is bound for group %d (aclgan_bind_ema)", group);
     Group& g = ctx->groups[group];
     ACL_REQUIRE(g.param && g.grad && g.m && g.v, "param/grad/exp_avg/exp_avg_sq must all be bound");
+    ctx->carry_drop();
     if (ctx->lscale) return adam_flat_scaled_ema(g.param, g.grad, g.m, g.v, ctx->ema, g.numel, opt, step, decay, mode, ctx->lscale, group, (hipStream_t)stream);
     return adam_flat_ema(g.param, g.grad, g.m, g.v, ctx->ema, g.numel, opt, step, decay, mode, (hipStream_t)stream);
 }
@@ -1829,12 +1957,14 @@
     ACL_REQUIRE(which == ACLGAN_WEIGHTS_LIVE || which == ACLGAN_WEIGHTS_EMA, "set_forward_weights: %d is neither ACLGAN_WEIGHTS_LIVE nor ACLGAN_WEIGHTS_EMA", which);
     ACL_REQUIRE(which == ACLGAN_WEIGHTS_LIVE || ctx->ema, "set_forward_weights: no averaged copy is bound (aclgan_bind_ema)");
     ctx->fwd_weights = which;
+    ctx->carry_drop();
     return ACLGAN_OK;
 }
 
 static int fwd_begin(aclgan_ctx* ctx, void* stream) {
     ACL_REQUIRE(ctx && ctx->ws, "bind a workspace first");
     ACL_REQUIRE(ctx->groups[0].param && ctx->groups[1].param, "bind parameters first");
+    ctx->carry.valid = false; ctx->carry_arm = ACLGAN_CARRY_OFF; ctx->carry_res = 0;
     ctx->reset_step();
     ctx->st = (hipStream_t)stream; ctx->dry = false; ctx->peak = 0; ctx->peak2 = 0; ctx->trained = -1;
     ctx->read_ema = ctx->fwd_weights == ACLGAN_WEIGHTS_EMA;
diff --git a/acl-gan_amd/csrc/switches.h b/acl-gan_amd/csrc/switches.h
--- a/acl-gan_amd/csrc/switches.h
+++ b/acl-gan_amd/csrc/switches.h
@@ -4,7 +4,7 @@
 namespace aclgan {
 
 enum SwitchId {
-    SW_LANES, SW_U_BATCH, SW_NORM_MASK, SW_MLP_FUSED, SW_FAULT_AT,
+    SW_LANES, SW_U_BATCH, SW_NORM_MASK, SW_MLP_FUSED, SW_FAULT_AT, SW_ENC_REUSE,
     SW_GLDS_TILE, SW_WINO_X3, SW_WINO_FUSED, SW_WINO_WGRAD_FUSED, SW_WINO_S2K4, SW_DGRAD16S_DIRECT, SW_FWD16_PATCH,
     SW_DETERMINISTIC,
     SW_NOFAST, SW_NOUP5, SW_SPLIT_NWG,
diff --git a/acl-gan_amd/csrc/switches.hip b/acl-gan_amd/csrc/switches.hip
--- a/acl-gan_amd/csrc/switches.hip
+++ b/acl-gan_amd/csrc/switches.hip
@@ -40,6 +40,7 @@
     {"norm_mask",         "ACLGAN_NORM_MASK",         1,  R_BOOL,  0, 0,       SETTABLE | EMPTY_UNSET, nullptr},
     {"mlp_fused",         "ACLGAN_MLP_FUSED",         1,  R_BOOL,  0, 0,       SETTABLE | EMPTY_UNSET, nullptr},
     {"fault_at",          nullptr,                    -1, R_INT,   0, 0,       SETTABLE, nullptr},
+    {"enc_reuse",         nullptr,                    1,  R_BOOL,  0, 0,       SETTABLE, nullptr},
     {"glds_tile",         "ACLGAN_GLDS_TILE",         0,  R_CLAMP, 0, INT_MAX, SETTABLE, nullptr},
     {"wino_x3",           "ACLGAN_WINO_X3",           0,  R_BOOL,  0, 0,       SETTABLE, nullptr},
     {"wino_fused",        "ACLGAN_WINO_FUSED",        1,  R_LOW4,  0, 2,       SETTABLE, nullptr},
@@ -151,6 +152,7 @@
 int aclgan_tuning_get(const char* key, long long* value) {
     ACL_REQUIRE(key && value, "aclgan_tuning_get: null argument");
     if (!strcmp(key, "epoch")) { *value = tuning_epoch(); return ACLGAN_OK; }
+    if (!strcmp(key, "enc_reuse_hits")) { *value = g_enc_reuse_hits.load(); return ACLGAN_OK; }
     const int i = find(key);
     if (i < 0) { set_error("aclgan_tuning_get: unknown key '%s'", key); return ACLGAN_EINVAL; }
     *value = sw((SwitchId)i);
diff --git a/acl-gan_amd/trainer.py b/acl-gan_amd/trainer.py
--- a/acl-gan_amd/trainer.py
+++ b/acl-gan_amd/trainer.py
@@ -99,6 +99,7 @@
         return OrderedDict()
 
     def load_state_dict(self, sd, strict=True):
+        self._t._carry_epoch += 1
         mine = OrderedDict(self.named_parameters())
         missing = [k for k in mine if k not in sd]
         unexpected = [k for k in sd if k not in mine and k not in self._buffers()]
@@ -323,6 +324,9 @@
         self._last_grp = None
         self._ema = None
         self._fwd_ema = False
+        self._carry = None
+        self._carry_epoch = 0
+        self.enc_reuse = bool(hp.get("enc_reuse", True))
         self._setup_data_parallel()
         if self._ema_decay > 0:
             self._ema = self._param[L.GROUP_GEN].clone()
@@ -346,6 +350,7 @@
         return sd
 
     def load_state_dict(self, sd, strict=True):
+        self._carry_epoch += 1
         known = set()
         for n in self.NETS:
             sub = OrderedDict((k[len(n) + 1:], v) for k, v in sd.items() if k.startswith(n + "."))
@@ -473,6 +478,11 @@
         own = float(self._gscale[grp].item())
         return own if own > 0 else live
 
+    def _carry_state(self, x_a):
+        g = L.GROUP_GEN
+        packs = tuple((t.data_ptr(), t._version) for t in (self._w16.get(g), self._w16t.get(g)) if t is not None)
+        return (x_a.data_ptr(), tuple(x_a.shape), x_a._version, self._param[g].data_ptr(), self._param[g]._version, packs, self._carry_epoch)
+
     def _draw_z(self, B):
         return [torch.randn(B, self.style_dim, 1, 1, generator=self._zgen) for _ in range(3)]
 
@@ -515,6 +525,13 @@
                 L.check(L.lib.aclgan_zero_grad(self._ctx, grp, st), "zero_grad")
                 if self._reducer is not None:
                     self._reducer.begin(grp)
+                kept, self._carry, carry = self._carry, None, L.CARRY_OFF
+                if self.enc_reuse and not self.hip_graph:
+                    if which == "dis":
+                        self._carry, carry = (x_a, self._carry_state(x_a)), L.CARRY_KEEP
+                    elif kept is not None and kept[0] is x_a and kept[1] == self._carry_state(x_a):
+                        carry = L.CARRY_ADOPT
+                L.check(L.lib.aclgan_ctx_carry_encodings(self._ctx, carry), "ctx_carry_encodings")
                 L.check(fn(self._ctx, L.ptr(x_a), L.ptr(x_b), L.ptr(zz), B, H, W, C.byref(hpc), L.ptr(self._losses), st), which + "_update")
             if getattr(self, "_sync_error", None) is not None:
                 raise self._sync_error
@@ -671,6 +688,7 @@
             self._select_forward_weights(prev)
 
     def _select_forward_weights(self, ema):
+        self._carry_epoch += 1
         L.check(L.lib.aclgan_set_forward_weights(self._ctx, L.WEIGHTS_EMA if ema else L.WEIGHTS_LIVE), "set_forward_weights")
         self._fwd_ema = ema
 
diff --git a/include/aclgan_hip.h b/include/aclgan_hip.h
--- a/include/aclgan_hip.h
+++ b/include/aclgan_hip.h
@@ -121,6 +121,10 @@
 int aclgan_workspace_bytes(aclgan_ctx* ctx, int B, int H, int W, size_t* out);
 int aclgan_bind_workspace(aclgan_ctx* ctx, void* workspace, size_t bytes);
 int aclgan_check_workspace(aclgan_ctx* ctx, int B, int H, int W);
+#define ACLGAN_CARRY_OFF 0
+#define ACLGAN_CARRY_KEEP 1
+#define ACLGAN_CARRY_ADOPT 2
+int aclgan_ctx_carry_encodings(aclgan_ctx* ctx, int mode);
 int aclgan_forward_workspace_bytes(aclgan_ctx* ctx, int B, int H, int W, size_t* out);
 int aclgan_step_algorithmic_bytes(aclgan_ctx* ctx, int which, int B, int H, int W, double* out);
 int aclgan_step_executed_flops(aclgan_ctx* ctx, int which, int B, int H, int W, double* out);
```

After: 104.2, median of 6. 1.04x the previous value.
